# ruanjue/smartdenovo

Hardware: AMD Instinct MI355X
Metric: Gbp of candidate pairs aligned/sec (wtzmo all-vs-all) (higher is better)
Workload: dtype int32/int16

## Files before the change

include/wtzmo_hip.h:

```cpp
#ifndef WTZMO_HIP_H
#define WTZMO_HIP_H

#include <stdint.h>

#ifdef __cplusplus
extern "C" {
#endif

#define WTZ_OK        0
#define WTZ_E_ARG    -1
#define WTZ_E_HIP    -2
#define WTZ_E_POOL   -3
#define WTZ_E_STATE  -4

typedef struct {
	uint32_t ksize, zsize, hk, hz, ksave, kovl, ncand, nbest;
	uint32_t kwin, kstep, ztot, zovl, max_kmer_freq, max_zmer_freq, max_kmer_var;
	float    win_rep_norm, win_rep_cutoff;
	int32_t  w, ew, W, M, X, O, E, T;
	int32_t  min_score; float min_id;
	int32_t  dot_matrix, xvar, yvar, min_block_len, max_overhang;
	float    deviation_penalty, gap_penalty;
	int32_t  refine;
	int32_t  aux_strand;
// ... 21 lines not shown
typedef struct { int32_t beg[2], end[2]; } wtz_winbox_t;

typedef struct {
	int32_t  score, tb, te, qb, qe, aln, mat, mis, ins, del;
	uint32_t n_regs;
	uint32_t cigar_len;
	uint64_t cigar_off;
	uint32_t text_len;
	uint32_t pad;
	uint64_t text_off;
} wtz_aln_result_t;

typedef struct {
	double   ms_index, ms_zindex, ms_candidates, ms_pairs, ms_winalign, ms_stitch;
	uint64_t n_candidates_q, n_pairs, n_winalign, n_stitch;
	uint64_t cells_shift, cells_fixed, cells_global;
	uint64_t bytes_seed_algo;
	uint64_t pool_peak;
	double   ms_ext;
	uint64_t n_extjobs;
	double   ms_gap;
	uint64_t bytes_zmer_algo;
	double   ms_ingest;
	uint64_t bytes_ingest_algo;
	double   ms_local;
	uint64_t n_local, cells_local;
	double   ms_kext;
	uint64_t n_kext, cells_kext;
	double   ms_kglob;
	uint64_t n_kglob, cells_kglob;
	uint64_t ticks_kglob_dp, ticks_kglob_tb;
	double   ms_pwtext;
	uint64_t n_pwtext, bytes_pwtext;
} wtz_counters_t;

const char *wtz_last_error(void);
int  wtz_device_count(void);
int  wtz_device_memory(int device, uint64_t *free_bytes, uint64_t *total_bytes);

int  wtz_ctx_create(int device, const wtz_params_c *params, uint64_t pool_bytes, wtz_ctx_t **out);
void wtz_ctx_destroy(wtz_ctx_t *ctx);
int  wtz_ctx_clone(wtz_ctx_t *parent, uint64_t pool_bytes, wtz_ctx_t **out);

int  wtz_upload_reads(wtz_ctx_t *ctx, const uint64_t *bits, uint64_t n_words, const uint64_t *rdoff, const uint32_t *rdlen, uint32_t n_reads);

int  wtz_upload_reads_ascii(wtz_ctx_t *ctx, const char *seq, uint64_t n_bases, const uint64_t *rdoff, const uint32_t *rdlen, uint32_t n_reads, uint64_t rand_calls_before, uint64_t *n_random);
int  wtz_append_revcomp_views(wtz_ctx_t *ctx);
int  wtz_fetch_read_bits(wtz_ctx_t *ctx, uint64_t *bits, uint64_t n_words);

int  wtz_index_build(wtz_ctx_t *ctx, uint32_t id_beg, uint32_t id_end, uint32_t *max_kmer_freq, wtz_index_stats_t *stats);

int  wtz_index_count(wtz_ctx_t *ctx, uint32_t id_beg, uint32_t id_end, uint64_t *n_distinct, uint64_t *n_occ);
int  wtz_index_counts_fetch(wtz_ctx_t *ctx, uint64_t *kmers, uint32_t *cnts);
int  wtz_index_finish(wtz_ctx_t *ctx, const uint32_t *total_cnt, uint32_t K, uint64_t *n_kept);
int  wtz_candidate_groups_begin(wtz_ctx_t *ctx, const uint32_t *qids, uint32_t nq);
int  wtz_candidate_groups_end(wtz_ctx_t *ctx, uint32_t *ngroups);
int  wtz_candidate_groups_fetch(wtz_ctx_t *ctx, uint64_t *groups, uint64_t total);
void wtz_cand_tail_host(const uint64_t *groups, uint32_t ng, uint32_t kovl, uint32_t ncand, uint64_t *heap, uint32_t *hn);

int  wtz_zindex_build(wtz_ctx_t *ctx);
int  wtz_zindex_build_subset(wtz_ctx_t *ctx, const uint32_t *ids, uint32_t n);
int  wtz_zindex_build_queries(wtz_ctx_t *ctx, const uint32_t *ids, uint32_t n);

int  wtz_candidates(wtz_ctx_t *ctx, const uint32_t *qids, uint32_t nq, uint64_t *cand, uint32_t *ncand_io);
int  wtz_candidates_begin(wtz_ctx_t *ctx, const uint32_t *qids, uint32_t nq, const uint64_t *cand, const uint32_t *ncand_in);
int  wtz_candidates_end(wtz_ctx_t *ctx, uint64_t *cand, uint32_t *ncand_out);
// ... 74 lines not shown
```

smartdenovo_amd/csrc/host/wtzmo_main.c:

```c
#define _GNU_SOURCE
#include <getopt.h>
#include <unistd.h>
#include <time.h>
#include <pthread.h>
#include <sys/uio.h>
#include <errno.h>
#include <sys/stat.h>
#include <fcntl.h>
#include "wtz_host.h"
#include "wtz_ovlb.h"
static int usage(void){
	printf(
	"WTZMO (MI355X): overlapper of long reads using homopolymer compressed k-mer seeding\n"
	"Drop-in for SMARTdenovo wtzmo 1.0 -- identical options and file formats; hot path on the GPU\n"
	"Usage: wtzmo [options]\n"
	" -t <int>    accepted for compatibility (the GPU path is deterministic and equals `wtzmo -t 1`)\n"
	" -P <int> -p <int>  total parallel jobs / index of this job\n"
	" -i <string> long reads (+) *   -I <string> query-only reads (+)   -b <string> clip regions (+)\n"
	" -J <int>    min read length    -o <string> output *  -f overwrite   -9 <string> tested pairs out\n"
	" -L <string> tested pairs in (+)  -F <string> reads to mask (+)  -C no .contained file  -N seeds only\n"
	" -H <int> -k <int> -K <int> -S <int> -d <int> -G <int>      k-mer seeding [3,16,0,4,300,1]\n"
	" -z <int> -Z <int> -l <int> -y <int> -R <int> -r <int> -q <int>  z-mer windows [10,64,2,800,200,300,100]\n"
	" -U <float>x5 | -U -1   dot-matrix engine    -A <int> -B <int> candidates / best [500,100]\n"
	" -w -e -W -M -X -O -E -T  alignment [50,800,3200,2,-5,-3,-1,-50]   -s <int> -m <float> [200,0.5]\n"
// ... 311 lines not shown
		ixjobs_join(E, ixth, ixj);
		const double ti = now_s();
		shard_index_build(E, n_rd, &K);
		t_index += now_s() - ti;
		build_zindex(E, zmod);
	}
	for(uint32_t i_idx = 0; i_idx < E->n_idx && !E->shard; i_idx++){
		pbbeg = pbend; pbend = pbbeg + (n_rd + E->n_idx - 1) / E->n_idx;
		const double ti = now_s();
		rc = wtz_index_build(E->ctx, pbbeg, pbend > n_rd ? n_rd : pbend, &K, &ist); DIE_WTZ(rc, "wtz_index_build");
		t_index += now_s() - ti;
		fprintf(stderr, "[wtzmo-mi355x] index %u/%u: %llu k-mer occurrences, %llu distinct, %llu kept, cutoff %u\n", i_idx + 1, E->n_idx,
			(unsigned long long)ist.n_occ, (unsigned long long)ist.n_distinct, (unsigned long long)ist.n_kept, K);
		if(i_idx + 1 >= E->n_idx){ build_zindex(E, zmod); break; }
		uint32_t n = 0;
		for(uint32_t j = 0; j < n_rd; j++){ if((j % E->n_job) != E->i_job) continue; if(E->masked[j]) continue; ids[n++] = j; }
		for(uint32_t a = 0; a < n; a += 4096){
			uint32_t m = n - a < 4096 ? n - a : 4096;
			uint64_t *tmp_rows = (uint64_t*)hx_realloc(NULL, (size_t)m * E->stride * 8); uint32_t *tmp_n = (uint32_t*)hx_realloc(NULL, (size_t)m * 4);
			for(uint32_t k = 0; k < m; k++){ memcpy(tmp_rows + (size_t)k * E->stride, E->rows + (size_t)ids[a + k] * E->stride, (size_t)E->stride * 8); tmp_n[k] = E->nrow[ids[a + k]]; }
			rc = wtz_candidates(E->ctx, ids + a, m, tmp_rows, tmp_n); DIE_WTZ(rc, "wtz_candidates");
			for(uint32_t k = 0; k < m; k++) g_pass_keep_rows(E, ids[a + k], tmp_rows + (size_t)k * E->stride, tmp_n[k]);
			free(tmp_rows); free(tmp_n);
		}
	}
	if(!E->shard) ixjobs_join(E, ixth, ixj);
	free(ids); return t_index;
}
static void ctx_counters_fold(eng_t *E, wtz_ctx_t *ctx, uint32_t w){
		wtz_counters_t cw; wtz_get_counters(ctx, &cw);
		if(w){ E->step.extra_ms[0] += cw.ms_candidates; E->step.extra_ms[1] += cw.ms_pairs; E->step.extra_ms[2] += cw.ms_winalign; E->step.extra_ms[3] += cw.ms_stitch; E->step.extra_ms[4] += cw.ms_ext; E->step.extra_ms[5] += cw.ms_gap; }
		E->step.extra_u64[0] += cw.cells_shift; E->step.extra_u64[1] += cw.cells_fixed; E->step.extra_u64[2] += cw.cells_global; E->step.extra_u64[3] += cw.bytes_seed_algo; E->step.extra_u64[4] += cw.n_extjobs; E->step.extra_u64[6] += cw.bytes_zmer_algo;
		if(cw.pool_peak > E->step.extra_u64[5]) E->step.extra_u64[5] = cw.pool_peak;
		if(w) wtz_ctx_destroy(ctx); else wtz_reset_counters(ctx);
}
static batch_t *batches_create(eng_t *E, uint32_t nw_run, int nalt, uint64_t pool_bytes){
	const uint32_t nw = nw_run + (uint32_t)nalt; int rc; batch_t *bs = (batch_t*)calloc(nw, sizeof(batch_t));
	const uint32_t nparts = g_dist.world > 1 ? (uint32_t)g_dist.world : (nw_run == 1 ? E->ndev : 1);
	for(uint32_t w = 0; w < nw; w++){
		bs[w].E = E;
		bs[w].nparts = nparts; bs[w].parts = (part_t*)calloc(nparts, sizeof(part_t)); bs[w].spare = (part_t*)calloc(nparts, sizeof(part_t)); bs[w].cparts = bs[w].parts;
		for(uint32_t d = 0; d < nparts; d++){
			part_t *pt = &bs[w].parts[d]; const uint32_t slot = w * nparts + d;
			pt->ext_base = slot < 8 ? (int)slot * 2 : -1;
			if(slot < 8) for(int k = 0; k < 2; k++){ pt->cigs[k] = E->cig_keep[slot * 2 + k]; pt->capcigs[k] = E->cig_keep_cap[slot * 2 + k]; E->cig_keep[slot * 2 + k] = NULL; E->cig_keep_cap[slot * 2 + k] = 0; }
			if(g_dist.world > 1){ pt->remote = (int)d; pt->ctx = d == 0 ? E->ctx : NULL; }
			else if(w == 0 || (nalt && w == 1)) pt->ctx = E->ctxs[d];
			else { rc = wtz_ctx_clone(E->ctx, pool_bytes, &pt->ctx); DIE_WTZ(rc, "wtz_ctx_clone"); }
		}
		bs[w].ctx = bs[w].parts[0].ctx;
	}
	if(nalt){ bs[0].alt = &bs[1]; bs[1].alt = &bs[0]; bs[1].shares_ctx = 1; }
	return bs;
}
static void batches_destroy(eng_t *E, batch_t *bs, uint32_t nw){
	const uint32_t nparts = nw ? bs[0].nparts : 0;
	for(uint32_t w = 0; w < nw; w++){
		for(uint32_t d = 0; d < nparts; d++){
			part_t *pt = &bs[w].parts[d]; const uint32_t slot = w * nparts + d;
			if((w || d) && pt->ctx && !bs[w].shares_ctx) ctx_counters_fold(E, pt->ctx, w);
			free(pt->cq_ids); free(pt->cq_nr); free(pt->cq_rows);
			free(pt->pq); free(pt->pc); free(pt->sum); free(pt->box_off); free(pt->boxes); free(pt->item_of); free(pt->it_pair); free(pt->it_dir); free(pt->aln);
			for(int k = 0; k < 2; k++){ if(slot < 8){ E->cig_keep[slot * 2 + k] = pt->cigs[k]; E->cig_keep_cap[slot * 2 + k] = pt->capcigs[k]; } else wtz_host_free(pt->cigs[k]); }
		}
		for(uint32_t d = 0; d < nparts; d++){ part_t *sp = &bs[w].spare[d]; free(sp->sum); free(sp->box_off); free(sp->boxes); free(sp->item_of); free(sp->it_pair); free(sp->it_dir); free(sp->aln); }
		free(bs[w].spare);
		free(bs[w].parts); free(bs[w].start_job);
		free(bs[w].bq); free(bs[w].want); free(bs[w].ids); free(bs[w].rows); free(bs[w].nrow); free(bs[w].rowpair); free(bs[w].pf_ids); free(bs[w].pf_rows); free(bs[w].pf_nr);
	}
	free(bs);
}
static void run_queries(eng_t *E, uint64_t pool_bytes){
	const uint32_t n_rd = E->st.n_rd;
	const uint32_t qbeg = E->st.n_qr ? n_rd : 0;
	E->step.qend = E->st.n_qr ? n_rd + E->st.n_qr : n_rd;
	E->step.cursor = qbeg; E->step.B = E->max_batch < E->first_batch ? E->max_batch : E->first_batch;
	if(!E->first_batch_set && E->n_workers == 1){
		uint32_t nq = 0; for(uint32_t j = qbeg; j < E->step.qend; j++) if((j % E->n_job) == E->i_job) nq++;
		if(nq <= E->max_batch) E->step.B = E->max_batch;
	}
	uint32_t nw = E->step.rows_all ? 1 : E->n_workers;
	const int nalt = (nw == 1 && g_dist.world == 1 && !E->step.rows_all && !(getenv("WTZ_BATCH_OVERLAP") && !atoi(getenv("WTZ_BATCH_OVERLAP"))) && !(getenv("WTZ_RANGE_OVERLAP") && !atoi(getenv("WTZ_RANGE_OVERLAP")))) ? 1 : 0;
	batch_t *bs = batches_create(E, nw, nalt, pool_bytes); pthread_t th[8];
	if(g_dist.rank > 0){
		part_t *me = &bs[0].parts[0]; me->ctx = E->ctx; me->remote = 0; me->ext_base = -1;
		remote_loop(E, me);
	} else {
		for(uint32_t w = 1; w < nw; w++) pthread_create(&th[w], NULL, worker_main, &bs[w]);
		worker_main(&bs[0]); for(uint32_t w = 1; w < nw; w++) pthread_join(th[w], NULL);
		if(g_dist.world > 1){ wtz_dist_hdr_t h; memset(&h, 0, sizeof h); h.cmd = WTZ_CMD_DONE; g_dist.bcast(&h, sizeof h); }
	}
	batches_destroy(E, bs, nw + (uint32_t)nalt);
}
static void step_report(eng_t *E, const opts_t *o, double t_step, double t_index){
	const char *statsf = o->statsf;
	wtz_counters_t cn; wtz_get_counters(E->ctx, &cn);
	cn.ms_candidates += E->step.extra_ms[0]; cn.ms_pairs += E->step.extra_ms[1]; cn.ms_winalign += E->step.extra_ms[2]; cn.ms_stitch += E->step.extra_ms[3]; cn.ms_ext += E->step.extra_ms[4]; cn.ms_gap += E->step.extra_ms[5];
	cn.cells_shift += E->step.extra_u64[0]; cn.cells_fixed += E->step.extra_u64[1]; cn.cells_global += E->step.extra_u64[2]; cn.bytes_seed_algo += E->step.extra_u64[3]; cn.n_extjobs += E->step.extra_u64[4]; cn.bytes_zmer_algo += E->step.extra_u64[6];
	if(E->step.extra_u64[5] > cn.pool_peak) cn.pool_peak = E->step.extra_u64[5];
	memset(E->step.extra_ms, 0, sizeof E->step.extra_ms); memset(E->step.extra_u64, 0, sizeof E->step.extra_u64);
	fprintf(stderr, "[wtzmo-mi355x] %llu records, %llu pairs aligned, %llu pair-bp, %.3f s (index %.3f s)\n", (unsigned long long)E->step.nrec, (unsigned long long)E->step.n_pairs, (unsigned long long)E->step.pair_bp, t_step, t_index);
	fprintf(stderr, "[wtzmo-mi355x] host seconds: in GPU-stage calls %.3f, commit %.3f, per-batch z-index %.3f; writer thread: formatting %.3f, write %.3f; waiting for it: %.3f before buffer reuse, %.3f at the end\n", E->step.t_gpu, E->step.t_commit, E->step.t_zbatch, g_ow.t_format, g_ow.t_write, E->step.t_io[0], E->step.t_io[1]);
	fprintf(stderr, "[wtzmo-mi355x] commit sections: candidate rows + closed filter + order %.3f, window depth + seed weights %.3f, hits %.3f; planning the pairs of the ranges %.3f\n", E->step.t_cq[0], E->step.t_cq[1], E->step.t_cq[2], E->step.t_cq[3]);
	fprintf(stderr, "[wtzmo-mi355x] queries prepared ahead of the commit by helper threads: %llu taken, %llu prepared again (their read's closed pairs had moved), %.3f s waited for a helper, %.3f s starting / joining them; merging the queries' results into the global state (flush) %.3f s; the sections below count the committing thread only\n", (unsigned long long)E->step.n_spec_hit, (unsigned long long)E->step.n_spec_miss, E->step.t_spec_wait, E->step.t_spec_ctl, E->step.t_flush);
	fprintf(stderr, "[wtzmo-mi355x] window depth + seed weights in parts: window marks %.3f, running depth %.3f, seed weights %.3f, seed order %.3f\n", E->step.t_cq1[0], E->step.t_cq1[1], E->step.t_cq1[2], E->step.t_cq1[3]);
	fprintf(stderr, "[wtzmo-mi355x] wall seconds per call: candidates %.3f pairs_seed %.3f pairs_windows %.3f pairs_align %.3f cigar_text %.3f\n", E->step.t_call[0], E->step.t_call[1], E->step.t_call[2], E->step.t_call[3], E->step.t_call[4]);
	if(E->step.n_split) fprintf(stderr, "[wtzmo-mi355x] %llu range(s) had to be split after a scratch-pool overflow (planned at %.0f KB per pair)\n", (unsigned long long)E->step.n_split, E->step.bytes_per_pair / 1024.0);
	fprintf(stderr, "[wtzmo-mi355x] %llu batches in %llu ranges on %u worker context(s); speculation: queries %llu/%llu pairs %llu/%llu alignments %llu/%llu (used/planned)\n",
			(unsigned long long)E->step.n_batches, (unsigned long long)E->step.n_ranges, E->step.rows_all ? 1u : E->n_workers, (unsigned long long)E->step.used_queries, (unsigned long long)E->step.spec_queries, (unsigned long long)E->step.used_pairs, (unsigned long long)E->step.spec_pairs, (unsigned long long)E->step.used_items, (unsigned long long)E->step.spec_items);
	fprintf(stderr, "[wtzmo-mi355x] kernel ms: index %.1f zindex %.1f candidates %.1f pairs %.1f winalign %.1f stitch %.1f (K-sw3 wave %.1f, K-sw2 gaps %.1f); cells shift %llu fixed %llu global %llu; pool peak %.2f GB\n",
		cn.ms_index, cn.ms_zindex, cn.ms_candidates, cn.ms_pairs, cn.ms_winalign, cn.ms_stitch, cn.ms_ext, cn.ms_gap, (unsigned long long)cn.cells_shift, (unsigned long long)cn.cells_fixed, (unsigned long long)cn.cells_global, cn.pool_peak / 1073741824.0);
	if(statsf){ FILE *sf = fopen(statsf, "a"); if(sf){ fprintf(sf, "%llu\t%llu\t%.6f\t%.6f\t%.3f\t%.3f\t%.3f\t%.3f\t%.3f\t%.3f\t%llu\t%llu\t%llu\t%llu\t%llu\t%.3f\t%llu\t%llu\t%llu\t%.3f\t%llu\t%llu\t%llu\t%.4f\t%llu\t%.4f\t%.4f\t%.4f\t%.4f\t%.4f\t%.4f\t%llu\t%llu\n", (unsigned long long)E->step.n_pairs, (unsigned long long)E->step.pair_bp, t_step, t_index,
			cn.ms_index, cn.ms_zindex, cn.ms_candidates, cn.ms_pairs, cn.ms_winalign, cn.ms_stitch, (unsigned long long)cn.cells_shift, (unsigned long long)cn.cells_fixed, (unsigned long long)cn.cells_global, (unsigned long long)cn.bytes_seed_algo, (unsigned long long)E->step.nrec,
			cn.ms_ext, (unsigned long long)cn.n_extjobs, (unsigned long long)E->step.used_queries, (unsigned long long)cn.pool_peak, cn.ms_gap, (unsigned long long)E->step.n_ranges, (unsigned long long)E->step.n_split, (unsigned long long)cn.bytes_zmer_algo, E->ing_ms, (unsigned long long)E->ing_bytes,
			E->step.t_gpu, E->step.t_commit, E->step.t_cq[0], E->step.t_cq[1], E->step.t_cq[2], E->step.t_cq[3], (unsigned long long)E->step.n_batches, (unsigned long long)E->step.spec_queries); fclose(sf); } }
}
static void write_side_files(eng_t *E, const opts_t *o){
	const char *output = o->output, *pairoutf = o->pairoutf; const uint32_t n_rd = E->st.n_rd;
	if(o->write_contained && strcmp(output, "-")){
		char *maskf = (char*)hx_realloc(NULL, strlen(output) + 16); sprintf(maskf, "%s.contained", output);
		FILE *mf = fopen(maskf, "w");
		for(uint32_t i = 0; i < n_rd; i++) if(E->masked[i]) fprintf(mf, "%s\n", E->st.reads[i].name);
		fclose(mf); free(maskf);
	}
	if(pairoutf){
		FILE *pf = fopen(pairoutf, "w");
		hx_refslots_t T; hx_refslots_init(&T, 1023);
		for(size_t i = 0; i < E->n_order; i++){ if(E->closed_order[i] & 1u) hx_refslots_touch(&T); else hx_refslots_put(&T, E->closed_order[i]); }
		for(uint64_t k = 0; k < T.size; k++) if(T.full[k]) fprintf(pf, "%s\t%s\n", E->st.reads[(uint32_t)(T.slot[k] >> 33)].name, E->st.reads[(uint32_t)((T.slot[k] & 0xFFFFFFFFu) >> 1)].name);
		fclose(pf); free(T.slot); free(T.full);
	}
}
#ifdef WTZ_AS_LIB
int wtzmo_main(int argc, char **argv){
	optind = 1;
#else
int main(int argc, char **argv){
#endif
	eng_t *E = (eng_t*)calloc(1, sizeof(eng_t));
	E->st.keep_text = 1;
	E->bpp_decay = getenv("WTZ_BPP_DECAY") ? atof(getenv("WTZ_BPP_DECAY")) : 0.0;
	wtz_params_c *P = &E->P;
	opts_t o; memset(&o, 0, sizeof o); pthread_mutex_init(&E->mu, NULL); pthread_cond_init(&E->cv, NULL);
	{ const int r = parse_options(argc, argv, E, &o); if(r >= 0) return r; }
// ... 73 lines not shown
```

smartdenovo_amd/csrc/host/wtzmo_types.h:

```cpp
static double now_s(void){ struct timespec t; clock_gettime(CLOCK_MONOTONIC, &t); return (double)t.tv_sec + 1e-9 * (double)t.tv_nsec; }
static inline void cpu_relax(void){
#if defined(__x86_64__) || defined(__i386__)
	__builtin_ia32_pause();
#elif defined(__aarch64__) || defined(__arm__)
	__asm__ __volatile__("yield");
#else
	sched_yield();
#endif
}
#define SWAP(T, a, b) do { T t_ = (a); (a) = (b); (b) = t_; } while(0)
typedef struct { uint64_t e; uint32_t pidx; uint32_t pad; } cand_t;
#define GT_CAND(a, b) ((uint32_t)(b)->e > (uint32_t)(a)->e)
HX_DEFINE_SORT_EXACT(sort_cands_exact, cand_t, GT_CAND)
static int gt_read(const void *a, const void *b, void *ctx){ (void)ctx; return ((const hx_read_t*)b)->len > ((const hx_read_t*)a)->len; }

typedef struct { uint32_t pb2, dir, ovl, closed, pidx; } seed_t;
#define GT_SEED(a, b) ((b)->ovl > (a)->ovl)
HX_DEFINE_SORT_EXACT(sort_seeds_exact, seed_t, GT_SEED)
typedef struct {
	cand_t *cand; size_t capcand; seed_t *seeds; size_t capseeds; uint16_t *dep; size_t capdep;
	uint32_t nc, nseed, ngate; double t[5];
} cq_work_t;

typedef struct { uint32_t pb1, pb2, dir2; int qb, qe, tb, te, score, mat, mis, ins, del, aln; char *cigar; } hit_t;
// ... 10 lines not shown
	wtz_params_c P; int do_align; uint32_t n_idx, n_job, i_job;
	hx_store_t st; uint8_t *masked; uint32_t *rdcovs; hx_set_t closed;
	uint32_t *rdlen; uint32_t avg_rdlen;
	uint64_t *closed_order; size_t n_order, cap_order; int keep_order;
	wtz_ctx_t *ctx; FILE *out;
	double ing_ms; uint64_t ing_bytes;
	int zbatch;
	int binary_out;
	int zsplit;
	int shard;
	uint32_t ndev; int devs[8]; wtz_ctx_t *ctxs[8];
	uint64_t *rows; uint32_t *nrow; uint32_t stride;
	uint32_t max_batch, first_batch, n_workers; int first_batch_set;
	pthread_mutex_t mu; pthread_cond_t cv;
	double bpp_decay; uint64_t main_cap;
	pending_t pend;
	cq_work_t cq;
	struct cq_spec_s *spec;
	uint32_t *closed_touch;
	char *cig_keep[16]; uint64_t cig_keep_cap[16];
	uint64_t cand_main_cap; uint32_t cand_cap0;
	uint8_t *masked0; uint64_t *closed0; size_t nclosed0, n_order0;
	struct {
		int rows_all; uint32_t cursor, qend, B; uint64_t next_seq, commit_seq; double bytes_per_pair; uint64_t n_split, n_ranges;
		uint64_t pair_bp, n_pairs, nrec, n_spec_hit, n_spec_miss; double t_spec_wait, t_spec_ctl, t_flush;
		double t_cq1[4];
		double t_cq[4];
		double t_gpu, t_commit, t_zbatch, t_call[6], t_io[2];
		uint64_t spec_pairs, used_pairs, spec_items, used_items, spec_queries, used_queries, n_batches;
		double pair_row_ratio;
		uint64_t n_masked;
		double cand_bpq;
		double last_mask_rate;
		double extra_ms[6]; uint64_t extra_u64[7];
	} step;
} eng_t;
typedef void (*wtz_dist_bcast_fn)(void *buf, uint64_t nbytes);
typedef void (*wtz_dist_send_fn)(const void *buf, uint64_t nbytes, int dst);
typedef void (*wtz_dist_recv_fn)(void *buf, uint64_t nbytes, int src);
typedef void (*wtz_dist_send_dev_fn)(const void *dev_buf, uint64_t nbytes, int dst);
static struct { int rank, world; wtz_dist_bcast_fn bcast; wtz_dist_send_fn send; wtz_dist_recv_fn recv; wtz_dist_send_dev_fn send_dev; } g_dist = { 0, 1, NULL, NULL, NULL, NULL };
void wtzmo_set_dist(int rank, int world, wtz_dist_bcast_fn b, wtz_dist_send_fn sd, wtz_dist_recv_fn rv){
	g_dist.rank = rank; g_dist.world = world < 1 ? 1 : world; g_dist.bcast = b; g_dist.send = sd; g_dist.recv = rv; g_dist.send_dev = NULL;
}
void wtzmo_set_dist_dev(wtz_dist_send_dev_fn f){ g_dist.send_dev = f; }
#define WTZ_DIST_MAX 16
enum { WTZ_CMD_DONE = 1, WTZ_CMD_PAIRS = 2, WTZ_CMD_CAND_BEGIN = 3, WTZ_CMD_CAND_END = 4, WTZ_CMD_GRP_BEGIN = 5, WTZ_CMD_GRP_END = 6,
       WTZ_CMD_ZIDX = 7,
       WTZ_CMD_ABORT = 8 };
typedef struct { uint64_t cmd, arg[2], count[WTZ_DIST_MAX]; } wtz_dist_hdr_t;
enum { WTZ_ST_OK = 0, WTZ_ST_AGAIN = 1, WTZ_ST_FAILED = 2 };

typedef struct {
	wtz_ctx_t *ctx; int remote;
	uint8_t *xbuf; uint64_t xcap;
	uint32_t *pq, *pc; uint32_t npair, cappair;
	wtz_pair_summary_t *sum; uint64_t *box_off; wtz_winbox_t *boxes; uint64_t nbox, capbox;
	uint32_t *item_of; uint32_t *it_pair; uint8_t *it_dir; uint32_t nitem; wtz_aln_result_t *aln; char *cig; uint64_t ncig;
	void *cig_dev;
	int text_pending;
	char *cigs[2]; uint64_t capcigs[2]; int cig_sel, cig_ext, ext_base;
	double t_call[6], t_io0;
	struct eng_s *E; int again;
	uint32_t *cq_ids, *cq_nr; uint64_t *cq_rows; uint32_t cq_n, cq_cap;
} part_t;
#define PIDX(part, local) (((uint32_t)(local) << 4) | (uint32_t)(part))
#define PART_OF(b, g) (&(b)->parts[(g) & 15u])
// ... 29 lines not shown
```

smartdenovo_amd/csrc/wtz_ctx.h:

```cpp
struct wtz_switches {
	uint32_t xcd_group = 256;
	int zread = 1;
	int ext_fused = 1;
	int ext_pk = 1;
	int heavy_first = -1;
	int gap_lane = 1;
	int lane = 1;
	bool trace = false;
	bool fail_once = false;
	unsigned fail_at = 0, tfail_at = 0;
	int dm_first_big = 1;
	int sw_mode = 0;
	int gap_side = 0;
	bool profile = false;
};
static int env_int(const char *name, int dflt){ const char *e = getenv(name); return e ? atoi(e) : dflt; }
static void wtz_switches_read(wtz_switches *s){
	s->xcd_group = (uint32_t)env_int("WTZ_XCD_GROUP", (int)s->xcd_group);
	s->zread = env_int("WTZ_ZREAD", s->zread);
	s->ext_fused = env_int("WTZ_EXT_FUSED", s->ext_fused);
	s->ext_pk = env_int("WTZ_EXT_PK", s->ext_pk);
	s->heavy_first = env_int("WTZ_PAIR_HEAVY_FIRST", s->heavy_first);
	s->gap_lane = env_int("WTZ_GAP_LANE", s->gap_lane);
	s->lane = env_int("WTZ_WINALIGN_LANE", s->lane);
// ... 4 lines not shown
#ifndef WTZ_EMUL
	s->dm_first_big = env_int("WTZ_DM_FIRST_BIG", s->dm_first_big);
	s->sw_mode = env_int("WTZ_SW_CHECK", 0) ? 2 : env_int("WTZ_SW_SCALAR", 0) ? 1 : 0;
	s->gap_side = env_int("WTZ_GAP_SIDESTREAM", 0) ? 1 : 0;
	s->profile = getenv("WTZ_PROFILE_PAIR") != NULL;
#endif
}

struct wtz_ctx {
	int device = 0;
	wtz_switches sw;
	struct zslot_t {
		std::vector<std::pair<void*, size_t> > parked, live;
		uint64_t *zoff = NULL; uint64_t n_z = 0; wtz_zindex_t Z; bool have = false; bool sub = false; uint64_t sub_cap = 0;
		zslot_t(){ memset(&Z, 0, sizeof Z); }
	} zs[2];
#ifndef WTZ_EMUL
	hipStream_t stream = 0;
	hipStream_t stream_side = 0; hipEvent_t ev_side_fork = 0, ev_side_join = 0;
	hipStream_t stream_gap = 0; hipEvent_t ev_gap_fork = 0, ev_gap_join = 0;
#endif
	bool shares_indexes = false;
	void *kpark_p[2] = {NULL, NULL}; size_t kpark_b[2] = {0, 0}, klive_b[2] = {0, 0};
	wtz_arena arena;
	uint32_t cap_pairs = 0, cap_items = 0;
	wtz_params_t P = wtz_params_t(); wtz_params_t *dP = NULL;
	uint64_t *bits = NULL; uint64_t n_words = 0; uint64_t *rdoff = NULL; uint32_t *rdlen = NULL; uint32_t n_reads = 0;
	std::vector<uint32_t> h_rdlen;
	wtz_kslot_t *ktab = NULL; uint64_t kmask = 0; uint32_t *kseeds = NULL; uint64_t n_kocc = 0;
	uint64_t *pend_keys = NULL; uint32_t *pend_vals = NULL; uint64_t pend_tot = 0; uint64_t *pend_dk = NULL, *pend_dstart = NULL; uint32_t *pend_dc = NULL; uint64_t pend_nd = 0; uint32_t pend_beg = 0, pend_end = 0;
	uint64_t *cq_gptr = NULL; uint32_t cq_gcap = 0; bool cq_groups = false; std::vector<uint32_t> cq_ng;
	uint32_t idx_beg = 0, idx_end = 0; bool idx_len_sorted = false;
	wtz_pool_t *dpool = NULL; uint8_t *pool_base = NULL; uint64_t pool_bytes = 0, main_bytes = 0;
	uint32_t *d_qid = NULL, *d_cid = NULL; wtz_pairres_t *d_pairres = NULL; uint32_t n_pairs = 0; std::vector<wtz_pairres_t> h_pairres;
	wtz_alnres_dev_t *d_alnres = NULL; uint32_t n_items = 0; std::vector<wtz_alnres_dev_t> h_alnres;
	char *d_text = NULL; size_t cap_text = 0;
#ifndef WTZ_EMUL
	hipStream_t stream_copy = 0; hipEvent_t ev_text_ready = 0, ev_text_done[2] = {0, 0}; std::atomic<uint64_t> text_begun{0}, text_known_done{0}, text_ended{0};
#endif
	bool have_pairs = false, have_items = false;
	uint32_t *cq_thr = NULL;
	uint32_t *cq_q = NULL, *cq_nc = NULL; uint64_t *cq_cand = NULL; unsigned long long *cq_bytes = NULL; uint32_t cq_cap = 0, cq_n = 0; bool cq_pending = false; wtz_timer cq_tm;
	wtz_counters_t cnt = wtz_counters_t();
	uint64_t tpool_peak_call = 0, main_used_call = 0;
	int last_pool_fail = 0;
	double ext_use_ratio = 0.4; uint64_t tpool_last_used = 0;
	bool fused_ran = false;
	unsigned long long ext_fr_total = 0;
	unsigned long long ext_open_total = 0;
};

#ifndef WTZ_EMUL
#define CTX_ENTER(c) (void)hipSetDevice((c)->device); g_stream = (c)->stream; wtz_arena_scope arena_scope_(&(c)->arena)
#else
#define CTX_ENTER(c) wtz_arena_scope arena_scope_(&(c)->arena)
#endif

#define STAGE(c, name) do { if((c)->sw.trace){ (void)dev_sync(); fprintf(stderr, "[stage] %s\n", name); fflush(stderr); } } while(0)

static wtz_reads_t ctx_reads(const wtz_ctx *c){ wtz_reads_t R; R.bits = c->bits; R.rdoff = c->rdoff; R.rdlen = c->rdlen; R.n_reads = c->n_reads; return R; }
static wtz_env_t ctx_env(const wtz_ctx *c){ wtz_env_t V; V.R = ctx_reads(c); V.Z = c->zs[0].Z; V.ZQ = c->zs[1].have ? c->zs[1].Z : c->zs[0].Z; V.P = c->dP; V.pool = c->dpool; V.dm_first_big = (uint32_t)c->sw.dm_first_big; return V; }

static int tpool_reset(wtz_ctx *c){
	wtz_pool_t p; wtz_pool_init(&p, c->pool_base + c->main_bytes, c->pool_bytes - c->main_bytes, c->sw.tfail_at);
	return dev_h2d(c->dpool + 1, &p, sizeof p);
}
static int pool_reset(wtz_ctx *c){
	wtz_pool_t p; wtz_pool_init(&p, c->pool_base, c->main_bytes, c->sw.fail_at);
	CHK(dev_h2d(c->dpool, &p, sizeof p));
	c->tpool_peak_call = 0;
	return tpool_reset(c);
}
static int tpool_check(wtz_ctx *c, const char *stage){
	wtz_pool_t p; CHK(dev_d2h(&p, c->dpool + 1, sizeof p));
	const uint64_t u = p.used > p.cap ? p.cap : p.used;
	c->tpool_last_used = u;
	if(u > c->tpool_peak_call) c->tpool_peak_call = u;
	if(p.overflow && c->sw.fail_once) c->sw.tfail_at = 0;
	if(p.overflow) c->last_pool_fail = 2;
	if(p.overflow) return wtz_fail(WTZ_E_POOL, "%s: transient trace pool exhausted (%llu of %llu bytes requested); use a larger pool",
		stage, (unsigned long long)p.used, (unsigned long long)p.cap);
	return WTZ_OK;
}
static int pool_check(wtz_ctx *c, const char *stage){
	wtz_pool_t p; CHK(dev_d2h(&p, c->dpool, sizeof p));
	const uint64_t u = (p.used > p.cap ? p.cap : p.used);
	c->main_used_call = u;
	if(u + c->tpool_peak_call > c->cnt.pool_peak) c->cnt.pool_peak = u + c->tpool_peak_call;
	if(p.overflow && c->sw.fail_once) c->sw.fail_at = 0;
	if(p.overflow) c->last_pool_fail = 1;
	if(p.overflow) return wtz_fail(WTZ_E_POOL, "%s: device scratch pool exhausted (%llu of %llu bytes requested); use fewer items per call or a larger pool",
		stage, (unsigned long long)p.used, (unsigned long long)p.cap);
	return WTZ_OK;
}
extern "C" int wtz_device_count(void){
#ifndef WTZ_EMUL
	int n = 0; if(hipGetDeviceCount(&n) != hipSuccess) return 0; return n;
#else
	return 1;
#endif
}

extern "C" int wtz_device_memory(int device, uint64_t *free_bytes, uint64_t *total_bytes){
	if(!free_bytes || !total_bytes) return wtz_fail(WTZ_E_ARG, "null argument");
#ifndef WTZ_EMUL
	int prev = 0; HIPCHK(hipGetDevice(&prev)); HIPCHK(hipSetDevice(device));
	size_t fr = 0, tot = 0; const hipError_t e = hipMemGetInfo(&fr, &tot); (void)hipSetDevice(prev);
	if(e != hipSuccess) return wtz_fail(WTZ_E_HIP, "hipMemGetInfo: %s", hipGetErrorString(e));
	*free_bytes = fr; *total_bytes = tot;
#else
	(void)device; *free_bytes = *total_bytes = 16ull << 30;
#endif
	return WTZ_OK;
}

extern "C" int wtz_ctx_create(int device, const wtz_params_c *params, uint64_t pool_bytes, wtz_ctx_t **out){
	if(!params || !out) return wtz_fail(WTZ_E_ARG, "null argument");
	if(params->ksize < 5 || params->ksize > 32 || params->zsize < 5 || params->zsize > 16 || params->ksave < 1) return wtz_fail(WTZ_E_ARG, "k/z/S out of range (wtzmo.c:1658-1660)");
#ifndef WTZ_EMUL
	int ndev = 0;
	if(hipGetDeviceCount(&ndev) != hipSuccess || ndev == 0) return wtz_fail(WTZ_E_HIP, "no HIP device visible: libwtzmo_hip needs an MI355X (gfx950); there is no CPU fallback");
	if(device < 0 || device >= ndev) return wtz_fail(WTZ_E_ARG, "device %d out of range (%d visible)", device, ndev);
	HIPCHK(hipSetDevice(device));
#endif
	wtz_ctx *c = new wtz_ctx();
	c->device = device; c->P = *params; wtz_switches_read(&c->sw);
	c->pool_bytes = pool_bytes ? pool_bytes : (4ull << 30);
#ifndef WTZ_EMUL
	if(!pool_bytes){
		size_t fr = 0, tot = 0;
		if(hipMemGetInfo(&fr, &tot) == hipSuccess && fr / 20 * 9 > c->pool_bytes) c->pool_bytes = (uint64_t)(fr / 20 * 9);
		if(c->pool_bytes > (128ull << 30)) c->pool_bytes = 128ull << 30;
		if(const char *e = getenv("WTZ_DEFAULT_POOL_MB")){ const long long mb = atoll(e); if(mb >= 64 && ((uint64_t)mb << 20) < c->pool_bytes) c->pool_bytes = (uint64_t)mb << 20; }
	}
#endif
	c->pool_bytes &= ~(uint64_t)4095; c->main_bytes = (c->pool_bytes / 2) & ~(uint64_t)4095;
#ifndef WTZ_EMUL
	{ void *ab = NULL; const size_t acap = (size_t)3 << 29;
	  if(hipMalloc(&ab, acap) == hipSuccess){ c->arena.base = (uint8_t*)ab; c->arena.cap = acap; } }
	if(hipStreamCreateWithFlags(&c->stream, hipStreamNonBlocking) != hipSuccess
			|| hipStreamCreateWithFlags(&c->stream_side, hipStreamNonBlocking) != hipSuccess || hipEventCreateWithFlags(&c->ev_side_fork, hipEventDisableTiming) != hipSuccess
			|| hipEventCreateWithFlags(&c->ev_side_join, hipEventDisableTiming) != hipSuccess
			|| hipStreamCreateWithFlags(&c->stream_gap, hipStreamNonBlocking) != hipSuccess || hipEventCreateWithFlags(&c->ev_gap_fork, hipEventDisableTiming) != hipSuccess
			|| hipEventCreateWithFlags(&c->ev_gap_join, hipEventDisableTiming) != hipSuccess){ wtz_ctx_destroy(c); return wtz_fail(WTZ_E_HIP, "hipStreamCreate / hipEventCreate failed"); }
	g_stream = c->stream;
#endif
	int rc;
	if((rc = dev_alloc_persist((void**)&c->dP, sizeof(wtz_params_t))) || (rc = dev_h2d(c->dP, &c->P, sizeof(wtz_params_t))) ||
	   (rc = dev_alloc_persist((void**)&c->dpool, 2 * sizeof(wtz_pool_t)))){
		wtz_ctx_destroy(c); return rc;
	}
	for(;;){
#ifndef WTZ_EMUL
		if(!pool_bytes && c->pool_bytes > (4ull << 30)){
			if(hipMalloc((void**)&c->pool_base, c->pool_bytes) == hipSuccess){ rc = WTZ_OK; break; }
			(void)hipGetLastError();
			c->pool_base = NULL;
			uint64_t nb = c->pool_bytes / 2; if(nb < (4ull << 30)) nb = 4ull << 30;
			c->pool_bytes = nb & ~(uint64_t)4095; c->main_bytes = (c->pool_bytes / 2) & ~(uint64_t)4095;
			continue;
		}
#endif
		rc = dev_alloc_persist((void**)&c->pool_base, c->pool_bytes);
		break;
	}
	if(rc || (rc = pool_reset(c))){
		wtz_ctx_destroy(c); return rc;
	}
	*out = c;
	return WTZ_OK;
}

static void free_pending_index(wtz_ctx *c);
static void kpark(wtz_ctx *c, int w, void *p, size_t bytes){ if(!p) return; if(c->kpark_p[w]) dev_free_persist(c->kpark_p[w]); c->kpark_p[w] = p; c->kpark_b[w] = bytes; }
static void kflush(wtz_ctx *c){ for(int w = 0; w < 2; w++){ if(c->kpark_p[w]) dev_free_persist(c->kpark_p[w]); c->kpark_p[w] = NULL; c->kpark_b[w] = 0; } }
static int kalloc(wtz_ctx *c, int w, void **p, size_t n){
	if(c->kpark_p[w] && c->kpark_b[w] >= n && c->kpark_b[w] <= n + n / 8 + ((size_t)1 << 20)){ *p = c->kpark_p[w]; c->klive_b[w] = c->kpark_b[w]; c->kpark_p[w] = NULL; c->kpark_b[w] = 0; return WTZ_OK; }
	if(c->kpark_p[w]){ dev_free_persist(c->kpark_p[w]); c->kpark_p[w] = NULL; c->kpark_b[w] = 0; }
	int rc = dev_alloc_persist(p, n); if(rc == WTZ_OK) c->klive_b[w] = n; return rc;
}
static void free_kindex(wtz_ctx *c){
	if(!c->shares_indexes){
		if(c->klive_b[0]) kpark(c, 0, c->ktab, c->klive_b[0]); else dev_free_persist(c->ktab);
		if(c->klive_b[1]) kpark(c, 1, c->kseeds, c->klive_b[1]); else dev_free_persist(c->kseeds);
		c->klive_b[0] = c->klive_b[1] = 0;
	}
	c->ktab = NULL; c->kseeds = NULL; c->kmask = 0;
}
static int zalloc(wtz_ctx::zslot_t *z, void **p, size_t n){
	if(n == 0) n = 16;
	for(size_t i = 0; i < z->parked.size(); i++){
		if(z->parked[i].second >= n && z->parked[i].second <= n + n / 8 + 4096){
			*p = z->parked[i].first; z->live.push_back(z->parked[i]); z->parked.erase(z->parked.begin() + (long)i); return WTZ_OK;
		}
	}
	int rc = dev_alloc_persist(p, n); if(rc) return rc;
	z->live.push_back(std::make_pair(*p, n)); return WTZ_OK;
}
static void zpark_all(wtz_ctx::zslot_t *z){ for(size_t i = 0; i < z->live.size(); i++) z->parked.push_back(z->live[i]); z->live.clear(); }
static void zflush_parked(wtz_ctx::zslot_t *z){ for(size_t i = 0; i < z->parked.size(); i++) dev_free_persist(z->parked[i].first); z->parked.clear(); }
static void free_zindex(wtz_ctx *c){
	for(int k = 0; k < 2; k++){
		wtz_ctx::zslot_t *z = &c->zs[k];
		if(!c->shares_indexes){ zpark_all(z); zflush_parked(z); }
		z->zoff = NULL; memset(&z->Z, 0, sizeof z->Z); z->have = false; z->sub = false; z->sub_cap = 0; z->n_z = 0;
	}
}
static void free_batch(wtz_ctx *c){ c->n_pairs = 0; c->n_items = 0; c->have_pairs = false; c->have_items = false; }
static void free_batch_storage(wtz_ctx *c){
	dev_free_persist(c->d_qid); dev_free_persist(c->d_cid); dev_free_persist(c->d_pairres); dev_free_persist(c->d_alnres);
	c->d_qid = c->d_cid = NULL; c->d_pairres = NULL; c->d_alnres = NULL; c->cap_pairs = c->cap_items = 0; free_batch(c);
}
static int reserve_pairs(wtz_ctx *c, uint32_t n){
	if(n <= c->cap_pairs && c->d_pairres) return WTZ_OK;
	uint32_t cap = c->cap_pairs ? c->cap_pairs : 4096; while(cap < n) cap *= 2;
	(void)dev_sync();
	dev_free_persist(c->d_qid); dev_free_persist(c->d_cid); dev_free_persist(c->d_pairres); c->d_qid = c->d_cid = NULL; c->d_pairres = NULL; c->cap_pairs = 0;
	CHK(dev_alloc_persist((void**)&c->d_qid, (size_t)cap * 4)); CHK(dev_alloc_persist((void**)&c->d_cid, (size_t)cap * 4));
	CHK(dev_alloc_persist((void**)&c->d_pairres, (size_t)cap * sizeof(wtz_pairres_t)));
	c->cap_pairs = cap; return WTZ_OK;
}
static int reserve_items(wtz_ctx *c, uint32_t m){
	if(m <= c->cap_items && c->d_alnres) return WTZ_OK;
	uint32_t cap = c->cap_items ? c->cap_items : 4096; while(cap < m) cap *= 2;
	(void)dev_sync();
	dev_free_persist(c->d_alnres); c->d_alnres = NULL; c->cap_items = 0;
	CHK(dev_alloc_persist((void**)&c->d_alnres, (size_t)cap * sizeof(wtz_alnres_dev_t)));
	c->cap_items = cap; return WTZ_OK;
}

extern "C" void wtz_ctx_destroy(wtz_ctx_t *c){
	if(!c) return;
	{ CTX_ENTER(c); (void)dev_sync(); }
	free_batch_storage(c); free_kindex(c); if(!c->shares_indexes) kflush(c); free_zindex(c);
	dev_free_persist(c->d_text);
	dev_free_persist(c->cq_q); dev_free_persist(c->cq_nc); dev_free_persist(c->cq_cand); dev_free_persist(c->cq_bytes); dev_free_persist(c->cq_thr); dev_free_persist(c->cq_gptr);
	free_pending_index(c);
#ifndef WTZ_EMUL
	arena_cache_flush(&c->arena);
	if(c->arena.base) (void)hipFree(c->arena.base);
#endif
	if(!c->shares_indexes){ dev_free_persist(c->bits); dev_free_persist(c->rdoff); dev_free_persist(c->rdlen); }
	dev_free_persist(c->dP); dev_free_persist(c->dpool); dev_free_persist(c->pool_base);
#ifndef WTZ_EMUL
	if(c->stream_side) (void)hipStreamDestroy(c->stream_side);
	if(c->stream_gap) (void)hipStreamDestroy(c->stream_gap);
	if(c->stream_copy){ (void)hipStreamSynchronize(c->stream_copy); (void)hipStreamDestroy(c->stream_copy); if(c->ev_text_ready) (void)hipEventDestroy(c->ev_text_ready); for(int k = 0; k < 2; k++) if(c->ev_text_done[k]) (void)hipEventDestroy(c->ev_text_done[k]); }
	{ hipEvent_t evs[4] = { c->ev_side_fork, c->ev_side_join, c->ev_gap_fork, c->ev_gap_join }; for(int k = 0; k < 4; k++) if(evs[k]) (void)hipEventDestroy(evs[k]); }
	if(c->stream) (void)hipStreamDestroy(c->stream);
#endif
	delete c;
}

extern "C" int wtz_ctx_clone(wtz_ctx_t *p, uint64_t pool_bytes, wtz_ctx_t **out){
	if(!p || !out) return wtz_fail(WTZ_E_ARG, "null argument");
	wtz_ctx_t *c = NULL;
	int rc = wtz_ctx_create(p->device, &p->P, pool_bytes ? pool_bytes : p->pool_bytes, &c);
	if(rc) return rc;
	c->shares_indexes = true;
	c->bits = p->bits; c->n_words = p->n_words; c->rdoff = p->rdoff; c->rdlen = p->rdlen; c->n_reads = p->n_reads; c->h_rdlen = p->h_rdlen;
	c->ktab = p->ktab; c->kmask = p->kmask; c->kseeds = p->kseeds; c->n_kocc = p->n_kocc;
	c->idx_beg = p->idx_beg; c->idx_end = p->idx_end; c->idx_len_sorted = p->idx_len_sorted;
	for(int k = 0; k < 2; k++){ c->zs[k].zoff = p->zs[k].zoff; c->zs[k].n_z = p->zs[k].n_z; c->zs[k].Z = p->zs[k].Z; c->zs[k].have = p->zs[k].have; }
	*out = c;
	return WTZ_OK;
}
```

smartdenovo_amd/csrc/wtz_dev.h:

```cpp
static thread_local char g_err[512] = "";
#define CHK(call) do { int rc_ = (call); if(rc_ != WTZ_OK) return rc_; } while(0)
static int wtz_fail(int code, const char *fmt, ...){
	va_list ap; va_start(ap, fmt); vsnprintf(g_err, sizeof g_err, fmt, ap); va_end(ap);
	return code;
}
#include <chrono>
static double wtz_wall(){ return std::chrono::duration<double>(std::chrono::steady_clock::now().time_since_epoch()).count(); }
#ifndef WTZ_EMUL
#include <hip/hip_runtime.h>
#include <rocprim/rocprim.hpp>
#define WTZ_LAMBDA __device__
#ifndef WTZ_OCC_WINALIGN
#define WTZ_OCC_WINALIGN 3
#endif
#ifndef WTZ_OCC_PAIR_DM
#define WTZ_OCC_PAIR_DM 4
#endif
#ifndef WTZ_OCC_PAIR
#define WTZ_OCC_PAIR 5
#endif
#ifndef WTZ_OCC_GAP
#define WTZ_OCC_GAP 3
#endif

static thread_local hipStream_t g_stream = 0;
#define HIPCHK(call) do { hipError_t e_ = (call); if(e_ != hipSuccess) return wtz_fail(WTZ_E_HIP, "%s failed: %s (%s:%d)", #call, hipGetErrorString(e_), __FILE__, __LINE__); } while(0)

#define WTZ_LAUNCH(kernel, blocks, threads, lds_bytes, stream, ...) do { hipLaunchKernelGGL(kernel, dim3(blocks), dim3(threads), lds_bytes, stream, __VA_ARGS__); HIPCHK(hipGetLastError()); } while(0)
struct wtz_stream_scope { hipStream_t prev;
	wtz_stream_scope(hipStream_t st) : prev(g_stream) { g_stream = st; }
	~wtz_stream_scope(){ g_stream = prev; }
	wtz_stream_scope(const wtz_stream_scope&) = delete; wtz_stream_scope &operator=(const wtz_stream_scope&) = delete; };

template<typename TAG, typename F> __global__ void __launch_bounds__(64) wtz_kernel_tasks(uint64_t n, F f){
	uint64_t i = (uint64_t)blockIdx.x * blockDim.x + threadIdx.x;
	WTZ_PROF_BEGIN();
	if(i < n) f(i);
	WTZ_PROF_END();
}
template<typename TAG, typename F> static int wtz_launch(uint64_t n, F f){
	if(n == 0) return WTZ_OK;
	const uint32_t bs = 64;
	uint64_t nb = (n + bs - 1) / bs;
	if(nb > 0x7FFFFFFFull) return wtz_fail(WTZ_E_ARG, "grid too large");
	WTZ_LAUNCH((wtz_kernel_tasks<TAG, F>), (uint32_t)nb, bs, 0, g_stream, n, f);
	return WTZ_OK;
}
template<typename TAG, typename F> __global__ void __launch_bounds__(64) wtz_kernel_wave_tasks(uint64_t n, F f){
	const uint64_t i = blockIdx.x;
	WTZ_PROF_BEGIN();
	if(i < n && threadIdx.x == 0) f(i);
	WTZ_PROF_END();
}
template<typename TAG> struct wtz_occ { static constexpr int waves = 1; };
template<> struct wtz_occ<K_winalign> { static constexpr int waves = WTZ_OCC_WINALIGN; };
template<> struct wtz_occ<K_pair> { static constexpr int waves = WTZ_OCC_PAIR; };
template<> struct wtz_occ<K_pair_dm> { static constexpr int waves = WTZ_OCC_PAIR_DM; };
template<> struct wtz_occ<K_pair_zbig> { static constexpr int waves = 2; };
template<> struct wtz_occ<K_gap> { static constexpr int waves = WTZ_OCC_GAP; };
#ifndef WTZ_OCC_LDP
#define WTZ_OCC_LDP 2
#endif
template<> struct wtz_occ<K_ldp> { static constexpr int waves = WTZ_OCC_LDP; };
template<> struct wtz_occ<K_gdp> { static constexpr int waves = WTZ_OCC_LDP; };
// ... 46 lines not shown
		}
	}
	if(hipMalloc(p, n) != hipSuccess){
		(void)hipGetLastError();
		if(g_arena && !g_arena->cache.empty()){ (void)hipDeviceSynchronize(); arena_cache_flush(g_arena); }
		HIPCHK(hipMalloc(p, n));
	}
	if(g_arena){ g_arena->overflow.push_back(*p); g_arena->overflow_bytes.push_back(n); }
	return WTZ_OK;
}
static void arena_cache_flush(wtz_arena *a){ for(size_t i = 0; i < a->cache.size(); i++) (void)hipFree(a->cache[i].first); a->cache.clear(); a->cache_bytes = 0; }
struct wtz_arena_scope { wtz_arena *a, *prev; size_t mark; size_t nover;
	wtz_arena_scope(wtz_arena *ar) : a(ar), prev(g_arena), mark(ar ? ar->top : 0), nover(ar ? ar->overflow.size() : 0) { g_arena = ar; }
	~wtz_arena_scope(){
		g_arena = prev;
		if(!a) return;
		if(a->overflow.size() > nover){
			(void)hipStreamSynchronize(g_stream);
			while(a->overflow.size() > nover){
				void *q = a->overflow.back(); const size_t qb = a->overflow_bytes.back(); a->overflow.pop_back(); a->overflow_bytes.pop_back();
				if(a->cache_bytes + qb <= WTZ_ARENA_CACHE_BYTES && a->cache.size() < 16){ a->cache.push_back(std::make_pair(q, qb)); a->cache_bytes += qb; }
				else (void)hipFree(q);
			}
		}
		a->top = mark;
	} };
static int dev_alloc_persist(void **p, size_t n){
	if(hipMalloc(p, n ? n : 16) == hipSuccess) return WTZ_OK;
	(void)hipGetLastError();
	if(g_arena && !g_arena->cache.empty()){ (void)hipDeviceSynchronize(); arena_cache_flush(g_arena); }
	HIPCHK(hipMalloc(p, n ? n : 16)); return WTZ_OK;
}
static void dev_free_persist(void *p){ if(p) (void)hipFree(p); }
static int dev_h2d(void *d, const void *h, size_t n){ if(n){ HIPCHK(hipMemcpyAsync(d, h, n, hipMemcpyHostToDevice, g_stream)); HIPCHK(hipStreamSynchronize(g_stream)); } return WTZ_OK; }
static int dev_d2h(void *h, const void *d, size_t n){ if(n){ HIPCHK(hipMemcpyAsync(h, d, n, hipMemcpyDeviceToHost, g_stream)); HIPCHK(hipStreamSynchronize(g_stream)); } return WTZ_OK; }
static int dev_set(void *d, int v, size_t n){ if(n) HIPCHK(hipMemsetAsync(d, v, n, g_stream)); return WTZ_OK; }
static int dev_d2d(void *d, const void *s, size_t n){ if(n) HIPCHK(hipMemcpyAsync(d, s, n, hipMemcpyDeviceToDevice, g_stream)); return WTZ_OK; }
static int dev_sync(){ HIPCHK(hipStreamSynchronize(g_stream)); return WTZ_OK; }

struct wtz_timer { hipEvent_t a, b; bool ok;
	wtz_timer(){ ok = hipEventCreate(&a) == hipSuccess && hipEventCreate(&b) == hipSuccess; }
	~wtz_timer(){ if(ok){ (void)hipEventDestroy(a); (void)hipEventDestroy(b); } }
	void start(){ if(ok) (void)hipEventRecord(a, g_stream); }
	double stop(){ float ms = 0; if(ok){ (void)hipEventRecord(b, g_stream); (void)hipEventSynchronize(b); (void)hipEventElapsedTime(&ms, a, b); } return ms; }
	void lap(){ if(ok) (void)hipEventRecord(b, g_stream); }
	double read(){ float ms = 0; if(ok){ (void)hipEventSynchronize(b); (void)hipEventElapsedTime(&ms, a, b); } return ms; } };

static int dev_sort_pairs_u64_u32(uint64_t *keys, uint32_t *vals, uint64_t n, unsigned end_bit){
	if(n < 2) return WTZ_OK;
	uint64_t *k2 = NULL; uint32_t *v2 = NULL; void *tmp = NULL; size_t tmp_bytes = 0; int rc;
	if((rc = dev_alloc((void**)&k2, n * 8))) return rc;
	if((rc = dev_alloc((void**)&v2, n * 4))) return rc;
	rocprim::double_buffer<uint64_t> kb(keys, k2); rocprim::double_buffer<uint32_t> vb(vals, v2);
	hipError_t e = rocprim::radix_sort_pairs(tmp, tmp_bytes, kb, vb, (size_t)n, 0u, end_bit, g_stream);
	if(e == hipSuccess && (rc = dev_alloc(&tmp, tmp_bytes)) == WTZ_OK){
		e = rocprim::radix_sort_pairs(tmp, tmp_bytes, kb, vb, (size_t)n, 0u, end_bit, g_stream);
		if(e == hipSuccess) e = hipStreamSynchronize(g_stream);
		if(e == hipSuccess && kb.current() != keys){ e = hipMemcpyAsync(keys, kb.current(), n * 8, hipMemcpyDeviceToDevice, g_stream); if(e == hipSuccess) e = hipMemcpyAsync(vals, vb.current(), n * 4, hipMemcpyDeviceToDevice, g_stream); if(e == hipSuccess) e = hipStreamSynchronize(g_stream); }
	}
	if(e != hipSuccess) return wtz_fail(WTZ_E_HIP, "radix_sort_pairs failed: %s", hipGetErrorString(e));
	return rc;
}
static int dev_exclusive_scan_u32(const uint32_t *in, uint32_t *out, uint64_t n){
	if(n == 0) return WTZ_OK;
	void *tmp = NULL; size_t tmp_bytes = 0;
	hipError_t e = rocprim::exclusive_scan(tmp, tmp_bytes, in, out, 0u, (size_t)n, rocprim::plus<uint32_t>(), g_stream);
	if(e != hipSuccess) return wtz_fail(WTZ_E_HIP, "exclusive_scan failed: %s", hipGetErrorString(e));
	CHK(dev_alloc(&tmp, tmp_bytes));
	e = rocprim::exclusive_scan(tmp, tmp_bytes, in, out, 0u, (size_t)n, rocprim::plus<uint32_t>(), g_stream);
	if(e == hipSuccess) e = hipStreamSynchronize(g_stream);
	if(e != hipSuccess) return wtz_fail(WTZ_E_HIP, "exclusive_scan failed: %s", hipGetErrorString(e));
	return WTZ_OK;
}
#else
#define WTZ_LAMBDA
template<typename TAG, typename F> static int wtz_launch(uint64_t n, F f){ for(uint64_t i = 0; i < n; i++) f(i); return WTZ_OK; }
template<typename TAG, typename F> static int wtz_launch_wave(uint64_t n, F f){ return wtz_launch<TAG>(n, f); }
template<typename TAG, typename F> static int wtz_launch_coop(uint64_t n, F f, uint32_t = 0){ return wtz_launch<TAG>(n, f); }
template<typename TAG, typename F> static int wtz_launch_wg(uint64_t n, F f, uint32_t, uint32_t){ for(uint64_t i = 0; i < n; i++) f(i); return WTZ_OK; }
struct wtz_arena { std::vector<void*> blocks; };
static thread_local wtz_arena *g_arena = NULL;
static int dev_alloc_persist(void **p, size_t n){ *p = malloc(n ? n : 16); return *p ? WTZ_OK : wtz_fail(WTZ_E_HIP, "malloc(%zu) failed", n); }
static void dev_free_persist(void *p){ free(p); }
static int dev_alloc(void **p, size_t n){
	if(!g_arena){ *p = NULL; return wtz_fail(WTZ_E_STATE, "dev_alloc(%zu) outside the arena scope of an API call", n); }
	CHK(dev_alloc_persist(p, n)); g_arena->blocks.push_back(*p); return WTZ_OK;
}
struct wtz_arena_scope { wtz_arena *a, *prev; size_t mark;
	wtz_arena_scope(wtz_arena *ar) : a(ar), prev(g_arena), mark(ar ? ar->blocks.size() : 0) { g_arena = ar; }
	~wtz_arena_scope(){ g_arena = prev; if(!a) return; while(a->blocks.size() > mark){ free(a->blocks.back()); a->blocks.pop_back(); } } };
static int dev_h2d(void *d, const void *h, size_t n){ if(n) memcpy(d, h, n); return WTZ_OK; }
static int dev_d2h(void *h, const void *d, size_t n){ if(n) memcpy(h, d, n); return WTZ_OK; }
static int dev_set(void *d, int v, size_t n){ if(n) memset(d, v, n); return WTZ_OK; }
static int dev_d2d(void *d, const void *s, size_t n){ if(n) memcpy(d, s, n); return WTZ_OK; }
static int dev_sync(){ return WTZ_OK; }
#include <time.h>
struct wtz_timer { struct timespec t0; void start(){ clock_gettime(CLOCK_MONOTONIC, &t0); }
	double stop(){ struct timespec t1; clock_gettime(CLOCK_MONOTONIC, &t1); return 1e3 * (double)(t1.tv_sec - t0.tv_sec) + 1e-6 * (double)(t1.tv_nsec - t0.tv_nsec); }
	double lapv = 0; void lap(){ lapv = stop(); } double read(){ return lapv; } };
static int dev_exclusive_scan_u32(const uint32_t *in, uint32_t *out, uint64_t n){ uint32_t a = 0; for(uint64_t i = 0; i < n; i++){ uint32_t v = in[i]; out[i] = a; a += v; } return WTZ_OK; }
static int dev_sort_pairs_u64_u32(uint64_t *keys, uint32_t *vals, uint64_t n, unsigned){
	std::vector<std::pair<uint64_t, uint32_t> > v((size_t)n);
	for(uint64_t i = 0; i < n; i++) v[(size_t)i] = std::make_pair(keys[i], vals[i]);
	std::stable_sort(v.begin(), v.end(), [](const std::pair<uint64_t, uint32_t> &a, const std::pair<uint64_t, uint32_t> &b){ return a.first < b.first; });
	for(uint64_t i = 0; i < n; i++){ keys[i] = v[(size_t)i].first; vals[i] = v[(size_t)i].second; }
	return WTZ_OK;
}
#endif

#ifndef WTZ_EMUL
static void *dev_host_alloc(size_t n){ void *p = NULL; if(hipHostMalloc(&p, n, hipHostMallocDefault) != hipSuccess){ (void)hipGetLastError(); return NULL; } return p; }
static void dev_host_free(void *p){ (void)hipHostFree(p); }
#else
static void *dev_host_alloc(size_t n){ return malloc(n); }
static void dev_host_free(void *p){ free(p); }
#endif
```

smartdenovo_amd/csrc/wtz_lib.cpp:

```cpp
#include <stdio.h>
#include <stdlib.h>
#include <stdarg.h>
#include <vector>
#include <atomic>
#include <algorithm>

#include "wtz_tasks.h"
#include "wtz_sw_frame.h"
#include "wtz_stitch_fused.h"
#include "wtz_sw_local.h"
#include "wtz_sw_kext.h"
#include "wtz_sw_kglob.h"
#include "wtz_pwtext.h"

struct K_candidates_wg;
struct K_extjob_scalar;
struct K_cigar_text;
struct K_misc;
struct K_gap;
struct K_gap_wide;
struct K_kcount;
struct K_lcount;
struct K_lplan;
struct K_ldp;
struct K_ltb;
struct K_lfold;
struct K_gplan;
struct K_gdp;
struct K_gtb;
struct K_glist;
struct K_poolalloc;
struct K_kfill;
struct K_kinsert;
struct K_khead;
struct K_kdistinct;
struct K_kinsert_total;
struct K_pack_groups;
struct K_kstats;
struct K_pack_cigars;
struct K_pack_windows;
struct K_pair;
struct K_pair_dm;
struct K_pair_zbig;
struct K_pair_big;
struct K_refine;
struct K_pack_ascii;
struct K_pack_fix;
struct K_revcomp_views;
struct K_stitch_fin;
struct K_stitch_left;
struct K_stitch_mid;
struct K_winalign;
struct K_winalign_big;
struct K_zfill; struct K_zread;
struct K_zrun;
struct K_zdistinct;
struct K_zdn;
struct K_zcount;
struct K_extcopy;
struct K_globcopy;
struct K_glob_ring;
struct K_glob_scalar;

#include "wtz_dev.h"
#include "wtz_ctx.h"
#include "wtz_lib_index.h"
#include "wtz_lib_pairs.h"
#include "wtz_lib_align.h"
#include "wtz_lib_fetch.h"
#include "wtz_lib_batch.h"

extern "C" const char *wtz_last_error(void){ return g_err; }
extern "C" void *wtz_host_alloc(uint64_t n_bytes){ return dev_host_alloc((size_t)(n_bytes ? n_bytes : 1)); }
extern "C" void wtz_host_free(void *p){ if(p) dev_host_free(p); }

extern "C" int wtz_pool_failure_kind(wtz_ctx_t *c){ return c ? c->last_pool_fail : 0; }

extern "C" int wtz_pool_info(wtz_ctx_t *c, wtz_pool_info_t *out){
	if(!c || !out) return wtz_fail(WTZ_E_ARG, "null argument");
	out->main_cap = c->main_bytes; out->main_used = c->main_used_call; out->transient_cap = c->pool_bytes - c->main_bytes; out->transient_peak = c->tpool_peak_call;
	return WTZ_OK;
}

extern "C" int wtz_get_counters(wtz_ctx_t *c, wtz_counters_t *out){
	if(!c || !out) return wtz_fail(WTZ_E_ARG, "null argument");
	*out = c->cnt;
#if !defined(WTZ_EMUL) && defined(WTZ_PROFILE)
	if(c->sw.profile){
		unsigned long long h[64], z[64]; memset(z, 0, sizeof z);
		if(hipMemcpyFromSymbol(h, HIP_SYMBOL(wtz_prof), sizeof h) == hipSuccess){
			fprintf(stderr, "[phase-profile] Mticks:");
			for(int k = 0; k < 64; k++) fprintf(stderr, " %d:%.1f", k, (double)h[k] / 1e6);
			fprintf(stderr, "\n");
			(void)hipMemcpyToSymbol(HIP_SYMBOL(wtz_prof), z, sizeof z);
		}
	}
#endif
// ... 15 lines not shown
```

smartdenovo_amd/csrc/wtz_lib_align.h:

```cpp
#ifndef WTZ_EMUL
WTZ_HD uint64_t wtz_ext_trace_need(int32_t qlen, int32_t tlen, int32_t init, int32_t W, int32_t M, int32_t O, int32_t E, int32_t T, int32_t *ql_out, int32_t *ncol_out){
	if(ql_out) *ql_out = 0;
	if(ncol_out) *ncol_out = 0;
	if(qlen <= 0 || tlen <= 0) return 0;
	if(init < 0) init = 0;
	int32_t ql, tl, n_col;
	wtz_ext_geometry(qlen, tlen, init, W, M, O, O, E, T, ql, tl, n_col);
	if(ql_out) *ql_out = ql;
	if(ncol_out) *ncol_out = n_col;
	const uint64_t c_reg = ((uint64_t)(n_col + 63) / 64 + 3) / 4, c_mw = ((uint64_t)(n_col + 255) / 256 + 3) / 4 * 4, c_gen = ((((uint64_t)(n_col + 63) / 64) | 1) + 3) / 4;
	uint64_t zrow = (c_reg > c_gen ? c_reg : c_gen) * 256; if(c_mw * 256 > zrow) zrow = c_mw * 256;
	uint64_t nb = ((uint64_t)(ql + 63) / 64) * 64 * zrow + (uint64_t)WTZ_TRACE_MAXCHUNK * 8 + (uint64_t)(ql + 2) * 4 + 256;
	if((n_col + 63) / 64 > 32 || (tl + 63) / 32 + 1 > 1032){
		uint64_t z = 1024; while(z < (uint64_t)ql * (uint64_t)n_col) z <<= 1;
		uint64_t r = 64; while(r < (uint64_t)tl + 3) r <<= 1;
		uint64_t zb = 64; while(zb < (uint64_t)ql + 2) zb <<= 1;
		nb = z + 8 * r + 4 * zb + 256;
	}
	return nb;
}
static uint64_t ext_trace_need(const wtz_ctx *c, int32_t qlen, int32_t tlen, int32_t init, int32_t W, int32_t *ql_out, int32_t *ncol_out){
	return wtz_ext_trace_need(qlen, tlen, init, W, c->P.M, c->P.O, c->P.E, c->P.T, ql_out, ncol_out);
}

// ... 8 lines not shown
		const int32_t pM = c->P.M, pO = c->P.O, pE = c->P.E, pT = c->P.T, pW = -c->P.ew;
		const bool use_pk = c->sw.ext_pk != 0; const wtz_params_t *dP = V.P;
		CHK(wtz_launch<K_misc>(m, [=] WTZ_LAMBDA (uint64_t t){
			const wtz_extjob_t &j = d_jl[t];
			int32_t qa = 0, qb = 0;
			unsigned long long nb = wtz_ext_trace_need(j.valid ? j.qlen : -1, j.tlen, 0, pW, pM, pO, pE, pT, &qa, (int32_t*)NULL);
			nb += wtz_ext_trace_need(d_rgeo[2 * t], d_rgeo[2 * t + 1], 0, pW, pM, pO, pE, pT, &qb, (int32_t*)NULL);
			const uint32_t rows = (uint32_t)qa + (uint32_t)qb;
			uint32_t to_fr = 0;
			if(use_pk){
				if(j.valid && j.qlen > 0 && j.tlen > 0){
					int32_t W = pW, ql = 0, tl = 0, nc = 0, bias, ng, sh; const int32_t in0 = j.init_score < 0 ? 0 : j.init_score;
					wtz_ext_geometry(j.qlen, j.tlen, in0, W, pM, pO, pO, pE, pT, ql, tl, nc);
					if(!wtz_pk_window(dP, in0, ql, tl, &bias, &ng, &sh)) to_fr = 1;
				}
				if(d_rgeo[2 * t] > 0 && d_rgeo[2 * t + 1] > 0){
					const wtz_stitch_state_t &st = d_st[t]; const wtz_alnitem_t &it = d_items[t];
					long long i_lo = st.x.score, gain = 0;
					if(j.valid && j.qlen > 0 && j.tlen > 0) gain = (long long)pM * (j.qlen < j.tlen ? j.qlen : j.tlen);
					const wtz_gapres_t *gp = d_gaps + (it.regs - d_items[0].regs);
					for(uint32_t k = st.first + 1; k < it.nwin; k++) if(it.regs[k].pass == 1) i_lo += (long long)gp[k].score + it.regs[k].x.score;
					int32_t W = pW, ql = 0, tl = 0, nc = 0;
					wtz_ext_geometry(d_rgeo[2 * t], d_rgeo[2 * t + 1], 0, W, pM, pO, pO, pE, pT, ql, tl, nc);
					if(!wtz_pk_window_range(dP, ql, tl, i_lo, i_lo + gain)) to_fr = 1;
				}
			}
			d_k[t] = ((uint64_t)to_fr << 32) | (uint64_t)(0xFFFFFFFFu - rows); d_order[t] = (uint32_t)t;
			if(to_fr) WTZ_ATOMIC_ADD64(&d_acc[2], 1ull);
			if(nb) WTZ_ATOMIC_ADD64(&d_acc[0], nb);
			if(rows) WTZ_ATOMIC_ADD64(&d_acc[1], (unsigned long long)rows);
		}));
	}
	CHK(dev_sort_pairs_u64_u32(d_k, d_order, m, 33));
	unsigned long long h_acc[3] = {0, 0, 0}; CHK(dev_d2h(h_acc, d_acc, 24));
	const uint64_t acc = h_acc[0]; const unsigned long long ext_sum = h_acc[1];
	const uint64_t budget = (c->pool_bytes - c->main_bytes) / 16 * 15;
	uint32_t ng = 1; while(ng < 4 && (double)acc * c->ext_use_ratio / ng > (double)budget) ng++;
	if((double)acc * c->ext_use_ratio / ng > (double)budget){ if(c->sw.profile) fprintf(stderr, "[ext-profile] fused launch declined: %u items, trace bounds %.1f GB x %.2f against %.1f GB\n", m, acc / 1e9, c->ext_use_ratio, budget / 1e9); return WTZ_OK; }
	double ms_l = 0; uint64_t used_sum = 0;
	for(uint32_t g = 0; g < ng; g++){
		const uint32_t mg = (m - g + ng - 1) / ng;
		if(mg == 0) continue;
		CHK(tpool_reset(c));
		wtz_timer te; te.start();
		if(c->sw.ext_pk){
			uint32_t n_fr = ng == 1 ? (uint32_t)h_acc[2] : 0u;
			if(n_fr > mg) n_fr = mg;
			CHK(dev_set(d_open, 0, 4));
			if(n_fr){
				HIPCHK(hipEventRecord(c->ev_side_fork, g_stream)); HIPCHK(hipStreamWaitEvent(c->stream_side, c->ev_side_fork, 0));
				WTZ_LAUNCH((wtz_kernel_stitch_ext_fr<1032>), n_fr, 64, WTZ_WAVE_LDS_BYTES, c->stream_side, V, d_items, d_st, d_jl, d_jr, d_gaps, (const uint32_t*)d_order + (mg - n_fr), n_fr, 1u, 0u);
				HIPCHK(hipEventRecord(c->ev_side_join, c->stream_side));
			}
			const uint32_t n_pk = mg - n_fr;
			if(n_pk){
				WTZ_LAUNCH((wtz_kernel_stitch_ext_pk<1032>), n_pk, 64, WTZ_PK_LDS_BYTES(1032), g_stream, V, d_items, d_st, d_jl, d_jr, d_gaps, (const uint32_t*)d_order, n_pk, ng, g, d_open);
			}
			if(n_fr) HIPCHK(hipStreamWaitEvent(g_stream, c->ev_side_join, 0));
			uint32_t n_open = 0; CHK(dev_d2h(&n_open, d_open, 4));
			c->ext_open_total += n_open; c->ext_fr_total += n_fr;
			if(n_open){ WTZ_LAUNCH((wtz_kernel_stitch_ext_fr<1032>), n_open, 64, WTZ_WAVE_LDS_BYTES, g_stream, V, d_items, d_st, d_jl, d_jr, d_gaps, (const uint32_t*)d_open + 1, n_open, 1u, 0u); }
		} else WTZ_LAUNCH((wtz_kernel_stitch_ext_fr<1032>), mg, 64, WTZ_WAVE_LDS_BYTES, g_stream, V, d_items, d_st, d_jl, d_jr, d_gaps, (const uint32_t*)d_order, mg, ng, g);
		ms_l += te.stop();
		{
			const int rc_t = tpool_check(c, "K-sw3 extension jobs (both ends on one wavefront)");
			if(rc_t != WTZ_OK){
				c->ext_use_ratio = c->ext_use_ratio * 2.0 > 1.0 ? 1.0 : c->ext_use_ratio * 2.0;
				return rc_t;
			}
		}
		used_sum += c->tpool_last_used;
	}
	c->cnt.ms_ext += ms_l; c->cnt.n_extjobs += 2ull * m;
	c->fused_ran = true;
	if(c->sw.profile) fprintf(stderr, "[ext-profile] fused launch: %u items in %u group(s), rows (upper bound) sum %llu, %.2f ms; items of the 32-bit form so far: dealt %llu, declined by the packed form %llu\n", m, ng, ext_sum, ms_l, c->ext_fr_total, c->ext_open_total);
	c->tpool_last_used = used_sum;
	if(acc){ const double seen = 1.3 * (double)c->tpool_last_used / (double)acc, keep = c->ext_use_ratio * 0.9; c->ext_use_ratio = seen > keep ? seen : keep; if(c->ext_use_ratio < 0.2) c->ext_use_ratio = 0.2; if(c->ext_use_ratio > 1.0) c->ext_use_ratio = 1.0; }
	return WTZ_OK;
}
#endif

static int run_extjobs(wtz_ctx *c, const wtz_env_t &V, wtz_extjob_t *d_jobs, uint32_t m, bool leftover = false){
	if(m == 0) return WTZ_OK;
#ifdef WTZ_EMUL
	(void)c; (void)leftover;
	return wtz_launch_wave<K_extjob_scalar>(m, [=] WTZ_LAMBDA (uint64_t t){ wtz_task_extjob_scalar((uint32_t)t, V, d_jobs); });
#else
	if(leftover){
		if(!c->fused_ran) leftover = false;
		else {
			wtz_timer te; te.start();
			WTZ_LAUNCH((wtz_kernel_extjobs<2048, 1032>), m, 64, 0, g_stream, d_jobs, (const uint32_t*)NULL, m, V.P, V.pool, V.pool + 1);
			c->cnt.ms_ext += te.stop();
			return tpool_check(c, "K-sw3 extension jobs");
		}
	}
	const int mode = c->sw.sw_mode;
	if(mode == 1) return wtz_launch_wave<K_extjob_scalar>(m, [=] WTZ_LAMBDA (uint64_t t){ wtz_task_extjob_scalar((uint32_t)t, V, d_jobs); });
// ... 59 lines not shown
			{ std::vector<wtz_extjob_t> jj(m); CHK(dev_d2h(jj.data(), d_jobs, (size_t)m * sizeof(wtz_extjob_t))); uint32_t nd[4] = {0, 0, 0, 0}; for(uint32_t i = 0; i < m; i++){ key[i] = jj[i].valid ? jj[i].x.qe : -1; if(jj[i].valid) nd[jj[i].done & 3]++; }
			  if(const char *dp = getenv("WTZ_EXT_DUMP")){
				if(FILE *df = fopen(dp, "ab")){ for(uint32_t i = 0; i < m; i++) if(jj[i].valid){ const int32_t r[8] = {jj[i].qlen, jj[i].tlen, jj[i].init_score, jj[i].W, jj[i].x.qe, jj[i].x.te, (int32_t)(jj[i].cells > 0x7FFFFFFFull ? 0x7FFFFFFF : jj[i].cells), (int32_t)jj[i].done}; fwrite(r, 4, 8, df); } fclose(df); } }
			  fprintf(stderr, "[ext-profile] %u launch group(s); valid jobs finished by: nobody %u, 32-bit frame form %u, packed form or general kernel %u\n", n_groups, nd[0], nd[1], nd[3]); }
			for(uint32_t i = 0; i < m; i++){ if(key[i] < 0) continue; nv++; if(key[i] >= 256) n256++; if(key[i] >= 512){ n512++; s512 += key[i]; } if(key[i] >= 1024) n1k++; if(key[i] >= 2048) n2k++; if(key[i] >= 4096) n4k++; }
			fprintf(stderr, "[ext-profile] %u jobs (%u valid), rows (upper bound) sum %llu max %d, %.2f ms; qe>=256 %u >=512 %u (sum %llu) >=1k %u >=2k %u >=4k %u; transient pool peak %.2f GB\n", m, nv, ext_sum, ext_max, ms_l, n256, n512, s512, n1k, n2k, n4k, c->tpool_peak_call / 1073741824.0);
		}
	}
	if(mode == 2){
		CHK(dev_sync());
		std::vector<wtz_extjob_t> got(m); CHK(dev_d2h(got.data(), d_jobs, (size_t)m * sizeof(wtz_extjob_t)));
		for(uint32_t i = 0; i < m; i++){
			if(!got[i].valid) continue;
			if(memcmp(&got[i].x, &ref[i].x, sizeof(wtz_aln_t)) || got[i].cigar_len != ref[i].cigar_len || got[i].cells != ref[i].cells)
				return wtz_fail(WTZ_E_STATE, "K-sw3 wave kernel differs from the scalar body on job %u: qlen %d tlen %d init %d W %d; score %d/%d qe %d/%d te %d/%d aln %d/%d cigar %u/%u cells %llu/%llu",
					i, got[i].qlen, got[i].tlen, got[i].init_score, got[i].W, got[i].x.score, ref[i].x.score, got[i].x.qe, ref[i].x.qe, got[i].x.te, ref[i].x.te,
					got[i].x.aln, ref[i].x.aln, got[i].cigar_len, ref[i].cigar_len, (unsigned long long)got[i].cells, (unsigned long long)ref[i].cells);
			if(got[i].cigar_len){
				std::vector<uint32_t> a(got[i].cigar_len), b(got[i].cigar_len);
				CHK(dev_d2h(a.data(), got[i].cigar, a.size() * 4)); CHK(dev_d2h(b.data(), ref[i].cigar, b.size() * 4));
				if(a != b) return wtz_fail(WTZ_E_STATE, "K-sw3 wave kernel: CIGAR differs on job %u", i);
			}
		}
	}
	return WTZ_OK;
#endif
}

#ifdef WTZ_EMUL
#define WTZ_HOST_WAVE 1u
#else
#define WTZ_HOST_WAVE 64u
#endif
static int pool_alloc_host(wtz_ctx *c, int which, size_t bytes, void **out){
	unsigned long long *d_p = NULL; CHK(dev_alloc((void**)&d_p, 8));
	wtz_pool_t *pool = c->dpool + which;
	CHK(wtz_launch<K_poolalloc>(1, [=] WTZ_LAMBDA (uint64_t){ *d_p = (unsigned long long)(uintptr_t)wtz_pool_alloc(pool, bytes); }));
	unsigned long long h = 0; CHK(dev_d2h(&h, d_p, 8));
	if(h == 0) return wtz_fail(WTZ_E_POOL, "device scratch pool exhausted (%zu bytes for the K-sw1 problem lists)", bytes);
	*out = (void*)(uintptr_t)h; return WTZ_OK;
}
static uint32_t lane_classes(const uint32_t ccnt[4], wtz_lclass_t *L){
	uint32_t lo = 0, wv = 0;
	for(int k = 0; k < 4; k++){ const uint32_t n = ccnt[3 - k]; L->lo[k] = lo; L->hi[k] = lo + n; wv += (n + WTZ_HOST_WAVE - 1) / WTZ_HOST_WAVE; L->wend[k] = wv; lo += n; }
	return wv;
}
static size_t carve_bytes(size_t n, size_t elem){ return (n * elem + 255) & ~(size_t)255; }
template<typename T> static void carve(uint8_t *&blk, T *&out, size_t n){ out = (T*)blk; blk += carve_bytes(n, sizeof(T)); }
template<typename KEYS> static int sort_leftovers(uint32_t *d_list, uint32_t nl, KEYS launch_keys){
	if(nl <= 64) return WTZ_OK;
	uint64_t *d_k2 = NULL; CHK(dev_alloc((void**)&d_k2, (size_t)nl * 8));
	CHK(launch_keys(d_k2));
	return dev_sort_pairs_u64_u32(d_k2, d_list + 1, nl, 32);
}
static int run_winalign_lane(wtz_ctx *c, const wtz_env_t &V, const wtz_wintask_t *d_wt, uint64_t nwt, const wtz_alnitem_t *d_items, uint32_t *d_fb, uint32_t *n_fb){
	*n_fb = 0;
	if(nwt == 0) return WTZ_OK;
	const bool prof = c->sw.profile; double tp[8] = {0, 0, 0, 0, 0, 0, 0, 0}, tp0 = 0;
	if(prof){ (void)dev_sync(); tp0 = wtz_wall(); }
	auto lap = [&](int k){ if(prof){ (void)dev_sync(); const double t = wtz_wall(); tp[k] += t - tp0; tp0 = t; } };
	uint32_t *d_na = NULL, *d_woff = NULL;
	CHK(dev_alloc((void**)&d_na, (nwt + 1) * 4)); CHK(dev_alloc((void**)&d_woff, (nwt + 1) * 4));
	CHK(dev_set(d_na, 0, (nwt + 1) * 4));
	CHK(wtz_launch<K_lcount>(nwt, [=] WTZ_LAMBDA (uint64_t t){ wtz_task_lcount((uint32_t)t, d_wt, d_items, d_na); }));
	CHK(dev_exclusive_scan_u32(d_na, d_woff, nwt + 1));
	uint32_t NS = 0; CHK(dev_d2h(&NS, d_woff + nwt, 4));
	lap(0);
	wtz_lprob_t *d_prob = NULL; uint32_t *d_cap = NULL, *d_roff = NULL, *d_val = NULL, *d_ccnt = NULL, *d_uidx = NULL, *d_nu = NULL; uint64_t *d_key = NULL; uint8_t *d_flag = NULL; wtz_lres_t *d_res = NULL;
	{
		const size_t nsp = (size_t)NS + 64;
		uint8_t *blk = NULL; CHK(pool_alloc_host(c, 0, carve_bytes(nsp, sizeof(wtz_lprob_t)) + carve_bytes(nsp, sizeof(wtz_lres_t)) + 4 * carve_bytes(nsp, 4) + carve_bytes(nsp, 8), (void**)&blk));
		carve(blk, d_prob, nsp); carve(blk, d_res, nsp); carve(blk, d_cap, nsp); carve(blk, d_roff, nsp); carve(blk, d_val, nsp); carve(blk, d_uidx, nsp); carve(blk, d_key, nsp);
	}
	CHK(dev_alloc((void**)&d_flag, nwt + 16)); CHK(dev_alloc((void**)&d_nu, (nwt + 1) * 4)); CHK(dev_alloc((void**)&d_ccnt, 32)); CHK(dev_set(d_ccnt, 0, 32));
	CHK(dev_set(d_cap, 0, ((size_t)NS + 1) * 4));
	CHK(dev_set(d_res, 0, ((size_t)NS + 1) * sizeof(wtz_lres_t)));
	CHK(wtz_launch<K_lplan>(nwt, [=] WTZ_LAMBDA (uint64_t t){ wtz_task_lplan((uint32_t)t, V, d_wt, d_items, d_woff, d_prob, d_cap, d_key, d_val, d_flag, d_ccnt, d_uidx, d_nu); }));
	lap(1);
	CHK(dev_exclusive_scan_u32(d_cap, d_roff, (uint64_t)NS + 1));
	uint32_t NR = 0, ccnt[4] = {0, 0, 0, 0};
	CHK(dev_d2h(&NR, d_roff + NS, 4)); CHK(dev_d2h(ccnt, d_ccnt, 16));
	uint32_t *d_runs = NULL; CHK(pool_alloc_host(c, 0, ((size_t)NR + 16) * 4, (void**)&d_runs));
	lap(2);
	CHK(dev_sort_pairs_u64_u32(d_key, d_val, NS, 16));
	lap(3);
	CHK(dev_set(d_fb, 0, 4));
	{
		const uint32_t *d_ord = d_val; const wtz_lprob_t *pp = d_prob; const uint32_t *ro = d_roff; uint32_t *rn = d_runs; wtz_lres_t *rs = d_res;
		wtz_lclass_t L; const uint32_t wv = lane_classes(ccnt, &L);
		uint64_t *d_wtr = NULL; uint32_t *d_wrm = NULL;
		CHK(dev_alloc((void**)&d_wtr, ((size_t)wv + 1) * 8)); CHK(dev_alloc((void**)&d_wrm, ((size_t)wv + 1) * 4)); CHK(dev_set(d_wtr, 0, ((size_t)wv + 1) * 8));
		if(wv) CHK(wtz_launch_coop<K_ldp>(wv, [=] WTZ_LAMBDA (uint64_t t){ wtz_task_ldp_all((uint32_t)t, L, V, d_wt, d_items, d_ord, pp, rs, d_wtr, d_wrm); }, 0));
		lap(4);
		if(wv) CHK(wtz_launch_coop<K_ltb>(wv, [=] WTZ_LAMBDA (uint64_t t){ wtz_task_ltb_all((uint32_t)t, L, V, d_wt, d_items, d_ord, pp, ro, rn, rs, d_wtr, d_wrm); }, 0));
		lap(6);
		CHK(wtz_launch<K_lfold>(nwt, [=] WTZ_LAMBDA (uint64_t t){ wtz_task_lfold((uint32_t)t, V, d_wt, d_items, d_woff, pp, ro, rn, rs, d_flag, d_fb, d_uidx, d_nu); }));
	}
	CHK(dev_d2h(n_fb, d_fb, 4));
	{
		const uint32_t nl = *n_fb; const uint32_t *lst = d_fb + 1;
		CHK(sort_leftovers(d_fb, nl, [&](uint64_t *d_k2){ return wtz_launch<K_misc>(nl, [=] WTZ_LAMBDA (uint64_t i){
			const wtz_wintask_t tk = d_wt[lst[i]];
			const wtz_win_t &w = d_items[tk.item].win[tk.widx];
			d_k2[i] = 0xFFFFFFFFull - (unsigned long long)(w.anchors[1] - w.anchors[0]);
		}); }));
	}
	lap(5);
	if(c->sw.profile) fprintf(stderr, "[lane-profile] %llu windows, %u anchor slots, K-sw1 problems by band class <=16 / <=32 / <=64 / <=104: %u / %u / %u / %u, %u run entries, %u windows left to the chained kernel; ms: count+scan %.2f plan %.2f scan+alloc %.2f sort %.2f dp %.2f traceback %.2f fold %.2f\n",
		(unsigned long long)nwt, NS, ccnt[0], ccnt[1], ccnt[2], ccnt[3], NR, *n_fb, tp[0] * 1e3, tp[1] * 1e3, tp[2] * 1e3, tp[3] * 1e3, tp[4] * 1e3, tp[6] * 1e3, tp[5] * 1e3);
	return WTZ_OK;
}

static int run_gap_lane(wtz_ctx *c, const wtz_env_t &V, const wtz_wintask_t *d_wt, uint64_t nwt, const wtz_alnitem_t *d_items, wtz_gapres_t *d_gaps, uint32_t *d_list, uint32_t *n_list){
	*n_list = 0;
	if(nwt == 0) return WTZ_OK;
	wtz_lgap_t *d_gp = NULL; uint32_t *d_cap = NULL, *d_roff = NULL, *d_val = NULL, *d_ccnt = NULL; uint64_t *d_key = NULL; uint8_t *d_done = NULL;
	{
		const size_t nsp = (size_t)nwt + 64;
		uint8_t *blk = NULL; CHK(pool_alloc_host(c, 0, carve_bytes(nsp, sizeof(wtz_lgap_t)) + 3 * carve_bytes(nsp, 4) + carve_bytes(nsp, 8) + carve_bytes(nsp, 1), (void**)&blk));
		carve(blk, d_gp, nsp); carve(blk, d_cap, nsp); carve(blk, d_roff, nsp); carve(blk, d_val, nsp); carve(blk, d_key, nsp); carve(blk, d_done, nsp);
	}
	CHK(dev_alloc((void**)&d_ccnt, 32)); CHK(dev_set(d_ccnt, 0, 32));
	CHK(dev_set(d_cap, 0, ((size_t)nwt + 1) * 4));
	CHK(wtz_launch<K_gplan>(nwt, [=] WTZ_LAMBDA (uint64_t t){ wtz_task_gplan((uint32_t)t, V, d_wt, d_items, d_gaps, d_gp, d_cap, d_key, d_val, d_done, d_ccnt); }));
	CHK(dev_exclusive_scan_u32(d_cap, d_roff, nwt + 1));
	uint32_t NR = 0, ccnt[4] = {0, 0, 0, 0};
	CHK(dev_d2h(&NR, d_roff + nwt, 4)); CHK(dev_d2h(ccnt, d_ccnt, 16));
	uint32_t *d_runs = NULL; CHK(pool_alloc_host(c, 0, ((size_t)NR + 16) * 4, (void**)&d_runs));
	CHK(dev_sort_pairs_u64_u32(d_key, d_val, nwt, 18));
	CHK(dev_set(d_list, 0, 4));
	{
		const uint32_t *d_ord = d_val; const wtz_lgap_t *gp = d_gp; const uint32_t *ro = d_roff; uint32_t *rn = d_runs; uint8_t *dn = d_done;
		wtz_lclass_t L; const uint32_t wv = lane_classes(ccnt, &L);
		uint64_t *d_wtr = NULL; uint32_t *d_wrm = NULL; wtz_lres_t *d_res = NULL;
		CHK(dev_alloc((void**)&d_wtr, ((size_t)wv + 1) * 8)); CHK(dev_alloc((void**)&d_wrm, ((size_t)wv + 1) * 4)); CHK(dev_set(d_wtr, 0, ((size_t)wv + 1) * 8));
		CHK(pool_alloc_host(c, 0, ((size_t)nwt + 1) * sizeof(wtz_lres_t), (void**)&d_res)); CHK(dev_set(d_res, 0, ((size_t)nwt + 1) * sizeof(wtz_lres_t)));
		if(wv) CHK(wtz_launch_coop<K_gdp>(wv, [=] WTZ_LAMBDA (uint64_t t){ wtz_task_gdp_all((uint32_t)t, L, V, d_wt, d_items, d_ord, gp, d_res, d_wtr, d_wrm); }, 0));
		if(wv) CHK(wtz_launch_coop<K_gtb>(wv, [=] WTZ_LAMBDA (uint64_t t){ wtz_task_gtb_all((uint32_t)t, L, V, d_wt, d_items, d_ord, gp, ro, rn, d_res, d_gaps, dn, d_wtr, d_wrm); }, 0));
		CHK(wtz_launch<K_glist>(nwt, [=] WTZ_LAMBDA (uint64_t t){ wtz_task_glist((uint32_t)t, dn, d_list); }));
	}
	CHK(dev_d2h(n_list, d_list, 4));
	{
		const uint32_t nl = *n_list; const wtz_lgap_t *gp = d_gp; const uint32_t *lst = d_list + 1;
		CHK(sort_leftovers(d_list, nl, [&](uint64_t *d_k2){ return wtz_launch<K_misc>(nl, [=] WTZ_LAMBDA (uint64_t i){
			const wtz_lgap_t G = gp[lst[i]];
			const int32_t nc = G.dq < 2 * G.w + 1 ? G.dq : 2 * G.w + 1;
			unsigned long long wgt = (unsigned long long)(G.dt > 0 ? G.dt : 0) * (unsigned long long)((nc > 0 ? nc : 0) / 64 + 1);
			if(wgt > 0xFFFFFFFEull) wgt = 0xFFFFFFFEull;
			d_k2[i] = 0xFFFFFFFFull - wgt;
		}); }));
	}
	if(c->sw.profile) fprintf(stderr, "[lane-profile] %llu window slots, K-sw2 gaps by band class <=16 / <=32 / <=64 / <=104: %u / %u / %u / %u, %u left to the wavefront kernel\n",
		(unsigned long long)nwt, ccnt[0], ccnt[1], ccnt[2], ccnt[3], *n_list);
	return WTZ_OK;
}

static int run_winalign_chained(wtz_ctx *c, const wtz_env_t &V, const wtz_wintask_t *d_wt, const wtz_alnitem_t *d_items, uint32_t *d_list, uint64_t n, uint32_t *n_redone = NULL){
	if(n_redone) *n_redone = 0;
	if(n == 0) return WTZ_OK;
#ifdef WTZ_EMUL
	if(d_list) return wtz_launch_coop<K_winalign>(n, [=] WTZ_LAMBDA (uint64_t t){ wtz_task_winalign((uint32_t)t, V, d_wt, d_items, (uint32_t*)NULL, d_list); }, WTZ_WINALIGN_LDS_BYTES + WTZ_WINALIGN_QW_BYTES);
	return wtz_launch_coop<K_winalign>(n, [=] WTZ_LAMBDA (uint64_t t){ wtz_task_winalign((uint32_t)t, V, d_wt, d_items); }, WTZ_WINALIGN_LDS_BYTES + WTZ_WINALIGN_QW_BYTES);
#else
	uint32_t *d_defer = NULL, n_def = 0; CHK(dev_alloc((void**)&d_defer, ((size_t)n + 1) * 4)); CHK(dev_set(d_defer, 0, 4));
	if(d_list) CHK(wtz_launch_coop<K_winalign>(n, [=] WTZ_LAMBDA (uint64_t t){ wtz_task_winalign<false>((uint32_t)t, V, d_wt, d_items, d_defer, d_list); }, WTZ_WINALIGN_LDS_BYTES + WTZ_WINALIGN_QW_BYTES));
	else CHK(wtz_launch_coop<K_winalign>(n, [=] WTZ_LAMBDA (uint64_t t){ wtz_task_winalign<false>((uint32_t)t, V, d_wt, d_items, d_defer, NULL); }, WTZ_WINALIGN_LDS_BYTES + WTZ_WINALIGN_QW_BYTES));
	CHK(dev_d2h(&n_def, d_defer, 4));
	if(n_def) CHK(wtz_launch_coop<K_winalign_big>(n_def, [=] WTZ_LAMBDA (uint64_t t){ wtz_task_winalign<true>((uint32_t)t, V, d_wt, d_items, NULL, d_defer); }, WTZ_WINALIGN_LDS_BYTES + WTZ_WINALIGN_QW_BYTES));
	if(n_redone) *n_redone = n_def;
	return WTZ_OK;
#endif
}

static int compare_lane_with_chained(const wtz_reg_t *ra, const wtz_reg_t *rb, uint64_t nreg){
	unsigned int *d_bad = NULL; CHK(dev_alloc((void**)&d_bad, 16)); CHK(dev_set(d_bad, 0, 16));
	CHK(wtz_launch<K_misc>(nreg, [=] WTZ_LAMBDA (uint64_t i){
		const wtz_reg_t &a = ra[i], &b = rb[i];
		bool same = a.pass == 2 || b.pass == 2 || (a.x.score == b.x.score && a.x.tb == b.x.tb && a.x.te == b.x.te && a.x.qb == b.x.qb && a.x.qe == b.x.qe && a.x.aln == b.x.aln && a.x.mat == b.x.mat && a.x.mis == b.x.mis && a.x.ins == b.x.ins && a.x.del == b.x.del && a.pass == b.pass && a.cigar_len == b.cigar_len && (a.cells == b.cells || a.cells == 0 || b.cells == 0));
		if(same && a.pass != 2 && b.pass != 2) for(uint32_t k = 0; k < a.cigar_len; k++) if(a.cigar[k] != b.cigar[k]){ same = false; break; }
		if(!same){ const unsigned int z = WTZ_ATOMIC_INC32(&d_bad[0]); if(z == 0) d_bad[1] = (unsigned int)i; }
	}));
	unsigned int hb[4]; CHK(dev_d2h(hb, d_bad, 16));
	if(hb[0]){
		wtz_reg_t a, b; CHK(dev_d2h(&a, ra + hb[1], sizeof a)); CHK(dev_d2h(&b, rb + hb[1], sizeof b));
		return wtz_fail(WTZ_E_STATE, "K-sw1 lane pipeline differs from the chained kernel on %u of %llu windows; first: window slot %u chained/lane score %d/%d tb %d/%d te %d/%d qb %d/%d qe %d/%d aln %d/%d mat %d/%d mis %d/%d ins %d/%d del %d/%d cigar %u/%u pass %u/%u cells %llu/%llu",
			hb[0], (unsigned long long)nreg, hb[1], a.x.score, b.x.score, a.x.tb, b.x.tb, a.x.te, b.x.te, a.x.qb, b.x.qb, a.x.qe, b.x.qe, a.x.aln, b.x.aln, a.x.mat, b.x.mat, a.x.mis, b.x.mis, a.x.ins, b.x.ins, a.x.del, b.x.del, a.cigar_len, b.cigar_len, a.pass, b.pass, a.cells, b.cells);
	}
	return WTZ_OK;
}

static int run_gap_wave(wtz_ctx *c, const wtz_env_t &V, const wtz_wintask_t *d_wt, const wtz_alnitem_t *d_items, wtz_gapres_t *d_gaps, const uint32_t *d_glist, uint32_t n_glist, uint64_t nwt){
#ifdef WTZ_EMUL
	(void)c; (void)nwt;
	return wtz_launch_coop<K_gap>(n_glist, [=] WTZ_LAMBDA (uint64_t t){ wtz_task_gap((uint32_t)t, V, d_wt, d_items, d_gaps, (uint32_t*)NULL, (const uint32_t*)d_glist); }, WTZ_GAP_LDS_BYTES);
#else
	uint32_t *d_defer = NULL, n_def = 0; CHK(dev_alloc((void**)&d_defer, (size_t)(nwt + 1) * 4)); CHK(dev_set(d_defer, 0, 4));
	STAGE(c, "K_gap");
	CHK(wtz_launch_coop<K_gap>(n_glist, [=] WTZ_LAMBDA (uint64_t t){ wtz_task_gap((uint32_t)t, V, d_wt, d_items, d_gaps, d_defer, (const uint32_t*)d_glist, 0u); }, WTZ_GAP_LDS_BYTES));
	CHK(dev_d2h(&n_def, d_defer, 4));
	if(n_def) CHK(wtz_launch_coop<K_gap_wide>(n_def, [=] WTZ_LAMBDA (uint64_t t){ wtz_task_gap((uint32_t)t, V, d_wt, d_items, d_gaps, NULL, d_defer, (uint32_t)WTZ_GAP_WIDE_LDS_BYTES); }, WTZ_GAP_WIDE_LDS_BYTES));
	if(c->sw.profile){ CHK(dev_sync()); fprintf(stderr, "[gap-profile] %llu window slots, %u wide gaps redone with 72 KB of LDS\n", (unsigned long long)nwt, n_def); }
	return WTZ_OK;
#endif
}

#ifdef WTZ_EMUL
static int check_right_geometry(const int32_t *d_rgeo, const wtz_extjob_t *d_jr, const wtz_stitch_state_t *d_st, uint32_t m){
	for(uint32_t t = 0; t < m; t++){
		const wtz_extjob_t &jr = d_jr[t];
		const int32_t pq = d_rgeo[2 * (size_t)t], pt = d_rgeo[2 * (size_t)t + 1];
		if(jr.valid ? (pq != jr.qlen || pt != jr.tlen) : (pq >= 0 && !d_st[t].bad))
			return wtz_fail(WTZ_E_STATE, "stitch: predicted right extension of item %u (%d x %d) differs from the one K_stitch_mid asks for (valid %u: %d x %d)", t, pq, pt, jr.valid, jr.qlen, jr.tlen);
	}
	return WTZ_OK;
}
#endif

extern "C" int wtz_pairs_align(wtz_ctx_t *c, const uint32_t *pair_idx, const uint8_t *dir, uint32_t m, wtz_aln_result_t *out){
	if(!c || !c->have_pairs) return wtz_fail(WTZ_E_STATE, "wtz_pairs_align before wtz_pairs_seed");
	if(m == 0) return WTZ_OK;
	CTX_ENTER(c);
	if(!pair_idx || !dir || !out) return wtz_fail(WTZ_E_ARG, "null argument");
	c->n_items = 0; c->have_items = false;
	const bool prof_wall = c->sw.profile; double tw[6] = {0, 0, 0, 0, 0, 0}; double tw0 = prof_wall ? wtz_wall() : 0;
	auto lapw = [&](int k){ if(prof_wall){ const double t = wtz_wall(); tw[k] += t - tw0; tw0 = t; } };
	CHK(reserve_items(c, m));
	std::vector<wtz_alnitem_t> items(m); uint64_t nreg = 0;
	std::vector<uint32_t> h_q(c->n_pairs), h_c(c->n_pairs);
	CHK(dev_d2h(h_q.data(), c->d_qid, (size_t)c->n_pairs * 4)); CHK(dev_d2h(h_c.data(), c->d_cid, (size_t)c->n_pairs * 4));
	for(uint32_t i = 0; i < m; i++){
		if(pair_idx[i] >= c->n_pairs || dir[i] > 1) return wtz_fail(WTZ_E_ARG, "align item %u out of range", i);
		const wtz_pairres_t &r = c->h_pairres[pair_idx[i]];
		wtz_alnitem_t it; it.q = h_q[pair_idx[i]]; it.c = h_c[pair_idx[i]]; it.dir = dir[i];
		it.win = r.win[dir[i]]; it.anchors = r.anchors[dir[i]]; it.nwin = r.nwin[dir[i]]; it.regs = (wtz_reg_t*)(uintptr_t)nreg;
		nreg += it.nwin; items[i] = it;
	}
	const uint64_t nwt = (size_t)nreg;
	wtz_reg_t *d_regs = NULL; wtz_alnitem_t *d_items = NULL; wtz_wintask_t *d_wt = NULL;
	CHK(dev_alloc((void**)&d_regs, (size_t)(nreg + 1) * sizeof(wtz_reg_t)));
	for(uint32_t i = 0; i < m; i++) items[i].regs = d_regs + (uintptr_t)items[i].regs;
	CHK(dev_alloc((void**)&d_items, (size_t)m * sizeof(wtz_alnitem_t))); CHK(dev_h2d(d_items, items.data(), (size_t)m * sizeof(wtz_alnitem_t)));
	CHK(dev_alloc((void**)&d_wt, (size_t)(nreg + 1) * sizeof(wtz_wintask_t)));
	{ const wtz_alnitem_t *di = d_items; wtz_wintask_t *dw = d_wt; const wtz_reg_t *r0 = d_regs;
	  CHK(wtz_launch<K_misc>(m, [=] WTZ_LAMBDA (uint64_t i){ const wtz_alnitem_t &it = di[i]; wtz_wintask_t *w = dw + (it.regs - r0); for(uint32_t k = 0; k < it.nwin; k++){ w[k].item = (uint32_t)i; w[k].widx = k; } })); }
	const wtz_env_t V = ctx_env(c); wtz_alnres_dev_t *d_res = c->d_alnres;
	lapw(0);
	wtz_timer tm; tm.start();
	wtz_reg_t *d_regs_chk = NULL;
	if(c->sw.lane){
		uint32_t *d_fb = NULL, n_fb = 0;
		CHK(dev_alloc((void**)&d_fb, (nwt + 1) * 4));
		STAGE(c, "K-sw1 lane pipeline");
		CHK(run_winalign_lane(c, V, d_wt, nwt, d_items, d_fb, &n_fb));
		CHK(run_winalign_chained(c, V, d_wt, d_items, d_fb, n_fb));
		if(c->sw.lane == 2){ CHK(dev_sync()); CHK(dev_alloc((void**)&d_regs_chk, (size_t)(nreg + 1) * sizeof(wtz_reg_t))); CHK(dev_d2d(d_regs_chk, d_regs, (size_t)nreg * sizeof(wtz_reg_t))); }
	}
	if(c->sw.lane == 0 || c->sw.lane == 2){
		uint32_t n_redone = 0;
		STAGE(c, "K_winalign");
		CHK(run_winalign_chained(c, V, d_wt, d_items, NULL, nwt, &n_redone));
		if(c->sw.profile) fprintf(stderr, "[winalign-profile] %zu windows, %u redone by the full task\n", (size_t)nreg, n_redone);
	}
	CHK(dev_sync());
	if(d_regs_chk) CHK(compare_lane_with_chained(d_regs, d_regs_chk, nreg));
	c->cnt.ms_winalign += tm.stop(); c->cnt.n_winalign += (size_t)nreg;
	lapw(1);
	tm.start();
	wtz_stitch_state_t *d_st = NULL; wtz_extjob_t *d_jl = NULL, *d_jr = NULL; wtz_gapres_t *d_gaps = NULL; int32_t *d_rgeo = NULL;
	CHK(dev_alloc((void**)&d_st, (size_t)m * sizeof(wtz_stitch_state_t)));
	CHK(dev_alloc((void**)&d_jl, (size_t)m * sizeof(wtz_extjob_t))); CHK(dev_alloc((void**)&d_jr, (size_t)m * sizeof(wtz_extjob_t)));
	CHK(dev_alloc((void**)&d_gaps, (size_t)(nreg + 1) * sizeof(wtz_gapres_t)));
#ifndef WTZ_EMUL
	const bool fused = c->sw.ext_fused && c->sw.sw_mode == 0, gap_side = c->sw.gap_side != 0;
	if(fused) CHK(dev_alloc((void**)&d_rgeo, (size_t)m * 8));
#else
	const bool fused = false, gap_side = false;
	CHK(dev_alloc((void**)&d_rgeo, (size_t)m * 8));
#endif
	STAGE(c, "K_stitch_left");
	CHK(wtz_launch_wave<K_stitch_left>(m, [=] WTZ_LAMBDA (uint64_t t){ wtz_task_stitch_left((uint32_t)t, V, d_items, d_st, d_jl, d_rgeo); }));
	uint32_t *d_glist = NULL, n_glist = (uint32_t)nwt;
	wtz_timer tgap; tgap.start();
	if(c->sw.gap_lane){
		CHK(dev_alloc((void**)&d_glist, (size_t)(nwt + 1) * 4));
		STAGE(c, "K-sw2 lane pipeline");
		CHK(run_gap_lane(c, V, d_wt, nwt, d_items, d_gaps, d_glist, &n_glist));
	}
#ifndef WTZ_EMUL
	if(gap_side){ HIPCHK(hipEventRecord(c->ev_gap_fork, g_stream)); HIPCHK(hipStreamWaitEvent(c->stream_gap, c->ev_gap_fork, 0)); }
	{ wtz_stream_scope on_gap_stream(gap_side ? c->stream_gap : g_stream); CHK(run_gap_wave(c, V, d_wt, d_items, d_gaps, d_glist, n_glist, nwt)); }
	if(gap_side) HIPCHK(hipEventRecord(c->ev_gap_join, c->stream_gap));
#else
	CHK(run_gap_wave(c, V, d_wt, d_items, d_gaps, d_glist, n_glist, nwt));
#endif
	if(!gap_side) tgap.lap();
#ifndef WTZ_EMUL
	if(fused){
		if(gap_side) HIPCHK(hipStreamWaitEvent(g_stream, c->ev_gap_join, 0));
		STAGE(c, "extjobs left + join + right on one wavefront"); CHK(run_stitch_fused(c, V, d_items, d_st, d_jl, d_jr, d_gaps, d_rgeo, m));
	}
#endif
	STAGE(c, "extjobs left");
	CHK(run_extjobs(c, V, d_jl, m, fused));
#ifndef WTZ_EMUL
	if(gap_side) HIPCHK(hipStreamWaitEvent(g_stream, c->ev_gap_join, 0));
#endif
	if(!gap_side) c->cnt.ms_gap += tgap.read();
	STAGE(c, "K_stitch_mid");
	CHK(wtz_launch_coop<K_stitch_mid>(m, [=] WTZ_LAMBDA (uint64_t t){ wtz_task_stitch_mid((uint32_t)t, V, d_items, d_st, d_jl, d_jr, d_gaps); }));
	STAGE(c, "extjobs right");
#ifdef WTZ_EMUL
	CHK(check_right_geometry(d_rgeo, d_jr, d_st, m));
#endif
	CHK(run_extjobs(c, V, d_jr, m, fused));
	STAGE(c, "K_stitch_fin");
	CHK(wtz_launch_coop<K_stitch_fin>(m, [=] WTZ_LAMBDA (uint64_t t){ wtz_task_stitch_fin((uint32_t)t, V, d_items, d_st, d_jl, d_jr, d_res); }));
	if(c->P.refine) STAGE(c, "K_refine");
	if(c->P.refine) CHK(wtz_launch_coop<K_refine>(m, [=] WTZ_LAMBDA (uint64_t t){ wtz_task_refine((uint32_t)t, V, d_items, d_res); }, WTZ_REFINE_LDS_BYTES));
	CHK(dev_sync());
	c->cnt.ms_stitch += tm.stop(); c->cnt.n_stitch += m;
	lapw(2);
	c->h_alnres.resize(m); c->n_items = m; c->have_items = true;
	CHK(dev_d2h(c->h_alnres.data(), c->d_alnres, (size_t)m * sizeof(wtz_alnres_dev_t)));
	CHK(pool_check(c, "wtz_pairs_align"));
	uint64_t coff = 0, toff = 0;
	for(uint32_t i = 0; i < m; i++){
		const wtz_alnres_dev_t &r = c->h_alnres[i];
		if(r.bad) return wtz_fail(WTZ_E_POOL, "wtz_pairs_align: item %u ran out of scratch", i);
		wtz_aln_result_t o; memset(&o, 0, sizeof o);
		o.score = r.x.score; o.tb = r.x.tb; o.te = r.x.te; o.qb = r.x.qb; o.qe = r.x.qe; o.aln = r.x.aln; o.mat = r.x.mat; o.mis = r.x.mis; o.ins = r.x.ins; o.del = r.x.del;
		o.n_regs = r.n_regs; o.cigar_len = r.cigar_len; o.cigar_off = coff; coff += r.cigar_len; o.text_len = r.text_len; o.text_off = toff; toff += r.text_len;
		c->cnt.cells_shift += r.cells_shift; c->cnt.cells_fixed += r.cells_fixed; c->cnt.cells_global += r.cells_global;
		out[i] = o;
	}
	lapw(3);
	if(prof_wall) fprintf(stderr, "[align-profile] %u items: host wall ms prep %.2f winalign %.2f stitch %.2f results %.2f\n", m, tw[0] * 1e3, tw[1] * 1e3, tw[2] * 1e3, tw[3] * 1e3);
	return WTZ_OK;
}
```

smartdenovo_amd/csrc/wtz_lib_fetch.h:

```cpp
extern "C" int wtz_fetch_cigars(wtz_ctx_t *c, uint32_t *dst, uint64_t n_ops){
	if(!c || !c->have_items) return wtz_fail(WTZ_E_STATE, "wtz_fetch_cigars before wtz_pairs_align");
	CTX_ENTER(c);
	uint64_t tot = 0; for(uint32_t i = 0; i < c->n_items; i++) tot += c->h_alnres[i].cigar_len;
	if(tot != n_ops) return wtz_fail(WTZ_E_ARG, "wtz_fetch_cigars: expected room for %llu ops, got %llu", (unsigned long long)tot, (unsigned long long)n_ops);
	if(tot == 0) return WTZ_OK;
	if(!dst) return wtz_fail(WTZ_E_ARG, "null output");
	std::vector<uint64_t> off((size_t)c->n_items + 1);
	uint64_t o = 0; for(uint32_t i = 0; i < c->n_items; i++){ off[i] = o; o += c->h_alnres[i].cigar_len; } off[c->n_items] = o;
	uint64_t *d_off = NULL; uint32_t *d_c = NULL;
	CHK(dev_alloc((void**)&d_off, off.size() * 8)); CHK(dev_h2d(d_off, off.data(), off.size() * 8));
	CHK(dev_alloc((void**)&d_c, (size_t)tot * 4));
	const wtz_alnres_dev_t *dr = c->d_alnres;
	CHK(wtz_launch<K_pack_cigars>(c->n_items, [=] WTZ_LAMBDA (uint64_t t){ const wtz_alnres_dev_t &r = dr[t]; for(uint32_t k = 0; k < r.cigar_len; k++) d_c[d_off[t] + k] = r.cigar[k]; }));
	CHK(dev_sync());
	CHK(dev_d2h(dst, d_c, (size_t)tot * 4));
	return WTZ_OK;
}

static int render_cigar_text(wtz_ctx_t *c, uint64_t n_bytes, char **d_text_out, bool wait = true){
	uint64_t tot = 0; for(uint32_t i = 0; i < c->n_items; i++) tot += c->h_alnres[i].text_len;
	if(tot != n_bytes) return wtz_fail(WTZ_E_ARG, "CIGAR text: expected room for %llu bytes, got %llu", (unsigned long long)tot, (unsigned long long)n_bytes);
	*d_text_out = NULL;
	if(tot == 0) return WTZ_OK;
#ifndef WTZ_EMUL
	{
		const uint64_t b = c->text_begun.load();
		if(b > c->text_known_done.load()){ HIPCHK(hipEventSynchronize(c->ev_text_done[(b - 1) & 1])); c->text_known_done.store(b); }
	}
#endif
	if(tot + 16 > c->cap_text){
		(void)dev_sync(); dev_free_persist(c->d_text); c->d_text = NULL; c->cap_text = 0;
		const size_t cap = (size_t)(tot + tot / 4 + 4096);
		CHK(dev_alloc_persist((void**)&c->d_text, cap)); c->cap_text = cap;
	}
	std::vector<uint64_t> off((size_t)c->n_items + 1);
	uint64_t o = 0; for(uint32_t i = 0; i < c->n_items; i++){ off[i] = o; o += c->h_alnres[i].text_len; } off[c->n_items] = o;
	uint64_t *d_off = NULL; char *d_t = c->d_text;
	CHK(dev_alloc((void**)&d_off, off.size() * 8)); CHK(dev_h2d(d_off, off.data(), off.size() * 8));
	const wtz_alnres_dev_t *dr = c->d_alnres;
	STAGE(c, "K_cigar_text");
	CHK(wtz_launch_coop<K_cigar_text>(c->n_items, [=] WTZ_LAMBDA (uint64_t t){ const wtz_alnres_dev_t &r = dr[t]; if(r.text_len) wtz_cigar_text_write_coop(r.cigar, r.cigar_len, d_t + d_off[t]); }));
	if(wait) CHK(dev_sync());
	*d_text_out = d_t;
	return WTZ_OK;
}
extern "C" int wtz_fetch_cigar_text(wtz_ctx_t *c, char *dst, uint64_t n_bytes){
	if(!c || !c->have_items) return wtz_fail(WTZ_E_STATE, "wtz_fetch_cigar_text before wtz_pairs_align");
	CTX_ENTER(c);
	char *d_t = NULL;
	CHK(render_cigar_text(c, n_bytes, &d_t));
	if(n_bytes == 0) return WTZ_OK;
	if(!dst) return wtz_fail(WTZ_E_ARG, "null output");
	CHK(dev_d2h(dst, d_t, (size_t)n_bytes));
	return WTZ_OK;
}
extern "C" int wtz_fetch_cigar_text_begin(wtz_ctx_t *c, char *dst, uint64_t n_bytes){
	if(!c || !c->have_items) return wtz_fail(WTZ_E_STATE, "wtz_fetch_cigar_text_begin before wtz_pairs_align");
	CTX_ENTER(c);
#ifdef WTZ_EMUL
	char *d_t = NULL; CHK(render_cigar_text(c, n_bytes, &d_t));
	if(n_bytes && !dst) return wtz_fail(WTZ_E_ARG, "null output");
	if(n_bytes) memcpy(dst, d_t, (size_t)n_bytes);
	return WTZ_OK;
#else
	if(!c->stream_copy){
		if(hipStreamCreateWithFlags(&c->stream_copy, hipStreamNonBlocking) != hipSuccess || hipEventCreateWithFlags(&c->ev_text_ready, hipEventDisableTiming) != hipSuccess
			|| hipEventCreateWithFlags(&c->ev_text_done[0], hipEventDisableTiming) != hipSuccess || hipEventCreateWithFlags(&c->ev_text_done[1], hipEventDisableTiming) != hipSuccess) return wtz_fail(WTZ_E_HIP, "hipStreamCreate / hipEventCreate failed");
	}
	char *d_t = NULL;
	CHK(render_cigar_text(c, n_bytes, &d_t, false));
	if(n_bytes == 0) return WTZ_OK;
// ... 27 lines not shown
```

smartdenovo_amd/csrc/wtz_lib_pairs.h:

```cpp
#ifndef WTZ_PAIR_DM_LDS_TIER2
#define WTZ_PAIR_DM_LDS_TIER2 49152u
#endif
#ifndef WTZ_PAIR_DM_LDS_TIER3
#define WTZ_PAIR_DM_LDS_TIER3 20480u
#endif
#ifndef WTZ_PAIR_DM_LDS_TIER4
#define WTZ_PAIR_DM_LDS_TIER4 36864u
#endif
extern "C" int wtz_batch_begin(wtz_ctx_t *c){
	if(!c) return wtz_fail(WTZ_E_ARG, "null context");
	CTX_ENTER(c);
	free_batch(c);
	return pool_reset(c);
}

#if defined(WTZ_DEBUG_CRUMBS) && !defined(WTZ_EMUL)
#include <signal.h>
#include <unistd.h>
static unsigned int *g_crumbs = NULL; static uint32_t g_crumbs_n = 0; static const uint32_t *g_crumbs_q = NULL, *g_crumbs_c = NULL;
static void wtz_crumbs_dump(int sig){
	unsigned hist[256]; memset(hist, 0, sizeof hist); unsigned shown = 0;
	for(uint32_t i = 0; i < g_crumbs_n; i++) hist[g_crumbs[i] & 0xFF]++;
	fprintf(stderr, "[crumbs] signal %d, %u pairs; tasks per last point:", sig, g_crumbs_n);
	for(int k = 0; k < 256; k++) if(hist[k]) fprintf(stderr, " %d:%u", k, hist[k]);
	fprintf(stderr, "\n");
	for(uint32_t i = 0; i < g_crumbs_n && shown < 16; i++) if((g_crumbs[i] & 0xFF) != 0xFF && (g_crumbs[i] & 0xFF) != 0){ fprintf(stderr, "[crumbs]   pair %u (q %u, c %u): point %u, hits %u\n", i, g_crumbs_q[i], g_crumbs_c[i], g_crumbs[i] & 0xFF, g_crumbs[i] >> 8); shown++; }
	fflush(stderr); _exit(86);
}
#endif

extern "C" int wtz_pairs_seed(wtz_ctx_t *c, const uint32_t *qid, const uint32_t *cid, uint32_t n, wtz_pair_summary_t *out){
	if(!c || !c->zs[0].have || (n && (!qid || !cid || !out))) return wtz_fail(WTZ_E_ARG, "z-index not built / null argument");
	CTX_ENTER(c);
	free_batch(c);
	CHK(pool_reset(c));
	if(n == 0){ c->n_pairs = 0; c->h_pairres.clear(); c->have_pairs = true; return WTZ_OK; }
	for(uint32_t i = 0; i < n; i++) if(qid[i] >= c->n_reads || cid[i] >= c->n_reads) return wtz_fail(WTZ_E_ARG, "pair %u: read id out of range", i);
	CHK(reserve_pairs(c, n));
	CHK(dev_h2d(c->d_qid, qid, (size_t)n * 4)); CHK(dev_h2d(c->d_cid, cid, (size_t)n * 4));
	const wtz_env_t V = ctx_env(c); const uint32_t *dq = c->d_qid, *dc = c->d_cid; wtz_pairres_t *dr = c->d_pairres;
	wtz_timer tm; tm.start();
	wtz_timer t1; t1.start();
	STAGE(c, "K_pair");
#if defined(WTZ_DEBUG_CRUMBS) && !defined(WTZ_EMUL)
	unsigned int *h_crumbs = NULL;
	if(getenv("WTZ_DEBUG_CRUMBS")){
		HIPCHK(hipHostMalloc((void**)&h_crumbs, (size_t)n * 4, hipHostMallocCoherent | hipHostMallocMapped)); memset(h_crumbs, 0, (size_t)n * 4);
		unsigned int *dptr = NULL; HIPCHK(hipHostGetDevicePointer((void**)&dptr, h_crumbs, 0));
		HIPCHK(hipMemcpyToSymbol(HIP_SYMBOL(wtz_crumbs), &dptr, sizeof dptr));
		g_crumbs = h_crumbs; g_crumbs_n = n; g_crumbs_q = qid; g_crumbs_c = cid;
		signal(SIGABRT, wtz_crumbs_dump); signal(SIGPIPE, wtz_crumbs_dump); signal(SIGSEGV, wtz_crumbs_dump); signal(SIGBUS, wtz_crumbs_dump); signal(SIGTERM, wtz_crumbs_dump);
	}
#endif
	const uint32_t xg = c->sw.xcd_group;
	uint32_t nh = 0; const uint32_t *d_ord = NULL;
#ifndef WTZ_EMUL
	if(c->sw.heavy_first >= 0 ? c->sw.heavy_first != 0 : c->P.dot_matrix != 0){
		nh = n / 32u;
		if(nh >= 8u){
			std::vector<uint64_t> key(n); std::vector<uint32_t> ord(n), hv(n);
			for(uint32_t i = 0; i < n; i++){ key[i] = (uint64_t)c->h_rdlen[qid[i]] * c->h_rdlen[cid[i]]; hv[i] = i; }
			std::nth_element(hv.begin(), hv.begin() + nh, hv.end(), [&](uint32_t a, uint32_t b){ return key[a] != key[b] ? key[a] > key[b] : a < b; });
			std::sort(hv.begin(), hv.begin() + nh, [&](uint32_t a, uint32_t b){ return key[a] != key[b] ? key[a] > key[b] : a < b; });
			std::vector<uint8_t> heavy(n, 0);
			for(uint32_t k = 0; k < nh; k++){ ord[k] = hv[k]; heavy[hv[k]] = 1; }
			uint32_t w = nh; for(uint32_t i = 0; i < n; i++) if(!heavy[i]) ord[w++] = i;
			uint32_t *dd = NULL; CHK(dev_alloc((void**)&dd, (size_t)n * 4)); CHK(dev_h2d(dd, ord.data(), (size_t)n * 4)); d_ord = dd;
		} else nh = 0;
	}
#endif
	const uint64_t n64 = n - nh; const uint64_t nh64 = nh;
#ifdef WTZ_EMUL
	CHK(wtz_launch_coop<K_pair>(n, [=] WTZ_LAMBDA (uint64_t b){ (void)xg; (void)n64; (void)nh64; (void)d_ord; wtz_task_pair<-1>((uint32_t)b, V, dq, dc, dr); }, c->P.dot_matrix ? WTZ_PAIR_DM_LDS_BYTES : WTZ_PAIR_LDS_BYTES));
#else
	if(c->P.dot_matrix){
		CHK(wtz_launch_coop<K_pair_dm>(n, [=] WTZ_LAMBDA (uint64_t b){
			uint64_t t = b;
			if(b >= nh64){ const uint64_t b2 = b - nh64; t = b2; if(xg){ const uint64_t per = 8ull * xg, full = n64 / per * per; if(b2 < full){ const uint64_t r = b2 % per; t = b2 - r + (r & 7u) * xg + (r >> 3); } } t += nh64; }
			if(d_ord) t = d_ord[t];
			wtz_task_pair<1>((uint32_t)t, V, dq, dc, dr); }, WTZ_PAIR_DM_LDS_BYTES));
	} else {
		CHK(wtz_launch_coop<K_pair>(n, [=] WTZ_LAMBDA (uint64_t b){
			uint64_t t = b;
			if(b >= nh64){ const uint64_t b2 = b - nh64; t = b2; if(xg){ const uint64_t per = 8ull * xg, full = n64 / per * per; if(b2 < full){ const uint64_t r = b2 % per; t = b2 - r + (r & 7u) * xg + (r >> 3); } } t += nh64; }
			if(d_ord) t = d_ord[t];
#ifdef WTZ_PAIR_TWO_LAUNCH
			wtz_task_pair<0, false>((uint32_t)t, V, dq, dc, dr); }, WTZ_PAIR_LDS_BYTES));
#else
			wtz_task_pair<0, true>((uint32_t)t, V, dq, dc, dr); }, WTZ_PAIR_LDS_BYTES));
#endif
	}
#endif
#if defined(WTZ_DEBUG_CRUMBS) && !defined(WTZ_EMUL)
	if(h_crumbs){
		const double t0 = wtz_wall(); const double limit = atof(getenv("WTZ_DEBUG_CRUMBS")) > 1 ? atof(getenv("WTZ_DEBUG_CRUMBS")) : 20.0;
		while(hipStreamQuery(g_stream) == hipErrorNotReady && wtz_wall() - t0 < limit){ struct timespec ts = {0, 50000000}; nanosleep(&ts, NULL); }
		if(hipStreamQuery(g_stream) == hipErrorNotReady){
			unsigned hist[256]; memset(hist, 0, sizeof hist); unsigned shown = 0;
			for(uint32_t i = 0; i < n; i++) hist[h_crumbs[i] & 0xFF]++;
			fprintf(stderr, "[crumbs] K_pair still running after %.0f s, %u pairs; tasks per last point:", limit, n);
			for(int k = 0; k < 256; k++) if(hist[k]) fprintf(stderr, " %d:%u", k, hist[k]);
			fprintf(stderr, "\n");
			for(uint32_t i = 0; i < n && shown < 12; i++) if((h_crumbs[i] & 0xFF) != 0xFF && (h_crumbs[i] & 0xFF) != 0){ fprintf(stderr, "[crumbs]   pair %u (q %u, c %u): point %u, hits %u\n", i, qid[i], cid[i], h_crumbs[i] & 0xFF, h_crumbs[i] >> 8); shown++; }
			fflush(stderr); _exit(86);
		}
	}
#endif
	CHK(dev_sync());
	{ const double ms1 = t1.stop(); if(c->sw.profile) fprintf(stderr, "[pair-profile] K_pair first launch: %u pairs, %.1f ms\n", n, ms1); }
	c->n_pairs = n; c->h_pairres.resize(n); c->have_pairs = true;
	CHK(dev_d2h(c->h_pairres.data(), c->d_pairres, (size_t)n * sizeof(wtz_pairres_t)));
#ifndef WTZ_EMUL
	if(!c->P.dot_matrix){
		std::vector<uint32_t> list;
		for(uint32_t i = 0; i < n; i++) if(c->h_pairres[i].gate && c->h_pairres[i].dm_dir == WTZ_PAIR_NEEDS_ZBIG && !c->h_pairres[i].bad) list.push_back(i);
		if(!list.empty()){
			uint32_t *d_list = NULL; CHK(dev_alloc((void**)&d_list, list.size() * 4)); CHK(dev_h2d(d_list, list.data(), list.size() * 4));
			wtz_timer tt; tt.start();
			STAGE(c, "K_pair_zbig");
			CHK(wtz_launch_coop<K_pair_zbig>(list.size(), [=] WTZ_LAMBDA (uint64_t t){ wtz_task_pair<0, true>(d_list[t], V, dq, dc, dr); }, WTZ_PAIR_LDS_BYTES));
			CHK(dev_sync());
			const double ms_t = tt.stop();
			CHK(dev_d2h(c->h_pairres.data(), c->d_pairres, (size_t)n * sizeof(wtz_pairres_t)));
			if(c->sw.profile) fprintf(stderr, "[pair-profile] zmo pairs with ranges beyond the LDS slice: %zu of %u, %.1f ms\n", list.size(), n, ms_t);
		}
	}
#endif
	if(c->P.dot_matrix){
		uint32_t tiers[3] = { WTZ_PAIR_DM_LDS_TIER2, WTZ_PAIR_DM_LDS_TIER3, WTZ_PAIR_DM_LDS_TIER4 };
		if(getenv("WTZ_DM_TIER3_KB")) tiers[1] = (uint32_t)atoi(getenv("WTZ_DM_TIER3_KB")) << 10;
		if(getenv("WTZ_DM_TIER4_KB")) tiers[2] = (uint32_t)atoi(getenv("WTZ_DM_TIER4_KB")) << 10;
		for(int tier = c->sw.dm_first_big ? 2 : 0; tier < 3; tier++){
			std::vector<uint32_t> list;
			for(uint32_t i = 0; i < n; i++) if(c->h_pairres[i].gate && c->h_pairres[i].dm_dir == -2 && !c->h_pairres[i].bad) list.push_back(i);
			if(list.empty()) break;
			uint32_t *d_list = NULL; CHK(dev_alloc((void**)&d_list, list.size() * 4)); CHK(dev_h2d(d_list, list.data(), list.size() * 4));
			const uint32_t lb = tiers[tier]; const bool last = (tier == 2), big = (tier >= 1);
			wtz_timer tt; tt.start();
			STAGE(c, "K_pair_big");
			CHK(wtz_launch_coop<K_pair_big>(list.size(), [=] WTZ_LAMBDA (uint64_t t){ wtz_task_pair_dm_big((uint32_t)t, V, d_list, dq, dc, dr, lb, last, big); }, lb));
			CHK(dev_sync());
			const double ms_t = tt.stop();
			CHK(dev_d2h(c->h_pairres.data(), c->d_pairres, (size_t)n * sizeof(wtz_pairres_t)));
			if(c->sw.profile) fprintf(stderr, "[pair-profile] dmo tier %d (%u KB LDS): %zu pairs, %.1f ms\n", tier + 2, lb >> 10, list.size(), ms_t);
		}
	}
	c->cnt.ms_pairs += tm.stop(); c->cnt.n_pairs += n;
	for(uint32_t i = 0; i < n; i++) c->cnt.bytes_zmer_algo += (uint64_t)c->h_rdlen[cid[i]] / 4 + 16ull * c->h_pairres[i].n_hits;
	CHK(pool_check(c, "wtz_pairs_seed"));
	if(c->sw.profile){
		uint64_t sum[4] = {0, 0, 0, 0}; uint32_t mx[4] = {0, 0, 0, 0}, arg = 0;
		for(uint32_t i = 0; i < n; i++){ for(int k = 0; k < 4; k++){ sum[k] += c->h_pairres[i].tick[k]; if(c->h_pairres[i].tick[k] > mx[k]){ mx[k] = c->h_pairres[i].tick[k]; if(k == 3) arg = i; } } }
		fprintf(stderr, "[pair-profile] n=%u kticks sum match/sort/win/total %llu/%llu/%llu/%llu max %u/%u/%u/%u; slowest pair: hits %u (its match/sort/win %u/%u/%u)\n", n,
			(unsigned long long)sum[0], (unsigned long long)sum[1], (unsigned long long)sum[2], (unsigned long long)sum[3], mx[0], mx[1], mx[2], mx[3],
			c->h_pairres[arg].n_hits, c->h_pairres[arg].tick[0], c->h_pairres[arg].tick[1], c->h_pairres[arg].tick[2]);
	}
	for(uint32_t i = 0; i < n; i++){
		const wtz_pairres_t &r = c->h_pairres[i];
		if(r.bad) return wtz_fail(WTZ_E_POOL, "wtz_pairs_seed: pair %u ran out of scratch", i);
		wtz_pair_summary_t s; memset(&s, 0, sizeof s);
		s.n_hits = r.n_hits; s.gate = r.gate; s.ovl[0] = r.ovl[0]; s.ovl[1] = r.ovl[1]; s.nwin[0] = r.nwin[0]; s.nwin[1] = r.nwin[1];
		s.dm_score = r.dm_score; s.dm_qb = r.dm_qb; s.dm_qe = r.dm_qe; s.dm_tb = r.dm_tb; s.dm_te = r.dm_te; s.dm_dir = r.dm_dir;
		out[i] = s;
	}
	return WTZ_OK;
}

extern "C" int wtz_pairs_windows(wtz_ctx_t *c, wtz_winbox_t *wins, uint64_t n_wins){
	if(!c || !c->have_pairs) return wtz_fail(WTZ_E_STATE, "wtz_pairs_windows before wtz_pairs_seed");
	CTX_ENTER(c);
	uint64_t tot = 0; for(uint32_t i = 0; i < c->n_pairs; i++) tot += c->h_pairres[i].nwin[0] + c->h_pairres[i].nwin[1];
	if(tot != n_wins) return wtz_fail(WTZ_E_ARG, "wtz_pairs_windows: expected room for %llu windows, got %llu", (unsigned long long)tot, (unsigned long long)n_wins);
	if(tot == 0) return WTZ_OK;
	if(!wins) return wtz_fail(WTZ_E_ARG, "null output");
	std::vector<uint64_t> off((size_t)c->n_pairs * 2 + 1);
	uint64_t o = 0; for(uint32_t i = 0; i < c->n_pairs; i++) for(int d = 0; d < 2; d++){ off[(size_t)i * 2 + d] = o; o += c->h_pairres[i].nwin[d]; }
	off[(size_t)c->n_pairs * 2] = o;
	uint64_t *d_off = NULL; wtz_winbox_t *d_w = NULL;
	CHK(dev_alloc((void**)&d_off, off.size() * 8)); CHK(dev_h2d(d_off, off.data(), off.size() * 8));
	CHK(dev_alloc((void**)&d_w, (size_t)tot * sizeof(wtz_winbox_t)));
	const wtz_pairres_t *dr = c->d_pairres;
	CHK(wtz_launch<K_pack_windows>((uint64_t)c->n_pairs * 2, [=] WTZ_LAMBDA (uint64_t t){
		const wtz_pairres_t &r = dr[t >> 1]; const uint32_t d = (uint32_t)(t & 1);
		for(uint32_t k = 0; k < r.nwin[d]; k++){ wtz_winbox_t b; b.beg[0] = r.win[d][k].beg[0]; b.beg[1] = r.win[d][k].beg[1]; b.end[0] = r.win[d][k].end[0]; b.end[1] = r.win[d][k].end[1]; d_w[d_off[t] + k] = b; }
	}));
	CHK(dev_sync());
	CHK(dev_d2h(wins, d_w, (size_t)tot * sizeof(wtz_winbox_t)));
	return WTZ_OK;
}
```

smartdenovo_amd/hipabi.py:

```python
from __future__ import annotations

import ctypes as C
import os

import numpy as np

_HERE = os.path.dirname(os.path.abspath(__file__))
LIB_PATH = os.path.join(_HERE, "libwtzmo_hip.so")

SYMBOLS = [
    "wtz_last_error", "wtz_device_count", "wtz_device_memory", "wtz_ctx_create", "wtz_ctx_destroy", "wtz_ctx_clone", "wtz_upload_reads",
    "wtz_index_build", "wtz_zindex_build", "wtz_candidates", "wtz_candidates_begin", "wtz_candidates_end", "wtz_batch_begin", "wtz_pairs_seed",
    "wtz_pairs_windows", "wtz_pairs_align", "wtz_fetch_cigars", "wtz_fetch_cigar_text", "wtz_fetch_cigar_text_begin", "wtz_fetch_cigar_text_end", "wtz_cigar_text_device", "wtz_host_alloc", "wtz_host_free", "wtz_get_counters", "wtz_reset_counters",
    "wtz_test_dp", "wtz_extend_batch", "wtz_local_batch", "wtz_kext_batch", "wtz_align_batch", "wtz_global_batch", "wtz_alignx_batch", "wtz_pwtext_batch", "wtz_pool_info", "wtz_pool_failure_kind",
    "wtz_index_count", "wtz_index_counts_fetch", "wtz_index_finish", "wtz_candidate_groups_begin", "wtz_candidate_groups_end", "wtz_candidate_groups_fetch", "wtz_cand_tail_host", "wtz_zindex_build_subset", "wtz_zindex_build_queries", "wtz_upload_reads_ascii", "wtz_fetch_read_bits", "wtz_append_revcomp_views",
]


class Params(C.Structure):
    _fields_ = [(n, C.c_uint32) for n in ("ksize", "zsize", "hk", "hz", "ksave", "kovl", "ncand", "nbest",
                                          "kwin", "kstep", "ztot", "zovl", "max_kmer_freq", "max_zmer_freq", "max_kmer_var")] + \
               [("win_rep_norm", C.c_float), ("win_rep_cutoff", C.c_float)] + \
               [(n, C.c_int32) for n in ("w", "ew", "W", "M", "X", "O", "E", "T", "min_score")] + [("min_id", C.c_float)] + \
               [(n, C.c_int32) for n in ("dot_matrix", "xvar", "yvar", "min_block_len", "max_overhang")] + \
# ... 25 lines not shown
                       ("text_len", "<u4"), ("pad", "<u4"), ("text_off", "<u8")])


DP_PROBLEM = np.dtype([("q_read", "<u4"), ("t_read", "<u4"), ("q_rev", "<u4"), ("t_rev", "<u4"), ("q_from", "<i4"), ("t_from", "<i4"),
                       ("q_strand", "<i4"), ("t_strand", "<i4"), ("q_len", "<i4"), ("t_len", "<i4"), ("init_score", "<i4"), ("W", "<i4")])
DP_RESULT = np.dtype([("score", "<i4"), ("tb", "<i4"), ("te", "<i4"), ("qb", "<i4"), ("qe", "<i4"), ("aln", "<i4"), ("mat", "<i4"),
                      ("mis", "<i4"), ("ins", "<i4"), ("del", "<i4"), ("cigar_len", "<u4"), ("form_used", "<u4"), ("cigar_off", "<u8"), ("cells", "<u8")])
DP_SHIFT, DP_FIXED, DP_GLOBAL = 0, 1, 2
LOCAL_RESULT = np.dtype([("score", "<i4"), ("te", "<i4"), ("qe", "<i4"), ("tb", "<i4"), ("qb", "<i4"), ("form_used", "<u4"), ("cells", "<u8")])
LOCAL_MAXLEN = 65535
KEXT_RESULT = np.dtype([("score", "<i4"), ("qle", "<i4"), ("tle", "<i4"), ("gtle", "<i4"), ("gscore", "<i4"), ("max_off", "<i4"),
                        ("form_used", "<u4"), ("rows", "<u4"), ("cells", "<u8")])
KEXT_MAXW = 1023
KEXT_MAXLEN = 0xFFFFF
ALIGN_RESULT = np.dtype([(n, "<i4") for n in ("found", "score", "tb", "te", "qb", "qe", "local_score", "local_tb", "local_te", "local_qb", "local_qe")])
GLOBAL_RESULT = np.dtype([(n, "<i4") for n in ("score", "aln", "mat", "mis", "ins", "del")] + [("cigar_len", "<u4"), ("form_used", "<u4"), ("cigar_off", "<u8"), ("cells", "<u8")])
GLOB_MAXSLOTS = 2047
ALIGNX_RESULT = np.dtype([(n, "<i4") for n in ("found", "score", "tb", "te", "qb", "qe", "aln", "mat", "mis", "ins", "del", "band")] +
                         [("form_used", "<u4"), ("cigar_len", "<u4"), ("cigar_off", "<u8")])
PWTEXT_IN = np.dtype([("qb", "<i4"), ("tb", "<i4"), ("cigar_len", "<u4"), ("pad", "<u4"), ("cigar_off", "<u8")])
PWTEXT_RESULT = np.dtype([("text_off", "<u8"), ("cols", "<u4"), ("pad", "<u4")])


class Counters(C.Structure):
    _fields_ = [(n, C.c_double) for n in ("ms_index", "ms_zindex", "ms_candidates", "ms_pairs", "ms_winalign", "ms_stitch")] + \
               [(n, C.c_uint64) for n in ("n_candidates_q", "n_pairs", "n_winalign", "n_stitch", "cells_shift", "cells_fixed",
                                          "cells_global", "bytes_seed_algo", "pool_peak")] + \
               [("ms_ext", C.c_double), ("n_extjobs", C.c_uint64), ("ms_gap", C.c_double), ("bytes_zmer_algo", C.c_uint64),
                ("ms_ingest", C.c_double), ("bytes_ingest_algo", C.c_uint64),
                ("ms_local", C.c_double), ("n_local", C.c_uint64), ("cells_local", C.c_uint64),
                ("ms_kext", C.c_double), ("n_kext", C.c_uint64), ("cells_kext", C.c_uint64),
                ("ms_kglob", C.c_double), ("n_kglob", C.c_uint64), ("cells_kglob", C.c_uint64),
                ("ticks_kglob_dp", C.c_uint64), ("ticks_kglob_tb", C.c_uint64),
                ("ms_pwtext", C.c_double), ("n_pwtext", C.c_uint64), ("bytes_pwtext", C.c_uint64)]


def load(path: str | None = None) -> C.CDLL:
    path = path or LIB_PATH
    if not os.path.exists(path):
        raise RuntimeError("libwtzmo_hip.so not found at %s: build it with `python __graft_entry__.py build` "
                           "(hipcc --offload-arch=gfx950). There is no CPU fallback for the hot path." % path)
    lib = C.CDLL(path)
    lib.wtz_last_error.restype = C.c_char_p
    lib.wtz_ctx_create.argtypes = [C.c_int, C.POINTER(Params), C.c_uint64, C.POINTER(C.c_void_p)]
    lib.wtz_ctx_destroy.argtypes = [C.c_void_p]
    lib.wtz_ctx_destroy.restype = None
    lib.wtz_upload_reads.argtypes = [C.c_void_p, C.c_void_p, C.c_uint64, C.c_void_p, C.c_void_p, C.c_uint32]
    lib.wtz_index_build.argtypes = [C.c_void_p, C.c_uint32, C.c_uint32, C.POINTER(C.c_uint32), C.POINTER(IndexStats)]
    lib.wtz_zindex_build.argtypes = [C.c_void_p]
    lib.wtz_candidates.argtypes = [C.c_void_p, C.c_void_p, C.c_uint32, C.c_void_p, C.c_void_p]
    lib.wtz_batch_begin.argtypes = [C.c_void_p]
    lib.wtz_pairs_seed.argtypes = [C.c_void_p, C.c_void_p, C.c_void_p, C.c_uint32, C.c_void_p]
    lib.wtz_pairs_windows.argtypes = [C.c_void_p, C.c_void_p, C.c_uint64]
    lib.wtz_pairs_align.argtypes = [C.c_void_p, C.c_void_p, C.c_void_p, C.c_uint32, C.c_void_p]
    lib.wtz_fetch_cigars.argtypes = [C.c_void_p, C.c_void_p, C.c_uint64]
    lib.wtz_get_counters.argtypes = [C.c_void_p, C.POINTER(Counters)]
    lib.wtz_reset_counters.argtypes = [C.c_void_p]
    lib.wtz_test_dp.argtypes = [C.c_void_p, C.c_int32, C.c_int32, C.c_void_p, C.c_uint32, C.c_void_p, C.c_void_p, C.c_uint64]
    return lib


def check_symbols(path: str | None = None) -> None:
    lib = C.CDLL(path or LIB_PATH)
    missing = [s for s in SYMBOLS if not hasattr(lib, s)]
    if missing:
        raise RuntimeError("libwtzmo_hip.so does not export: " + ", ".join(missing))

# ... 176 lines not shown
```

Measured before the change: 10.65.

## Cut host-device stream syncs with pinned staging buffers, mailbox, and device-side pool init

Replaces the synchronous host-to-device and device-to-host copies in the pair/window/pool paths with async copies into persistent page-locked staging buffers. The pool-head reads now ride on existing syncs through a pinned mailbox, and pool initialisation moves to a device kernel instead of an upload. Redundant dev_sync calls, such as the one after the radix sort and before packing windows, are removed. Counters for syncs and copies are added for visibility. The goal is to cut per-batch host round-trip latency, at the cost of extra bookkeeping to avoid reusing staging buffers while uploads are still pending.

```diff
diff --git a/include/wtzmo_hip.h b/include/wtzmo_hip.h
--- a/include/wtzmo_hip.h
+++ b/include/wtzmo_hip.h
@@ -77,6 +77,8 @@
 	uint64_t ticks_kglob_dp, ticks_kglob_tb;
 	double   ms_pwtext;
 	uint64_t n_pwtext, bytes_pwtext;
+	uint64_t n_stream_syncs;
+	uint64_t n_copies_h2d, n_copies_d2h, bytes_d2h;
 } wtz_counters_t;
 
 const char *wtz_last_error(void);
diff --git a/smartdenovo_amd/csrc/host/wtzmo_main.c b/smartdenovo_amd/csrc/host/wtzmo_main.c
--- a/smartdenovo_amd/csrc/host/wtzmo_main.c
+++ b/smartdenovo_amd/csrc/host/wtzmo_main.c
@@ -367,6 +367,7 @@
 		if(w){ E->step.extra_ms[0] += cw.ms_candidates; E->step.extra_ms[1] += cw.ms_pairs; E->step.extra_ms[2] += cw.ms_winalign; E->step.extra_ms[3] += cw.ms_stitch; E->step.extra_ms[4] += cw.ms_ext; E->step.extra_ms[5] += cw.ms_gap; }
 		E->step.extra_u64[0] += cw.cells_shift; E->step.extra_u64[1] += cw.cells_fixed; E->step.extra_u64[2] += cw.cells_global; E->step.extra_u64[3] += cw.bytes_seed_algo; E->step.extra_u64[4] += cw.n_extjobs; E->step.extra_u64[6] += cw.bytes_zmer_algo;
 		if(cw.pool_peak > E->step.extra_u64[5]) E->step.extra_u64[5] = cw.pool_peak;
+		E->step.extra_u64[7] += cw.n_stream_syncs; E->step.extra_u64[8] += cw.n_copies_h2d; E->step.extra_u64[9] += cw.n_copies_d2h; E->step.extra_u64[10] += cw.bytes_d2h;
 		if(w) wtz_ctx_destroy(ctx); else wtz_reset_counters(ctx);
 }
 static batch_t *batches_create(eng_t *E, uint32_t nw_run, int nalt, uint64_t pool_bytes){
@@ -433,6 +434,7 @@
 	cn.ms_candidates += E->step.extra_ms[0]; cn.ms_pairs += E->step.extra_ms[1]; cn.ms_winalign += E->step.extra_ms[2]; cn.ms_stitch += E->step.extra_ms[3]; cn.ms_ext += E->step.extra_ms[4]; cn.ms_gap += E->step.extra_ms[5];
 	cn.cells_shift += E->step.extra_u64[0]; cn.cells_fixed += E->step.extra_u64[1]; cn.cells_global += E->step.extra_u64[2]; cn.bytes_seed_algo += E->step.extra_u64[3]; cn.n_extjobs += E->step.extra_u64[4]; cn.bytes_zmer_algo += E->step.extra_u64[6];
 	if(E->step.extra_u64[5] > cn.pool_peak) cn.pool_peak = E->step.extra_u64[5];
+	cn.n_stream_syncs += E->step.extra_u64[7]; cn.n_copies_h2d += E->step.extra_u64[8]; cn.n_copies_d2h += E->step.extra_u64[9]; cn.bytes_d2h += E->step.extra_u64[10];
 	memset(E->step.extra_ms, 0, sizeof E->step.extra_ms); memset(E->step.extra_u64, 0, sizeof E->step.extra_u64);
 	fprintf(stderr, "[wtzmo-mi355x] %llu records, %llu pairs aligned, %llu pair-bp, %.3f s (index %.3f s)\n", (unsigned long long)E->step.nrec, (unsigned long long)E->step.n_pairs, (unsigned long long)E->step.pair_bp, t_step, t_index);
 	fprintf(stderr, "[wtzmo-mi355x] host seconds: in GPU-stage calls %.3f, commit %.3f, per-batch z-index %.3f; writer thread: formatting %.3f, write %.3f; waiting for it: %.3f before buffer reuse, %.3f at the end\n", E->step.t_gpu, E->step.t_commit, E->step.t_zbatch, g_ow.t_format, g_ow.t_write, E->step.t_io[0], E->step.t_io[1]);
@@ -445,6 +447,8 @@
 			(unsigned long long)E->step.n_batches, (unsigned long long)E->step.n_ranges, E->step.rows_all ? 1u : E->n_workers, (unsigned long long)E->step.used_queries, (unsigned long long)E->step.spec_queries, (unsigned long long)E->step.used_pairs, (unsigned long long)E->step.spec_pairs, (unsigned long long)E->step.used_items, (unsigned long long)E->step.spec_items);
 	fprintf(stderr, "[wtzmo-mi355x] kernel ms: index %.1f zindex %.1f candidates %.1f pairs %.1f winalign %.1f stitch %.1f (K-sw3 wave %.1f, K-sw2 gaps %.1f); cells shift %llu fixed %llu global %llu; pool peak %.2f GB\n",
 		cn.ms_index, cn.ms_zindex, cn.ms_candidates, cn.ms_pairs, cn.ms_winalign, cn.ms_stitch, cn.ms_ext, cn.ms_gap, (unsigned long long)cn.cells_shift, (unsigned long long)cn.cells_fixed, (unsigned long long)cn.cells_global, cn.pool_peak / 1073741824.0);
+	fprintf(stderr, "[wtzmo-mi355x] host <-> device: n_stream_syncs %llu n_copies_h2d %llu n_copies_d2h %llu bytes_d2h %llu (index builds included; %llu ranges)\n",
+		(unsigned long long)cn.n_stream_syncs, (unsigned long long)cn.n_copies_h2d, (unsigned long long)cn.n_copies_d2h, (unsigned long long)cn.bytes_d2h, (unsigned long long)E->step.n_ranges);
 	if(statsf){ FILE *sf = fopen(statsf, "a"); if(sf){ fprintf(sf, "%llu\t%llu\t%.6f\t%.6f\t%.3f\t%.3f\t%.3f\t%.3f\t%.3f\t%.3f\t%llu\t%llu\t%llu\t%llu\t%llu\t%.3f\t%llu\t%llu\t%llu\t%.3f\t%llu\t%llu\t%llu\t%.4f\t%llu\t%.4f\t%.4f\t%.4f\t%.4f\t%.4f\t%.4f\t%llu\t%llu\n", (unsigned long long)E->step.n_pairs, (unsigned long long)E->step.pair_bp, t_step, t_index,
 			cn.ms_index, cn.ms_zindex, cn.ms_candidates, cn.ms_pairs, cn.ms_winalign, cn.ms_stitch, (unsigned long long)cn.cells_shift, (unsigned long long)cn.cells_fixed, (unsigned long long)cn.cells_global, (unsigned long long)cn.bytes_seed_algo, (unsigned long long)E->step.nrec,
 			cn.ms_ext, (unsigned long long)cn.n_extjobs, (unsigned long long)E->step.used_queries, (unsigned long long)cn.pool_peak, cn.ms_gap, (unsigned long long)E->step.n_ranges, (unsigned long long)E->step.n_split, (unsigned long long)cn.bytes_zmer_algo, E->ing_ms, (unsigned long long)E->ing_bytes,
diff --git a/smartdenovo_amd/csrc/host/wtzmo_types.h b/smartdenovo_amd/csrc/host/wtzmo_types.h
--- a/smartdenovo_amd/csrc/host/wtzmo_types.h
+++ b/smartdenovo_amd/csrc/host/wtzmo_types.h
@@ -66,7 +66,7 @@
 		uint64_t n_masked;
 		double cand_bpq;
 		double last_mask_rate;
-		double extra_ms[6]; uint64_t extra_u64[7];
+		double extra_ms[6]; uint64_t extra_u64[11];
 	} step;
 } eng_t;
 typedef void (*wtz_dist_bcast_fn)(void *buf, uint64_t nbytes);
diff --git a/smartdenovo_amd/csrc/wtz_ctx.h b/smartdenovo_amd/csrc/wtz_ctx.h
--- a/smartdenovo_amd/csrc/wtz_ctx.h
+++ b/smartdenovo_amd/csrc/wtz_ctx.h
@@ -60,8 +60,10 @@
 	uint64_t *cq_gptr = NULL; uint32_t cq_gcap = 0; bool cq_groups = false; std::vector<uint32_t> cq_ng;
 	uint32_t idx_beg = 0, idx_end = 0; bool idx_len_sorted = false;
 	wtz_pool_t *dpool = NULL; uint8_t *pool_base = NULL; uint64_t pool_bytes = 0, main_bytes = 0;
-	uint32_t *d_qid = NULL, *d_cid = NULL; wtz_pairres_t *d_pairres = NULL; uint32_t n_pairs = 0; std::vector<wtz_pairres_t> h_pairres;
-	wtz_alnres_dev_t *d_alnres = NULL; uint32_t n_items = 0; std::vector<wtz_alnres_dev_t> h_alnres;
+	uint32_t *d_qid = NULL, *d_cid = NULL; wtz_pairres_t *d_pairres = NULL; uint32_t n_pairs = 0;
+	wtz_alnres_dev_t *d_alnres = NULL; uint32_t n_items = 0;
+	wtz_staging stg; wtz_mailbox mb;
+	wtz_pairres_t *h_pairres = NULL; wtz_alnres_dev_t *h_alnres = NULL; const uint32_t *h_qid = NULL, *h_cid = NULL;
 	char *d_text = NULL; size_t cap_text = 0;
 #ifndef WTZ_EMUL
 	hipStream_t stream_copy = 0; hipEvent_t ev_text_ready = 0, ev_text_done[2] = {0, 0}; std::atomic<uint64_t> text_begun{0}, text_known_done{0}, text_ended{0};
@@ -79,9 +81,9 @@
 };
 
 #ifndef WTZ_EMUL
-#define CTX_ENTER(c) (void)hipSetDevice((c)->device); g_stream = (c)->stream; wtz_arena_scope arena_scope_(&(c)->arena)
+#define CTX_ENTER(c) (void)hipSetDevice((c)->device); g_stream = (c)->stream; wtz_arena_scope arena_scope_(&(c)->arena); wtz_cnt_scope cnt_scope_(&(c)->cnt, &(c)->stg.up_pending)
 #else
-#define CTX_ENTER(c) wtz_arena_scope arena_scope_(&(c)->arena)
+#define CTX_ENTER(c) wtz_arena_scope arena_scope_(&(c)->arena); wtz_cnt_scope cnt_scope_(&(c)->cnt, &(c)->stg.up_pending)
 #endif
 
 #define STAGE(c, name) do { if((c)->sw.trace){ (void)dev_sync(); fprintf(stderr, "[stage] %s\n", name); fflush(stderr); } } while(0)
@@ -89,18 +91,26 @@
 static wtz_reads_t ctx_reads(const wtz_ctx *c){ wtz_reads_t R; R.bits = c->bits; R.rdoff = c->rdoff; R.rdlen = c->rdlen; R.n_reads = c->n_reads; return R; }
 static wtz_env_t ctx_env(const wtz_ctx *c){ wtz_env_t V; V.R = ctx_reads(c); V.Z = c->zs[0].Z; V.ZQ = c->zs[1].have ? c->zs[1].Z : c->zs[0].Z; V.P = c->dP; V.pool = c->dpool; V.dm_first_big = (uint32_t)c->sw.dm_first_big; return V; }
 
-static int tpool_reset(wtz_ctx *c){
-	wtz_pool_t p; wtz_pool_init(&p, c->pool_base + c->main_bytes, c->pool_bytes - c->main_bytes, c->sw.tfail_at);
-	return dev_h2d(c->dpool + 1, &p, sizeof p);
-}
+static int pool_init_dev(wtz_pool_t *dp, uint8_t *base, uint64_t cap, unsigned fail_at){
+	wtz_pool_t h; wtz_pool_init(&h, base, cap, fail_at);
+	const unsigned long long slab = h.slab, cap_ = cap;
+	return wtz_launch<K_misc>((uint64_t)WTZ_POOL_NSHARD * 16, [=] WTZ_LAMBDA (uint64_t i){
+		if(i == 0){ dp->base = base; dp->cap = cap_; dp->used = 0; dp->overflow = 0; dp->fail_at = fail_at; dp->nalloc = 0; dp->slab = slab; }
+		dp->shard[i] = (i & 15u) ? 0ull : slab;
+	});
+}
+static int tpool_reset(wtz_ctx *c){ return pool_init_dev(c->dpool + 1, c->pool_base + c->main_bytes, c->pool_bytes - c->main_bytes, c->sw.tfail_at); }
 static int pool_reset(wtz_ctx *c){
-	wtz_pool_t p; wtz_pool_init(&p, c->pool_base, c->main_bytes, c->sw.fail_at);
-	CHK(dev_h2d(c->dpool, &p, sizeof p));
+	CHK(pool_init_dev(c->dpool, c->pool_base, c->main_bytes, c->sw.fail_at));
 	c->tpool_peak_call = 0;
 	return tpool_reset(c);
 }
-static int tpool_check(wtz_ctx *c, const char *stage){
-	wtz_pool_t p; CHK(dev_d2h(&p, c->dpool + 1, sizeof p));
+#define WTZ_POOL_HEAD_BYTES offsetof(wtz_pool_t, shard)
+static int pool_head_post(wtz_ctx *c, int which){ return dev_d2h_async(c->mb.h + WTZ_MBOX_WORDS + 8 * which, c->dpool + which, WTZ_POOL_HEAD_BYTES); }
+static void pool_head(const wtz_ctx *c, int which, wtz_pool_t *p){ memset(p, 0, WTZ_POOL_HEAD_BYTES); memcpy(p, c->mb.h + WTZ_MBOX_WORDS + 8 * which, WTZ_POOL_HEAD_BYTES); }
+static int tpool_check(wtz_ctx *c, const char *stage, bool posted = false){
+	if(!posted){ CHK(pool_head_post(c, 1)); CHK(dev_sync()); }
+	wtz_pool_t p; pool_head(c, 1, &p);
 	const uint64_t u = p.used > p.cap ? p.cap : p.used;
 	c->tpool_last_used = u;
 	if(u > c->tpool_peak_call) c->tpool_peak_call = u;
@@ -110,8 +120,9 @@
 		stage, (unsigned long long)p.used, (unsigned long long)p.cap);
 	return WTZ_OK;
 }
-static int pool_check(wtz_ctx *c, const char *stage){
-	wtz_pool_t p; CHK(dev_d2h(&p, c->dpool, sizeof p));
+static int pool_check(wtz_ctx *c, const char *stage, bool posted = false){
+	if(!posted){ CHK(pool_head_post(c, 0)); CHK(dev_sync()); }
+	wtz_pool_t p; pool_head(c, 0, &p);
 	const uint64_t u = (p.used > p.cap ? p.cap : p.used);
 	c->main_used_call = u;
 	if(u + c->tpool_peak_call > c->cnt.pool_peak) c->cnt.pool_peak = u + c->tpool_peak_call;
@@ -121,6 +132,12 @@
 		stage, (unsigned long long)p.used, (unsigned long long)p.cap);
 	return WTZ_OK;
 }
+static int fetch_small(wtz_ctx *c, const void *d, size_t bytes, const unsigned long long **w){
+	c->mb.h[0] = c->mb.h[1] = c->mb.h[2] = 0;
+	CHK(dev_d2h_async(c->mb.h, d, bytes)); *w = c->mb.h;
+	return dev_sync();
+}
+static int fetch_u32(wtz_ctx *c, const uint32_t *d, uint32_t *out){ const unsigned long long *w = NULL; CHK(fetch_small(c, d, 4, &w)); *out = (uint32_t)w[0]; return WTZ_OK; }
 extern "C" int wtz_device_count(void){
 #ifndef WTZ_EMUL
 	int n = 0; if(hipGetDeviceCount(&n) != hipSuccess) return 0; return n;
@@ -175,7 +192,7 @@
 #endif
 	int rc;
 	if((rc = dev_alloc_persist((void**)&c->dP, sizeof(wtz_params_t))) || (rc = dev_h2d(c->dP, &c->P, sizeof(wtz_params_t))) ||
-	   (rc = dev_alloc_persist((void**)&c->dpool, 2 * sizeof(wtz_pool_t)))){
+	   (rc = dev_alloc_persist((void**)&c->dpool, 2 * sizeof(wtz_pool_t))) || (rc = mbox_create(&c->mb))){
 		wtz_ctx_destroy(c); return rc;
 	}
 	for(;;){
@@ -192,7 +209,7 @@
 		rc = dev_alloc_persist((void**)&c->pool_base, c->pool_bytes);
 		break;
 	}
-	if(rc || (rc = pool_reset(c))){
+	if(rc || (rc = pool_reset(c)) || (rc = dev_sync())){
 		wtz_ctx_destroy(c); return rc;
 	}
 	*out = c;
@@ -234,7 +251,7 @@
 		z->zoff = NULL; memset(&z->Z, 0, sizeof z->Z); z->have = false; z->sub = false; z->sub_cap = 0; z->n_z = 0;
 	}
 }
-static void free_batch(wtz_ctx *c){ c->n_pairs = 0; c->n_items = 0; c->have_pairs = false; c->have_items = false; }
+static void free_batch(wtz_ctx *c){ c->n_pairs = 0; c->n_items = 0; c->have_pairs = false; c->have_items = false; c->h_pairres = NULL; c->h_alnres = NULL; c->h_qid = c->h_cid = NULL; }
 static void free_batch_storage(wtz_ctx *c){
 	dev_free_persist(c->d_qid); dev_free_persist(c->d_cid); dev_free_persist(c->d_pairres); dev_free_persist(c->d_alnres);
 	c->d_qid = c->d_cid = NULL; c->d_pairres = NULL; c->d_alnres = NULL; c->cap_pairs = c->cap_items = 0; free_batch(c);
@@ -262,6 +279,7 @@
 	{ CTX_ENTER(c); (void)dev_sync(); }
 	free_batch_storage(c); free_kindex(c); if(!c->shares_indexes) kflush(c); free_zindex(c);
 	dev_free_persist(c->d_text);
+	stage_free(&c->stg); mbox_free(&c->mb);
 	dev_free_persist(c->cq_q); dev_free_persist(c->cq_nc); dev_free_persist(c->cq_cand); dev_free_persist(c->cq_bytes); dev_free_persist(c->cq_thr); dev_free_persist(c->cq_gptr);
 	free_pending_index(c);
 #ifndef WTZ_EMUL
diff --git a/smartdenovo_amd/csrc/wtz_dev.h b/smartdenovo_amd/csrc/wtz_dev.h
--- a/smartdenovo_amd/csrc/wtz_dev.h
+++ b/smartdenovo_amd/csrc/wtz_dev.h
@@ -6,6 +6,15 @@
 }
 #include <chrono>
 static double wtz_wall(){ return std::chrono::duration<double>(std::chrono::steady_clock::now().time_since_epoch()).count(); }
+static thread_local wtz_counters_t *g_cnt = NULL;
+static thread_local uint32_t *g_up = NULL;
+struct wtz_cnt_scope { wtz_counters_t *prev; uint32_t *prev_up;
+	wtz_cnt_scope(wtz_counters_t *k, uint32_t *up) : prev(g_cnt), prev_up(g_up) { g_cnt = k; g_up = up; }
+	~wtz_cnt_scope(){ g_cnt = prev; g_up = prev_up; }
+	wtz_cnt_scope(const wtz_cnt_scope&) = delete; wtz_cnt_scope &operator=(const wtz_cnt_scope&) = delete; };
+static inline void cnt_sync(){ if(g_cnt) g_cnt->n_stream_syncs++; if(g_up) *g_up = 0; }
+static inline void cnt_h2d(){ if(g_cnt) g_cnt->n_copies_h2d++; }
+static inline void cnt_d2h(size_t n){ if(g_cnt){ g_cnt->n_copies_d2h++; g_cnt->bytes_d2h += n; } }
 #ifndef WTZ_EMUL
 #include <hip/hip_runtime.h>
 #include <rocprim/rocprim.hpp>
@@ -27,9 +36,9 @@
 #define HIPCHK(call) do { hipError_t e_ = (call); if(e_ != hipSuccess) return wtz_fail(WTZ_E_HIP, "%s failed: %s (%s:%d)", #call, hipGetErrorString(e_), __FILE__, __LINE__); } while(0)
 
 #define WTZ_LAUNCH(kernel, blocks, threads, lds_bytes, stream, ...) do { hipLaunchKernelGGL(kernel, dim3(blocks), dim3(threads), lds_bytes, stream, __VA_ARGS__); HIPCHK(hipGetLastError()); } while(0)
-struct wtz_stream_scope { hipStream_t prev;
-	wtz_stream_scope(hipStream_t st) : prev(g_stream) { g_stream = st; }
-	~wtz_stream_scope(){ g_stream = prev; }
+struct wtz_stream_scope { hipStream_t prev; uint32_t *prev_up;
+	wtz_stream_scope(hipStream_t st) : prev(g_stream), prev_up(g_up) { if(st != g_stream) g_up = NULL; g_stream = st; }
+	~wtz_stream_scope(){ g_stream = prev; g_up = prev_up; }
 	wtz_stream_scope(const wtz_stream_scope&) = delete; wtz_stream_scope &operator=(const wtz_stream_scope&) = delete; };
 
 template<typename TAG, typename F> __global__ void __launch_bounds__(64) wtz_kernel_tasks(uint64_t n, F f){
@@ -142,11 +151,13 @@
 	HIPCHK(hipMalloc(p, n ? n : 16)); return WTZ_OK;
 }
 static void dev_free_persist(void *p){ if(p) (void)hipFree(p); }
-static int dev_h2d(void *d, const void *h, size_t n){ if(n){ HIPCHK(hipMemcpyAsync(d, h, n, hipMemcpyHostToDevice, g_stream)); HIPCHK(hipStreamSynchronize(g_stream)); } return WTZ_OK; }
-static int dev_d2h(void *h, const void *d, size_t n){ if(n){ HIPCHK(hipMemcpyAsync(h, d, n, hipMemcpyDeviceToHost, g_stream)); HIPCHK(hipStreamSynchronize(g_stream)); } return WTZ_OK; }
+static int dev_h2d(void *d, const void *h, size_t n){ if(n){ cnt_h2d(); cnt_sync(); HIPCHK(hipMemcpyAsync(d, h, n, hipMemcpyHostToDevice, g_stream)); HIPCHK(hipStreamSynchronize(g_stream)); } return WTZ_OK; }
+static int dev_d2h(void *h, const void *d, size_t n){ if(n){ cnt_d2h(n); cnt_sync(); HIPCHK(hipMemcpyAsync(h, d, n, hipMemcpyDeviceToHost, g_stream)); HIPCHK(hipStreamSynchronize(g_stream)); } return WTZ_OK; }
+static int dev_h2d_async(void *d, const void *h, size_t n){ if(n){ cnt_h2d(); HIPCHK(hipMemcpyAsync(d, h, n, hipMemcpyHostToDevice, g_stream)); } return WTZ_OK; }
+static int dev_d2h_async(void *h, const void *d, size_t n){ if(n){ cnt_d2h(n); HIPCHK(hipMemcpyAsync(h, d, n, hipMemcpyDeviceToHost, g_stream)); } return WTZ_OK; }
 static int dev_set(void *d, int v, size_t n){ if(n) HIPCHK(hipMemsetAsync(d, v, n, g_stream)); return WTZ_OK; }
 static int dev_d2d(void *d, const void *s, size_t n){ if(n) HIPCHK(hipMemcpyAsync(d, s, n, hipMemcpyDeviceToDevice, g_stream)); return WTZ_OK; }
-static int dev_sync(){ HIPCHK(hipStreamSynchronize(g_stream)); return WTZ_OK; }
+static int dev_sync(){ cnt_sync(); HIPCHK(hipStreamSynchronize(g_stream)); return WTZ_OK; }
 
 struct wtz_timer { hipEvent_t a, b; bool ok;
 	wtz_timer(){ ok = hipEventCreate(&a) == hipSuccess && hipEventCreate(&b) == hipSuccess; }
@@ -165,8 +176,7 @@
 	hipError_t e = rocprim::radix_sort_pairs(tmp, tmp_bytes, kb, vb, (size_t)n, 0u, end_bit, g_stream);
 	if(e == hipSuccess && (rc = dev_alloc(&tmp, tmp_bytes)) == WTZ_OK){
 		e = rocprim::radix_sort_pairs(tmp, tmp_bytes, kb, vb, (size_t)n, 0u, end_bit, g_stream);
-		if(e == hipSuccess) e = hipStreamSynchronize(g_stream);
-		if(e == hipSuccess && kb.current() != keys){ e = hipMemcpyAsync(keys, kb.current(), n * 8, hipMemcpyDeviceToDevice, g_stream); if(e == hipSuccess) e = hipMemcpyAsync(vals, vb.current(), n * 4, hipMemcpyDeviceToDevice, g_stream); if(e == hipSuccess) e = hipStreamSynchronize(g_stream); }
+		if(e == hipSuccess && kb.current() != keys){ e = hipMemcpyAsync(keys, kb.current(), n * 8, hipMemcpyDeviceToDevice, g_stream); if(e == hipSuccess) e = hipMemcpyAsync(vals, vb.current(), n * 4, hipMemcpyDeviceToDevice, g_stream); }
 	}
 	if(e != hipSuccess) return wtz_fail(WTZ_E_HIP, "radix_sort_pairs failed: %s", hipGetErrorString(e));
 	return rc;
@@ -178,7 +188,6 @@
 	if(e != hipSuccess) return wtz_fail(WTZ_E_HIP, "exclusive_scan failed: %s", hipGetErrorString(e));
 	CHK(dev_alloc(&tmp, tmp_bytes));
 	e = rocprim::exclusive_scan(tmp, tmp_bytes, in, out, 0u, (size_t)n, rocprim::plus<uint32_t>(), g_stream);
-	if(e == hipSuccess) e = hipStreamSynchronize(g_stream);
 	if(e != hipSuccess) return wtz_fail(WTZ_E_HIP, "exclusive_scan failed: %s", hipGetErrorString(e));
 	return WTZ_OK;
 }
@@ -199,11 +208,13 @@
 struct wtz_arena_scope { wtz_arena *a, *prev; size_t mark;
 	wtz_arena_scope(wtz_arena *ar) : a(ar), prev(g_arena), mark(ar ? ar->blocks.size() : 0) { g_arena = ar; }
 	~wtz_arena_scope(){ g_arena = prev; if(!a) return; while(a->blocks.size() > mark){ free(a->blocks.back()); a->blocks.pop_back(); } } };
-static int dev_h2d(void *d, const void *h, size_t n){ if(n) memcpy(d, h, n); return WTZ_OK; }
-static int dev_d2h(void *h, const void *d, size_t n){ if(n) memcpy(h, d, n); return WTZ_OK; }
+static int dev_h2d(void *d, const void *h, size_t n){ if(n){ cnt_h2d(); cnt_sync(); memcpy(d, h, n); } return WTZ_OK; }
+static int dev_d2h(void *h, const void *d, size_t n){ if(n){ cnt_d2h(n); cnt_sync(); memcpy(h, d, n); } return WTZ_OK; }
+static int dev_h2d_async(void *d, const void *h, size_t n){ if(n){ cnt_h2d(); memcpy(d, h, n); } return WTZ_OK; }
+static int dev_d2h_async(void *h, const void *d, size_t n){ if(n){ cnt_d2h(n); memcpy(h, d, n); } return WTZ_OK; }
 static int dev_set(void *d, int v, size_t n){ if(n) memset(d, v, n); return WTZ_OK; }
 static int dev_d2d(void *d, const void *s, size_t n){ if(n) memcpy(d, s, n); return WTZ_OK; }
-static int dev_sync(){ return WTZ_OK; }
+static int dev_sync(){ cnt_sync(); return WTZ_OK; }
 #include <time.h>
 struct wtz_timer { struct timespec t0; void start(){ clock_gettime(CLOCK_MONOTONIC, &t0); }
 	double stop(){ struct timespec t1; clock_gettime(CLOCK_MONOTONIC, &t1); return 1e3 * (double)(t1.tv_sec - t0.tv_sec) + 1e-6 * (double)(t1.tv_nsec - t0.tv_nsec); }
diff --git a/smartdenovo_amd/csrc/wtz_lib.cpp b/smartdenovo_amd/csrc/wtz_lib.cpp
--- a/smartdenovo_amd/csrc/wtz_lib.cpp
+++ b/smartdenovo_amd/csrc/wtz_lib.cpp
@@ -1,6 +1,7 @@
 #include <stdio.h>
 #include <stdlib.h>
 #include <stdarg.h>
+#include <stddef.h>
 #include <vector>
 #include <atomic>
 #include <algorithm>
@@ -63,6 +64,7 @@
 struct K_glob_scalar;
 
 #include "wtz_dev.h"
+#include "wtz_stage.h"
 #include "wtz_ctx.h"
 #include "wtz_lib_index.h"
 #include "wtz_lib_pairs.h"
diff --git a/smartdenovo_amd/csrc/wtz_lib_align.h b/smartdenovo_amd/csrc/wtz_lib_align.h
--- a/smartdenovo_amd/csrc/wtz_lib_align.h
+++ b/smartdenovo_amd/csrc/wtz_lib_align.h
@@ -64,7 +64,8 @@
 		}));
 	}
 	CHK(dev_sort_pairs_u64_u32(d_k, d_order, m, 33));
-	unsigned long long h_acc[3] = {0, 0, 0}; CHK(dev_d2h(h_acc, d_acc, 24));
+	unsigned long long h_acc[3] = {0, 0, 0};
+	{ const unsigned long long *w = NULL; CHK(fetch_small(c, d_acc, 24, &w)); h_acc[0] = w[0]; h_acc[1] = w[1]; h_acc[2] = w[2]; }
 	const uint64_t acc = h_acc[0]; const unsigned long long ext_sum = h_acc[1];
 	const uint64_t budget = (c->pool_bytes - c->main_bytes) / 16 * 15;
 	uint32_t ng = 1; while(ng < 4 && (double)acc * c->ext_use_ratio / ng > (double)budget) ng++;
@@ -75,6 +76,7 @@
 		if(mg == 0) continue;
 		CHK(tpool_reset(c));
 		wtz_timer te; te.start();
+		bool head_posted = false;
 		if(c->sw.ext_pk){
 			uint32_t n_fr = ng == 1 ? (uint32_t)h_acc[2] : 0u;
 			if(n_fr > mg) n_fr = mg;
@@ -89,13 +91,14 @@
 				WTZ_LAUNCH((wtz_kernel_stitch_ext_pk<1032>), n_pk, 64, WTZ_PK_LDS_BYTES(1032), g_stream, V, d_items, d_st, d_jl, d_jr, d_gaps, (const uint32_t*)d_order, n_pk, ng, g, d_open);
 			}
 			if(n_fr) HIPCHK(hipStreamWaitEvent(g_stream, c->ev_side_join, 0));
-			uint32_t n_open = 0; CHK(dev_d2h(&n_open, d_open, 4));
+			uint32_t n_open = 0;
+			{ const unsigned long long *w = NULL; c->mb.h[0] = 0; CHK(dev_d2h_async(c->mb.h, d_open, 4)); CHK(pool_head_post(c, 1)); CHK(dev_sync()); w = c->mb.h; n_open = (uint32_t)w[0]; head_posted = true; }
 			c->ext_open_total += n_open; c->ext_fr_total += n_fr;
-			if(n_open){ WTZ_LAUNCH((wtz_kernel_stitch_ext_fr<1032>), n_open, 64, WTZ_WAVE_LDS_BYTES, g_stream, V, d_items, d_st, d_jl, d_jr, d_gaps, (const uint32_t*)d_open + 1, n_open, 1u, 0u); }
+			if(n_open){ head_posted = false; WTZ_LAUNCH((wtz_kernel_stitch_ext_fr<1032>), n_open, 64, WTZ_WAVE_LDS_BYTES, g_stream, V, d_items, d_st, d_jl, d_jr, d_gaps, (const uint32_t*)d_open + 1, n_open, 1u, 0u); }
 		} else WTZ_LAUNCH((wtz_kernel_stitch_ext_fr<1032>), mg, 64, WTZ_WAVE_LDS_BYTES, g_stream, V, d_items, d_st, d_jl, d_jr, d_gaps, (const uint32_t*)d_order, mg, ng, g);
 		ms_l += te.stop();
 		{
-			const int rc_t = tpool_check(c, "K-sw3 extension jobs (both ends on one wavefront)");
+			const int rc_t = tpool_check(c, "K-sw3 extension jobs (both ends on one wavefront)", head_posted);
 			if(rc_t != WTZ_OK){
 				c->ext_use_ratio = c->ext_use_ratio * 2.0 > 1.0 ? 1.0 : c->ext_use_ratio * 2.0;
 				return rc_t;
@@ -221,20 +224,24 @@
 #else
 #define WTZ_HOST_WAVE 64u
 #endif
+static int pool_letter(wtz_ctx *c, uint32_t n, uint32_t ptr0, uint32_t n_ptr, const char *what, const unsigned long long **w){
+	CHK(mbox_read(&c->mb, n, w));
+	for(uint32_t k = ptr0; k < ptr0 + n_ptr; k++) if((*w)[k] == 0){ c->last_pool_fail = 1; return wtz_fail(WTZ_E_POOL, "device scratch pool exhausted (%s)", what); }
+	return WTZ_OK;
+}
 static int pool_alloc_host(wtz_ctx *c, int which, size_t bytes, void **out){
-	unsigned long long *d_p = NULL; CHK(dev_alloc((void**)&d_p, 8));
-	wtz_pool_t *pool = c->dpool + which;
-	CHK(wtz_launch<K_poolalloc>(1, [=] WTZ_LAMBDA (uint64_t){ *d_p = (unsigned long long)(uintptr_t)wtz_pool_alloc(pool, bytes); }));
-	unsigned long long h = 0; CHK(dev_d2h(&h, d_p, 8));
-	if(h == 0) return wtz_fail(WTZ_E_POOL, "device scratch pool exhausted (%zu bytes for the K-sw1 problem lists)", bytes);
-	*out = (void*)(uintptr_t)h; return WTZ_OK;
+	unsigned long long *const d_mb = c->mb.d; wtz_pool_t *pool = c->dpool + which; const unsigned long long *w = NULL;
+	CHK(wtz_launch<K_poolalloc>(1, [=] WTZ_LAMBDA (uint64_t){ d_mb[0] = (unsigned long long)(uintptr_t)wtz_pool_alloc(pool, bytes); }));
+	CHK(mbox_read(&c->mb, 1, &w));
+	if(w[0] == 0){ c->last_pool_fail = which + 1; return wtz_fail(WTZ_E_POOL, "device scratch pool exhausted (%zu bytes for a host-side array)", bytes); }
+	*out = (void*)(uintptr_t)w[0]; return WTZ_OK;
 }
 static uint32_t lane_classes(const uint32_t ccnt[4], wtz_lclass_t *L){
 	uint32_t lo = 0, wv = 0;
 	for(int k = 0; k < 4; k++){ const uint32_t n = ccnt[3 - k]; L->lo[k] = lo; L->hi[k] = lo + n; wv += (n + WTZ_HOST_WAVE - 1) / WTZ_HOST_WAVE; L->wend[k] = wv; lo += n; }
 	return wv;
 }
-static size_t carve_bytes(size_t n, size_t elem){ return (n * elem + 255) & ~(size_t)255; }
+WTZ_HD size_t carve_bytes(size_t n, size_t elem){ return (n * elem + 255) & ~(size_t)255; }
 template<typename T> static void carve(uint8_t *&blk, T *&out, size_t n){ out = (T*)blk; blk += carve_bytes(n, sizeof(T)); }
 template<typename KEYS> static int sort_leftovers(uint32_t *d_list, uint32_t nl, KEYS launch_keys){
 	if(nl <= 64) return WTZ_OK;
@@ -253,12 +260,21 @@
 	CHK(dev_set(d_na, 0, (nwt + 1) * 4));
 	CHK(wtz_launch<K_lcount>(nwt, [=] WTZ_LAMBDA (uint64_t t){ wtz_task_lcount((uint32_t)t, d_wt, d_items, d_na); }));
 	CHK(dev_exclusive_scan_u32(d_na, d_woff, nwt + 1));
-	uint32_t NS = 0; CHK(dev_d2h(&NS, d_woff + nwt, 4));
-	lap(0);
+	unsigned long long *const d_mb = c->mb.d; wtz_pool_t *const mpool = c->dpool; const unsigned long long *w = NULL;
 	wtz_lprob_t *d_prob = NULL; uint32_t *d_cap = NULL, *d_roff = NULL, *d_val = NULL, *d_ccnt = NULL, *d_uidx = NULL, *d_nu = NULL; uint64_t *d_key = NULL; uint8_t *d_flag = NULL; wtz_lres_t *d_res = NULL;
-	{
+	uint32_t NS = 0;
+	{
+		const uint32_t *d_ns = d_woff + nwt;
+		CHK(wtz_launch<K_poolalloc>(1, [=] WTZ_LAMBDA (uint64_t){
+			const size_t nsp = (size_t)*d_ns + 64;
+			d_mb[0] = *d_ns;
+			d_mb[1] = (unsigned long long)(uintptr_t)wtz_pool_alloc(mpool, carve_bytes(nsp, sizeof(wtz_lprob_t)) + carve_bytes(nsp, sizeof(wtz_lres_t)) + 4 * carve_bytes(nsp, 4) + carve_bytes(nsp, 8));
+		}));
+		CHK(pool_letter(c, 2, 1, 1, "the K-sw1 problem lists", &w));
+		NS = (uint32_t)w[0];
+		lap(0);
 		const size_t nsp = (size_t)NS + 64;
-		uint8_t *blk = NULL; CHK(pool_alloc_host(c, 0, carve_bytes(nsp, sizeof(wtz_lprob_t)) + carve_bytes(nsp, sizeof(wtz_lres_t)) + 4 * carve_bytes(nsp, 4) + carve_bytes(nsp, 8), (void**)&blk));
+		uint8_t *blk = (uint8_t*)(uintptr_t)w[1];
 		carve(blk, d_prob, nsp); carve(blk, d_res, nsp); carve(blk, d_cap, nsp); carve(blk, d_roff, nsp); carve(blk, d_val, nsp); carve(blk, d_uidx, nsp); carve(blk, d_key, nsp);
 	}
 	CHK(dev_alloc((void**)&d_flag, nwt + 16)); CHK(dev_alloc((void**)&d_nu, (nwt + 1) * 4)); CHK(dev_alloc((void**)&d_ccnt, 32)); CHK(dev_set(d_ccnt, 0, 32));
@@ -267,9 +283,16 @@
 	CHK(wtz_launch<K_lplan>(nwt, [=] WTZ_LAMBDA (uint64_t t){ wtz_task_lplan((uint32_t)t, V, d_wt, d_items, d_woff, d_prob, d_cap, d_key, d_val, d_flag, d_ccnt, d_uidx, d_nu); }));
 	lap(1);
 	CHK(dev_exclusive_scan_u32(d_cap, d_roff, (uint64_t)NS + 1));
-	uint32_t NR = 0, ccnt[4] = {0, 0, 0, 0};
-	CHK(dev_d2h(&NR, d_roff + NS, 4)); CHK(dev_d2h(ccnt, d_ccnt, 16));
-	uint32_t *d_runs = NULL; CHK(pool_alloc_host(c, 0, ((size_t)NR + 16) * 4, (void**)&d_runs));
+	uint32_t NR = 0, ccnt[4] = {0, 0, 0, 0}; uint32_t *d_runs = NULL;
+	{
+		const uint32_t *d_nr = d_roff + NS, *d_cc = d_ccnt;
+		CHK(wtz_launch<K_poolalloc>(1, [=] WTZ_LAMBDA (uint64_t){
+			d_mb[0] = *d_nr; for(int k = 0; k < 4; k++) d_mb[1 + k] = d_cc[k];
+			d_mb[5] = (unsigned long long)(uintptr_t)wtz_pool_alloc(mpool, ((size_t)*d_nr + 16) * 4);
+		}));
+		CHK(pool_letter(c, 6, 5, 1, "the K-sw1 run lists", &w));
+		NR = (uint32_t)w[0]; for(int k = 0; k < 4; k++) ccnt[k] = (uint32_t)w[1 + k]; d_runs = (uint32_t*)(uintptr_t)w[5];
+	}
 	lap(2);
 	CHK(dev_sort_pairs_u64_u32(d_key, d_val, NS, 16));
 	lap(3);
@@ -285,7 +308,7 @@
 		lap(6);
 		CHK(wtz_launch<K_lfold>(nwt, [=] WTZ_LAMBDA (uint64_t t){ wtz_task_lfold((uint32_t)t, V, d_wt, d_items, d_woff, pp, ro, rn, rs, d_flag, d_fb, d_uidx, d_nu); }));
 	}
-	CHK(dev_d2h(n_fb, d_fb, 4));
+	CHK(fetch_u32(c, d_fb, n_fb));
 	{
 		const uint32_t nl = *n_fb; const uint32_t *lst = d_fb + 1;
 		CHK(sort_leftovers(d_fb, nl, [&](uint64_t *d_k2){ return wtz_launch<K_misc>(nl, [=] WTZ_LAMBDA (uint64_t i){
@@ -304,31 +327,46 @@
 	*n_list = 0;
 	if(nwt == 0) return WTZ_OK;
 	wtz_lgap_t *d_gp = NULL; uint32_t *d_cap = NULL, *d_roff = NULL, *d_val = NULL, *d_ccnt = NULL; uint64_t *d_key = NULL; uint8_t *d_done = NULL;
+	unsigned long long *const d_mb = c->mb.d; wtz_pool_t *const mpool = c->dpool; const unsigned long long *w = NULL;
+	wtz_lres_t *d_res = NULL;
 	{
 		const size_t nsp = (size_t)nwt + 64;
-		uint8_t *blk = NULL; CHK(pool_alloc_host(c, 0, carve_bytes(nsp, sizeof(wtz_lgap_t)) + 3 * carve_bytes(nsp, 4) + carve_bytes(nsp, 8) + carve_bytes(nsp, 1), (void**)&blk));
+		const size_t b_slots = carve_bytes(nsp, sizeof(wtz_lgap_t)) + 3 * carve_bytes(nsp, 4) + carve_bytes(nsp, 8) + carve_bytes(nsp, 1), b_res = ((size_t)nwt + 1) * sizeof(wtz_lres_t);
+		CHK(wtz_launch<K_poolalloc>(1, [=] WTZ_LAMBDA (uint64_t){
+			d_mb[0] = (unsigned long long)(uintptr_t)wtz_pool_alloc(mpool, b_slots);
+			d_mb[1] = (unsigned long long)(uintptr_t)wtz_pool_alloc(mpool, b_res);
+		}));
+		CHK(pool_letter(c, 2, 0, 2, "the K-sw2 problem lists", &w));
+		uint8_t *blk = (uint8_t*)(uintptr_t)w[0]; d_res = (wtz_lres_t*)(uintptr_t)w[1];
 		carve(blk, d_gp, nsp); carve(blk, d_cap, nsp); carve(blk, d_roff, nsp); carve(blk, d_val, nsp); carve(blk, d_key, nsp); carve(blk, d_done, nsp);
 	}
 	CHK(dev_alloc((void**)&d_ccnt, 32)); CHK(dev_set(d_ccnt, 0, 32));
 	CHK(dev_set(d_cap, 0, ((size_t)nwt + 1) * 4));
 	CHK(wtz_launch<K_gplan>(nwt, [=] WTZ_LAMBDA (uint64_t t){ wtz_task_gplan((uint32_t)t, V, d_wt, d_items, d_gaps, d_gp, d_cap, d_key, d_val, d_done, d_ccnt); }));
 	CHK(dev_exclusive_scan_u32(d_cap, d_roff, nwt + 1));
-	uint32_t NR = 0, ccnt[4] = {0, 0, 0, 0};
-	CHK(dev_d2h(&NR, d_roff + nwt, 4)); CHK(dev_d2h(ccnt, d_ccnt, 16));
-	uint32_t *d_runs = NULL; CHK(pool_alloc_host(c, 0, ((size_t)NR + 16) * 4, (void**)&d_runs));
+	uint32_t ccnt[4] = {0, 0, 0, 0}; uint32_t *d_runs = NULL;
+	{
+		const uint32_t *d_nr = d_roff + nwt, *d_cc = d_ccnt;
+		CHK(wtz_launch<K_poolalloc>(1, [=] WTZ_LAMBDA (uint64_t){
+			d_mb[0] = *d_nr; for(int k = 0; k < 4; k++) d_mb[1 + k] = d_cc[k];
+			d_mb[5] = (unsigned long long)(uintptr_t)wtz_pool_alloc(mpool, ((size_t)*d_nr + 16) * 4);
+		}));
+		CHK(pool_letter(c, 6, 5, 1, "the K-sw2 run lists", &w));
+		for(int k = 0; k < 4; k++) ccnt[k] = (uint32_t)w[1 + k]; d_runs = (uint32_t*)(uintptr_t)w[5];
+	}
 	CHK(dev_sort_pairs_u64_u32(d_key, d_val, nwt, 18));
 	CHK(dev_set(d_list, 0, 4));
 	{
 		const uint32_t *d_ord = d_val; const wtz_lgap_t *gp = d_gp; const uint32_t *ro = d_roff; uint32_t *rn = d_runs; uint8_t *dn = d_done;
 		wtz_lclass_t L; const uint32_t wv = lane_classes(ccnt, &L);
-		uint64_t *d_wtr = NULL; uint32_t *d_wrm = NULL; wtz_lres_t *d_res = NULL;
+		uint64_t *d_wtr = NULL; uint32_t *d_wrm = NULL;
 		CHK(dev_alloc((void**)&d_wtr, ((size_t)wv + 1) * 8)); CHK(dev_alloc((void**)&d_wrm, ((size_t)wv + 1) * 4)); CHK(dev_set(d_wtr, 0, ((size_t)wv + 1) * 8));
-		CHK(pool_alloc_host(c, 0, ((size_t)nwt + 1) * sizeof(wtz_lres_t), (void**)&d_res)); CHK(dev_set(d_res, 0, ((size_t)nwt + 1) * sizeof(wtz_lres_t)));
+		CHK(dev_set(d_res, 0, ((size_t)nwt + 1) * sizeof(wtz_lres_t)));
 		if(wv) CHK(wtz_launch_coop<K_gdp>(wv, [=] WTZ_LAMBDA (uint64_t t){ wtz_task_gdp_all((uint32_t)t, L, V, d_wt, d_items, d_ord, gp, d_res, d_wtr, d_wrm); }, 0));
 		if(wv) CHK(wtz_launch_coop<K_gtb>(wv, [=] WTZ_LAMBDA (uint64_t t){ wtz_task_gtb_all((uint32_t)t, L, V, d_wt, d_items, d_ord, gp, ro, rn, d_res, d_gaps, dn, d_wtr, d_wrm); }, 0));
 		CHK(wtz_launch<K_glist>(nwt, [=] WTZ_LAMBDA (uint64_t t){ wtz_task_glist((uint32_t)t, dn, d_list); }));
 	}
-	CHK(dev_d2h(n_list, d_list, 4));
+	CHK(fetch_u32(c, d_list, n_list));
 	{
 		const uint32_t nl = *n_list; const wtz_lgap_t *gp = d_gp; const uint32_t *lst = d_list + 1;
 		CHK(sort_leftovers(d_list, nl, [&](uint64_t *d_k2){ return wtz_launch<K_misc>(nl, [=] WTZ_LAMBDA (uint64_t i){
@@ -354,14 +392,14 @@
 	uint32_t *d_defer = NULL, n_def = 0; CHK(dev_alloc((void**)&d_defer, ((size_t)n + 1) * 4)); CHK(dev_set(d_defer, 0, 4));
 	if(d_list) CHK(wtz_launch_coop<K_winalign>(n, [=] WTZ_LAMBDA (uint64_t t){ wtz_task_winalign<false>((uint32_t)t, V, d_wt, d_items, d_defer, d_list); }, WTZ_WINALIGN_LDS_BYTES + WTZ_WINALIGN_QW_BYTES));
 	else CHK(wtz_launch_coop<K_winalign>(n, [=] WTZ_LAMBDA (uint64_t t){ wtz_task_winalign<false>((uint32_t)t, V, d_wt, d_items, d_defer, NULL); }, WTZ_WINALIGN_LDS_BYTES + WTZ_WINALIGN_QW_BYTES));
-	CHK(dev_d2h(&n_def, d_defer, 4));
+	CHK(fetch_u32(c, d_defer, &n_def));
 	if(n_def) CHK(wtz_launch_coop<K_winalign_big>(n_def, [=] WTZ_LAMBDA (uint64_t t){ wtz_task_winalign<true>((uint32_t)t, V, d_wt, d_items, NULL, d_defer); }, WTZ_WINALIGN_LDS_BYTES + WTZ_WINALIGN_QW_BYTES));
 	if(n_redone) *n_redone = n_def;
 	return WTZ_OK;
 #endif
 }
 
-static int compare_lane_with_chained(const wtz_reg_t *ra, const wtz_reg_t *rb, uint64_t nreg){
+static int compare_lane_with_chained(wtz_ctx *c, const wtz_reg_t *ra, const wtz_reg_t *rb, uint64_t nreg){
 	unsigned int *d_bad = NULL; CHK(dev_alloc((void**)&d_bad, 16)); CHK(dev_set(d_bad, 0, 16));
 	CHK(wtz_launch<K_misc>(nreg, [=] WTZ_LAMBDA (uint64_t i){
 		const wtz_reg_t &a = ra[i], &b = rb[i];
@@ -369,7 +407,7 @@
 		if(same && a.pass != 2 && b.pass != 2) for(uint32_t k = 0; k < a.cigar_len; k++) if(a.cigar[k] != b.cigar[k]){ same = false; break; }
 		if(!same){ const unsigned int z = WTZ_ATOMIC_INC32(&d_bad[0]); if(z == 0) d_bad[1] = (unsigned int)i; }
 	}));
-	unsigned int hb[4]; CHK(dev_d2h(hb, d_bad, 16));
+	unsigned int hb[4]; { const unsigned long long *w = NULL; CHK(fetch_small(c, d_bad, 16, &w)); memcpy(hb, w, 16); }
 	if(hb[0]){
 		wtz_reg_t a, b; CHK(dev_d2h(&a, ra + hb[1], sizeof a)); CHK(dev_d2h(&b, rb + hb[1], sizeof b));
 		return wtz_fail(WTZ_E_STATE, "K-sw1 lane pipeline differs from the chained kernel on %u of %llu windows; first: window slot %u chained/lane score %d/%d tb %d/%d te %d/%d qb %d/%d qe %d/%d aln %d/%d mat %d/%d mis %d/%d ins %d/%d del %d/%d cigar %u/%u pass %u/%u cells %llu/%llu",
@@ -386,7 +424,7 @@
 	uint32_t *d_defer = NULL, n_def = 0; CHK(dev_alloc((void**)&d_defer, (size_t)(nwt + 1) * 4)); CHK(dev_set(d_defer, 0, 4));
 	STAGE(c, "K_gap");
 	CHK(wtz_launch_coop<K_gap>(n_glist, [=] WTZ_LAMBDA (uint64_t t){ wtz_task_gap((uint32_t)t, V, d_wt, d_items, d_gaps, d_defer, (const uint32_t*)d_glist, 0u); }, WTZ_GAP_LDS_BYTES));
-	CHK(dev_d2h(&n_def, d_defer, 4));
+	CHK(fetch_u32(c, d_defer, &n_def));
 	if(n_def) CHK(wtz_launch_coop<K_gap_wide>(n_def, [=] WTZ_LAMBDA (uint64_t t){ wtz_task_gap((uint32_t)t, V, d_wt, d_items, d_gaps, NULL, d_defer, (uint32_t)WTZ_GAP_WIDE_LDS_BYTES); }, WTZ_GAP_WIDE_LDS_BYTES));
 	if(c->sw.profile){ CHK(dev_sync()); fprintf(stderr, "[gap-profile] %llu window slots, %u wide gaps redone with 72 KB of LDS\n", (unsigned long long)nwt, n_def); }
 	return WTZ_OK;
@@ -410,13 +448,13 @@
 	if(m == 0) return WTZ_OK;
 	CTX_ENTER(c);
 	if(!pair_idx || !dir || !out) return wtz_fail(WTZ_E_ARG, "null argument");
-	c->n_items = 0; c->have_items = false;
+	c->n_items = 0; c->have_items = false; c->h_alnres = NULL; c->last_pool_fail = 0;
 	const bool prof_wall = c->sw.profile; double tw[6] = {0, 0, 0, 0, 0, 0}; double tw0 = prof_wall ? wtz_wall() : 0;
 	auto lapw = [&](int k){ if(prof_wall){ const double t = wtz_wall(); tw[k] += t - tw0; tw0 = t; } };
 	CHK(reserve_items(c, m));
-	std::vector<wtz_alnitem_t> items(m); uint64_t nreg = 0;
-	std::vector<uint32_t> h_q(c->n_pairs), h_c(c->n_pairs);
-	CHK(dev_d2h(h_q.data(), c->d_qid, (size_t)c->n_pairs * 4)); CHK(dev_d2h(h_c.data(), c->d_cid, (size_t)c->n_pairs * 4));
+	wtz_alnitem_t *items = NULL; wtz_alnres_dev_t *h_res = NULL; uint64_t nreg = 0;
+	CHK(stage_reserve(&c->stg, WTZ_ST_ITEMS, (size_t)m * sizeof(wtz_alnitem_t), (void**)&items)); CHK(stage_reserve(&c->stg, WTZ_ST_ALNRES, (size_t)m * sizeof(wtz_alnres_dev_t), (void**)&h_res));
+	const uint32_t *h_q = c->h_qid, *h_c = c->h_cid;
 	for(uint32_t i = 0; i < m; i++){
 		if(pair_idx[i] >= c->n_pairs || dir[i] > 1) return wtz_fail(WTZ_E_ARG, "align item %u out of range", i);
 		const wtz_pairres_t &r = c->h_pairres[pair_idx[i]];
@@ -428,7 +466,7 @@
 	wtz_reg_t *d_regs = NULL; wtz_alnitem_t *d_items = NULL; wtz_wintask_t *d_wt = NULL;
 	CHK(dev_alloc((void**)&d_regs, (size_t)(nreg + 1) * sizeof(wtz_reg_t)));
 	for(uint32_t i = 0; i < m; i++) items[i].regs = d_regs + (uintptr_t)items[i].regs;
-	CHK(dev_alloc((void**)&d_items, (size_t)m * sizeof(wtz_alnitem_t))); CHK(dev_h2d(d_items, items.data(), (size_t)m * sizeof(wtz_alnitem_t)));
+	CHK(dev_alloc((void**)&d_items, (size_t)m * sizeof(wtz_alnitem_t))); CHK(dev_h2d_async(d_items, items, (size_t)m * sizeof(wtz_alnitem_t))); stage_uploaded(&c->stg, WTZ_ST_ITEMS);
 	CHK(dev_alloc((void**)&d_wt, (size_t)(nreg + 1) * sizeof(wtz_wintask_t)));
 	{ const wtz_alnitem_t *di = d_items; wtz_wintask_t *dw = d_wt; const wtz_reg_t *r0 = d_regs;
 	  CHK(wtz_launch<K_misc>(m, [=] WTZ_LAMBDA (uint64_t i){ const wtz_alnitem_t &it = di[i]; wtz_wintask_t *w = dw + (it.regs - r0); for(uint32_t k = 0; k < it.nwin; k++){ w[k].item = (uint32_t)i; w[k].widx = k; } })); }
@@ -450,11 +488,10 @@
 		CHK(run_winalign_chained(c, V, d_wt, d_items, NULL, nwt, &n_redone));
 		if(c->sw.profile) fprintf(stderr, "[winalign-profile] %zu windows, %u redone by the full task\n", (size_t)nreg, n_redone);
 	}
-	CHK(dev_sync());
-	if(d_regs_chk) CHK(compare_lane_with_chained(d_regs, d_regs_chk, nreg));
-	c->cnt.ms_winalign += tm.stop(); c->cnt.n_winalign += (size_t)nreg;
+	if(d_regs_chk){ CHK(dev_sync()); CHK(compare_lane_with_chained(c, d_regs, d_regs_chk, nreg)); }
+	tm.lap(); c->cnt.n_winalign += (size_t)nreg;
 	lapw(1);
-	tm.start();
+	wtz_timer tm_s; tm_s.start();
 	wtz_stitch_state_t *d_st = NULL; wtz_extjob_t *d_jl = NULL, *d_jr = NULL; wtz_gapres_t *d_gaps = NULL; int32_t *d_rgeo = NULL;
 	CHK(dev_alloc((void**)&d_st, (size_t)m * sizeof(wtz_stitch_state_t)));
 	CHK(dev_alloc((void**)&d_jl, (size_t)m * sizeof(wtz_extjob_t))); CHK(dev_alloc((void**)&d_jr, (size_t)m * sizeof(wtz_extjob_t)));
@@ -506,16 +543,17 @@
 	CHK(wtz_launch_coop<K_stitch_fin>(m, [=] WTZ_LAMBDA (uint64_t t){ wtz_task_stitch_fin((uint32_t)t, V, d_items, d_st, d_jl, d_jr, d_res); }));
 	if(c->P.refine) STAGE(c, "K_refine");
 	if(c->P.refine) CHK(wtz_launch_coop<K_refine>(m, [=] WTZ_LAMBDA (uint64_t t){ wtz_task_refine((uint32_t)t, V, d_items, d_res); }, WTZ_REFINE_LDS_BYTES));
+	tm_s.lap();
+	c->h_alnres = h_res; c->n_items = m; c->have_items = true;
+	CHK(dev_d2h_async(c->h_alnres, c->d_alnres, (size_t)m * sizeof(wtz_alnres_dev_t))); CHK(pool_head_post(c, 0));
 	CHK(dev_sync());
-	c->cnt.ms_stitch += tm.stop(); c->cnt.n_stitch += m;
+	c->cnt.ms_winalign += tm.read(); c->cnt.ms_stitch += tm_s.read(); c->cnt.n_stitch += m;
 	lapw(2);
-	c->h_alnres.resize(m); c->n_items = m; c->have_items = true;
-	CHK(dev_d2h(c->h_alnres.data(), c->d_alnres, (size_t)m * sizeof(wtz_alnres_dev_t)));
-	CHK(pool_check(c, "wtz_pairs_align"));
+	CHK(pool_check(c, "wtz_pairs_align", true));
 	uint64_t coff = 0, toff = 0;
 	for(uint32_t i = 0; i < m; i++){
 		const wtz_alnres_dev_t &r = c->h_alnres[i];
-		if(r.bad) return wtz_fail(WTZ_E_POOL, "wtz_pairs_align: item %u ran out of scratch", i);
+		if(r.bad){ c->last_pool_fail = 1; return wtz_fail(WTZ_E_POOL, "wtz_pairs_align: item %u ran out of scratch", i); }
 		wtz_aln_result_t o; memset(&o, 0, sizeof o);
 		o.score = r.x.score; o.tb = r.x.tb; o.te = r.x.te; o.qb = r.x.qb; o.qe = r.x.qe; o.aln = r.x.aln; o.mat = r.x.mat; o.mis = r.x.mis; o.ins = r.x.ins; o.del = r.x.del;
 		o.n_regs = r.n_regs; o.cigar_len = r.cigar_len; o.cigar_off = coff; coff += r.cigar_len; o.text_len = r.text_len; o.text_off = toff; toff += r.text_len;
diff --git a/smartdenovo_amd/csrc/wtz_lib_fetch.h b/smartdenovo_amd/csrc/wtz_lib_fetch.h
--- a/smartdenovo_amd/csrc/wtz_lib_fetch.h
+++ b/smartdenovo_amd/csrc/wtz_lib_fetch.h
@@ -5,14 +5,14 @@
 	if(tot != n_ops) return wtz_fail(WTZ_E_ARG, "wtz_fetch_cigars: expected room for %llu ops, got %llu", (unsigned long long)tot, (unsigned long long)n_ops);
 	if(tot == 0) return WTZ_OK;
 	if(!dst) return wtz_fail(WTZ_E_ARG, "null output");
-	std::vector<uint64_t> off((size_t)c->n_items + 1);
+	const size_t n_off = (size_t)c->n_items + 1;
+	uint64_t *off = NULL; CHK(stage_reserve(&c->stg, WTZ_ST_OFF, n_off * 8, (void**)&off));
 	uint64_t o = 0; for(uint32_t i = 0; i < c->n_items; i++){ off[i] = o; o += c->h_alnres[i].cigar_len; } off[c->n_items] = o;
 	uint64_t *d_off = NULL; uint32_t *d_c = NULL;
-	CHK(dev_alloc((void**)&d_off, off.size() * 8)); CHK(dev_h2d(d_off, off.data(), off.size() * 8));
+	CHK(dev_alloc((void**)&d_off, n_off * 8)); CHK(dev_h2d_async(d_off, off, n_off * 8)); stage_uploaded(&c->stg, WTZ_ST_OFF);
 	CHK(dev_alloc((void**)&d_c, (size_t)tot * 4));
 	const wtz_alnres_dev_t *dr = c->d_alnres;
 	CHK(wtz_launch<K_pack_cigars>(c->n_items, [=] WTZ_LAMBDA (uint64_t t){ const wtz_alnres_dev_t &r = dr[t]; for(uint32_t k = 0; k < r.cigar_len; k++) d_c[d_off[t] + k] = r.cigar[k]; }));
-	CHK(dev_sync());
 	CHK(dev_d2h(dst, d_c, (size_t)tot * 4));
 	return WTZ_OK;
 }
@@ -33,10 +33,11 @@
 		const size_t cap = (size_t)(tot + tot / 4 + 4096);
 		CHK(dev_alloc_persist((void**)&c->d_text, cap)); c->cap_text = cap;
 	}
-	std::vector<uint64_t> off((size_t)c->n_items + 1);
+	const size_t n_off = (size_t)c->n_items + 1;
+	uint64_t *off = NULL; CHK(stage_reserve(&c->stg, WTZ_ST_OFF, n_off * 8, (void**)&off));
 	uint64_t o = 0; for(uint32_t i = 0; i < c->n_items; i++){ off[i] = o; o += c->h_alnres[i].text_len; } off[c->n_items] = o;
 	uint64_t *d_off = NULL; char *d_t = c->d_text;
-	CHK(dev_alloc((void**)&d_off, off.size() * 8)); CHK(dev_h2d(d_off, off.data(), off.size() * 8));
+	CHK(dev_alloc((void**)&d_off, n_off * 8)); CHK(dev_h2d_async(d_off, off, n_off * 8)); stage_uploaded(&c->stg, WTZ_ST_OFF);
 	const wtz_alnres_dev_t *dr = c->d_alnres;
 	STAGE(c, "K_cigar_text");
 	CHK(wtz_launch_coop<K_cigar_text>(c->n_items, [=] WTZ_LAMBDA (uint64_t t){ const wtz_alnres_dev_t &r = dr[t]; if(r.text_len) wtz_cigar_text_write_coop(r.cigar, r.cigar_len, d_t + d_off[t]); }));
diff --git a/smartdenovo_amd/csrc/wtz_lib_pairs.h b/smartdenovo_amd/csrc/wtz_lib_pairs.h
--- a/smartdenovo_amd/csrc/wtz_lib_pairs.h
+++ b/smartdenovo_amd/csrc/wtz_lib_pairs.h
@@ -33,11 +33,16 @@
 	if(!c || !c->zs[0].have || (n && (!qid || !cid || !out))) return wtz_fail(WTZ_E_ARG, "z-index not built / null argument");
 	CTX_ENTER(c);
 	free_batch(c);
+	c->last_pool_fail = 0;
 	CHK(pool_reset(c));
-	if(n == 0){ c->n_pairs = 0; c->h_pairres.clear(); c->have_pairs = true; return WTZ_OK; }
+	if(n == 0){ c->n_pairs = 0; c->have_pairs = true; return WTZ_OK; }
 	for(uint32_t i = 0; i < n; i++) if(qid[i] >= c->n_reads || cid[i] >= c->n_reads) return wtz_fail(WTZ_E_ARG, "pair %u: read id out of range", i);
 	CHK(reserve_pairs(c, n));
-	CHK(dev_h2d(c->d_qid, qid, (size_t)n * 4)); CHK(dev_h2d(c->d_cid, cid, (size_t)n * 4));
+	uint32_t *h_ids = NULL, *h_ord = NULL; wtz_pairres_t *h_res = NULL;
+	CHK(stage_reserve(&c->stg, WTZ_ST_IDS, (size_t)n * 8, (void**)&h_ids)); CHK(stage_reserve(&c->stg, WTZ_ST_ORD, (size_t)n * 4, (void**)&h_ord));
+	CHK(stage_reserve(&c->stg, WTZ_ST_PAIRRES, (size_t)n * sizeof(wtz_pairres_t), (void**)&h_res));
+	memcpy(h_ids, qid, (size_t)n * 4); memcpy(h_ids + n, cid, (size_t)n * 4);
+	CHK(dev_h2d_async(c->d_qid, h_ids, (size_t)n * 4)); CHK(dev_h2d_async(c->d_cid, h_ids + n, (size_t)n * 4)); stage_uploaded(&c->stg, WTZ_ST_IDS);
 	const wtz_env_t V = ctx_env(c); const uint32_t *dq = c->d_qid, *dc = c->d_cid; wtz_pairres_t *dr = c->d_pairres;
 	wtz_timer tm; tm.start();
 	wtz_timer t1; t1.start();
@@ -58,14 +63,14 @@
 	if(c->sw.heavy_first >= 0 ? c->sw.heavy_first != 0 : c->P.dot_matrix != 0){
 		nh = n / 32u;
 		if(nh >= 8u){
-			std::vector<uint64_t> key(n); std::vector<uint32_t> ord(n), hv(n);
+			std::vector<uint64_t> key(n); std::vector<uint32_t> hv(n); uint32_t *ord = h_ord;
 			for(uint32_t i = 0; i < n; i++){ key[i] = (uint64_t)c->h_rdlen[qid[i]] * c->h_rdlen[cid[i]]; hv[i] = i; }
 			std::nth_element(hv.begin(), hv.begin() + nh, hv.end(), [&](uint32_t a, uint32_t b){ return key[a] != key[b] ? key[a] > key[b] : a < b; });
 			std::sort(hv.begin(), hv.begin() + nh, [&](uint32_t a, uint32_t b){ return key[a] != key[b] ? key[a] > key[b] : a < b; });
 			std::vector<uint8_t> heavy(n, 0);
 			for(uint32_t k = 0; k < nh; k++){ ord[k] = hv[k]; heavy[hv[k]] = 1; }
 			uint32_t w = nh; for(uint32_t i = 0; i < n; i++) if(!heavy[i]) ord[w++] = i;
-			uint32_t *dd = NULL; CHK(dev_alloc((void**)&dd, (size_t)n * 4)); CHK(dev_h2d(dd, ord.data(), (size_t)n * 4)); d_ord = dd;
+			uint32_t *dd = NULL; CHK(dev_alloc((void**)&dd, (size_t)n * 4)); CHK(dev_h2d_async(dd, ord, (size_t)n * 4)); stage_uploaded(&c->stg, WTZ_ST_ORD); d_ord = dd;
 		} else nh = 0;
 	}
 #endif
@@ -106,10 +111,10 @@
 		}
 	}
 #endif
+	if(c->sw.profile){ const double ms1 = t1.stop(); fprintf(stderr, "[pair-profile] K_pair first launch: %u pairs, %.1f ms\n", n, ms1); }
+	c->n_pairs = n; c->h_pairres = h_res; c->h_qid = h_ids; c->h_cid = h_ids + n; c->have_pairs = true;
+	CHK(dev_d2h_async(c->h_pairres, c->d_pairres, (size_t)n * sizeof(wtz_pairres_t))); CHK(pool_head_post(c, 0));
 	CHK(dev_sync());
-	{ const double ms1 = t1.stop(); if(c->sw.profile) fprintf(stderr, "[pair-profile] K_pair first launch: %u pairs, %.1f ms\n", n, ms1); }
-	c->n_pairs = n; c->h_pairres.resize(n); c->have_pairs = true;
-	CHK(dev_d2h(c->h_pairres.data(), c->d_pairres, (size_t)n * sizeof(wtz_pairres_t)));
 #ifndef WTZ_EMUL
 	if(!c->P.dot_matrix){
 		std::vector<uint32_t> list;
@@ -119,9 +124,9 @@
 			wtz_timer tt; tt.start();
 			STAGE(c, "K_pair_zbig");
 			CHK(wtz_launch_coop<K_pair_zbig>(list.size(), [=] WTZ_LAMBDA (uint64_t t){ wtz_task_pair<0, true>(d_list[t], V, dq, dc, dr); }, WTZ_PAIR_LDS_BYTES));
+			const double ms_t = c->sw.profile ? tt.stop() : 0.0;
+			CHK(dev_d2h_async(c->h_pairres, c->d_pairres, (size_t)n * sizeof(wtz_pairres_t))); CHK(pool_head_post(c, 0));
 			CHK(dev_sync());
-			const double ms_t = tt.stop();
-			CHK(dev_d2h(c->h_pairres.data(), c->d_pairres, (size_t)n * sizeof(wtz_pairres_t)));
 			if(c->sw.profile) fprintf(stderr, "[pair-profile] zmo pairs with ranges beyond the LDS slice: %zu of %u, %.1f ms\n", list.size(), n, ms_t);
 		}
 	}
@@ -139,15 +144,15 @@
 			wtz_timer tt; tt.start();
 			STAGE(c, "K_pair_big");
 			CHK(wtz_launch_coop<K_pair_big>(list.size(), [=] WTZ_LAMBDA (uint64_t t){ wtz_task_pair_dm_big((uint32_t)t, V, d_list, dq, dc, dr, lb, last, big); }, lb));
+			const double ms_t = c->sw.profile ? tt.stop() : 0.0;
+			CHK(dev_d2h_async(c->h_pairres, c->d_pairres, (size_t)n * sizeof(wtz_pairres_t))); CHK(pool_head_post(c, 0));
 			CHK(dev_sync());
-			const double ms_t = tt.stop();
-			CHK(dev_d2h(c->h_pairres.data(), c->d_pairres, (size_t)n * sizeof(wtz_pairres_t)));
 			if(c->sw.profile) fprintf(stderr, "[pair-profile] dmo tier %d (%u KB LDS): %zu pairs, %.1f ms\n", tier + 2, lb >> 10, list.size(), ms_t);
 		}
 	}
 	c->cnt.ms_pairs += tm.stop(); c->cnt.n_pairs += n;
 	for(uint32_t i = 0; i < n; i++) c->cnt.bytes_zmer_algo += (uint64_t)c->h_rdlen[cid[i]] / 4 + 16ull * c->h_pairres[i].n_hits;
-	CHK(pool_check(c, "wtz_pairs_seed"));
+	CHK(pool_check(c, "wtz_pairs_seed", true));
 	if(c->sw.profile){
 		uint64_t sum[4] = {0, 0, 0, 0}; uint32_t mx[4] = {0, 0, 0, 0}, arg = 0;
 		for(uint32_t i = 0; i < n; i++){ for(int k = 0; k < 4; k++){ sum[k] += c->h_pairres[i].tick[k]; if(c->h_pairres[i].tick[k] > mx[k]){ mx[k] = c->h_pairres[i].tick[k]; if(k == 3) arg = i; } } }
@@ -157,7 +162,7 @@
 	}
 	for(uint32_t i = 0; i < n; i++){
 		const wtz_pairres_t &r = c->h_pairres[i];
-		if(r.bad) return wtz_fail(WTZ_E_POOL, "wtz_pairs_seed: pair %u ran out of scratch", i);
+		if(r.bad){ c->last_pool_fail = 1; return wtz_fail(WTZ_E_POOL, "wtz_pairs_seed: pair %u ran out of scratch", i); }
 		wtz_pair_summary_t s; memset(&s, 0, sizeof s);
 		s.n_hits = r.n_hits; s.gate = r.gate; s.ovl[0] = r.ovl[0]; s.ovl[1] = r.ovl[1]; s.nwin[0] = r.nwin[0]; s.nwin[1] = r.nwin[1];
 		s.dm_score = r.dm_score; s.dm_qb = r.dm_qb; s.dm_qe = r.dm_qe; s.dm_tb = r.dm_tb; s.dm_te = r.dm_te; s.dm_dir = r.dm_dir;
@@ -173,18 +178,18 @@
 	if(tot != n_wins) return wtz_fail(WTZ_E_ARG, "wtz_pairs_windows: expected room for %llu windows, got %llu", (unsigned long long)tot, (unsigned long long)n_wins);
 	if(tot == 0) return WTZ_OK;
 	if(!wins) return wtz_fail(WTZ_E_ARG, "null output");
-	std::vector<uint64_t> off((size_t)c->n_pairs * 2 + 1);
+	const size_t n_off = (size_t)c->n_pairs * 2 + 1;
+	uint64_t *off = NULL; CHK(stage_reserve(&c->stg, WTZ_ST_OFF, n_off * 8, (void**)&off));
 	uint64_t o = 0; for(uint32_t i = 0; i < c->n_pairs; i++) for(int d = 0; d < 2; d++){ off[(size_t)i * 2 + d] = o; o += c->h_pairres[i].nwin[d]; }
 	off[(size_t)c->n_pairs * 2] = o;
 	uint64_t *d_off = NULL; wtz_winbox_t *d_w = NULL;
-	CHK(dev_alloc((void**)&d_off, off.size() * 8)); CHK(dev_h2d(d_off, off.data(), off.size() * 8));
+	CHK(dev_alloc((void**)&d_off, n_off * 8)); CHK(dev_h2d_async(d_off, off, n_off * 8)); stage_uploaded(&c->stg, WTZ_ST_OFF);
 	CHK(dev_alloc((void**)&d_w, (size_t)tot * sizeof(wtz_winbox_t)));
 	const wtz_pairres_t *dr = c->d_pairres;
 	CHK(wtz_launch<K_pack_windows>((uint64_t)c->n_pairs * 2, [=] WTZ_LAMBDA (uint64_t t){
 		const wtz_pairres_t &r = dr[t >> 1]; const uint32_t d = (uint32_t)(t & 1);
 		for(uint32_t k = 0; k < r.nwin[d]; k++){ wtz_winbox_t b; b.beg[0] = r.win[d][k].beg[0]; b.beg[1] = r.win[d][k].beg[1]; b.end[0] = r.win[d][k].end[0]; b.end[1] = r.win[d][k].end[1]; d_w[d_off[t] + k] = b; }
 	}));
-	CHK(dev_sync());
 	CHK(dev_d2h(wins, d_w, (size_t)tot * sizeof(wtz_winbox_t)));
 	return WTZ_OK;
 }
diff --git a/smartdenovo_amd/csrc/wtz_stage.h b/smartdenovo_amd/csrc/wtz_stage.h
--- /dev/null
+++ b/smartdenovo_amd/csrc/wtz_stage.h
@@ -0,0 +1,49 @@
+enum { WTZ_ST_PAIRRES = 0,
+       WTZ_ST_ALNRES,
+       WTZ_ST_IDS,
+       WTZ_ST_ORD,
+       WTZ_ST_ITEMS,
+       WTZ_ST_OFF,
+       WTZ_ST_N };
+struct wtz_staging {
+	void *p[WTZ_ST_N]; size_t cap[WTZ_ST_N];
+	uint64_t n_grow;
+	uint32_t up_pending;
+	wtz_staging(){ for(int k = 0; k < WTZ_ST_N; k++){ p[k] = NULL; cap[k] = 0; } n_grow = 0; up_pending = 0; }
+};
+static int stage_reserve(wtz_staging *st, int k, size_t n, void **out){
+	*out = NULL;
+	if(k < 0 || k >= WTZ_ST_N) return wtz_fail(WTZ_E_ARG, "staging slot %d out of range", k);
+	if(st->up_pending >> k & 1u){ CHK(dev_sync()); st->up_pending = 0; }
+	if(n > st->cap[k]){
+		size_t cap = st->cap[k] ? st->cap[k] : 4096; while(cap < n) cap += cap / 2 + 4096;
+		CHK(dev_sync());
+		if(st->p[k]) dev_host_free(st->p[k]);
+		st->p[k] = NULL; st->cap[k] = 0;
+		void *q = dev_host_alloc(cap);
+		if(!q) return wtz_fail(WTZ_E_HIP, "cannot allocate %zu bytes of page-locked host memory", cap);
+		st->p[k] = q; st->cap[k] = cap; st->n_grow++;
+	}
+	*out = st->p[k];
+	return WTZ_OK;
+}
+static void stage_free(wtz_staging *st){ for(int k = 0; k < WTZ_ST_N; k++){ if(st->p[k]) dev_host_free(st->p[k]); st->p[k] = NULL; st->cap[k] = 0; } st->up_pending = 0; }
+static void stage_uploaded(wtz_staging *st, int k){ st->up_pending |= 1u << k; }
+
+#define WTZ_MBOX_WORDS 16
+struct wtz_mailbox { unsigned long long *h, *d; uint64_t round; wtz_mailbox() : h(NULL), d(NULL), round(0) {} };
+static int mbox_create(wtz_mailbox *mb){
+	mb->h = (unsigned long long*)dev_host_alloc((WTZ_MBOX_WORDS + 16) * 8);
+	if(!mb->h) return wtz_fail(WTZ_E_HIP, "cannot allocate the page-locked mailbox");
+	memset(mb->h, 0, (WTZ_MBOX_WORDS + 16) * 8);
+	return dev_alloc_persist((void**)&mb->d, WTZ_MBOX_WORDS * 8);
+}
+static void mbox_free(wtz_mailbox *mb){ if(mb->h) dev_host_free(mb->h); dev_free_persist(mb->d); mb->h = NULL; mb->d = NULL; }
+static int mbox_read(wtz_mailbox *mb, uint32_t n, const unsigned long long **out){
+	*out = mb->h;
+	if(n == 0) return WTZ_OK;
+	if(n > WTZ_MBOX_WORDS) return wtz_fail(WTZ_E_ARG, "mailbox: %u words asked for, %d there", n, WTZ_MBOX_WORDS);
+	mb->round++;
+	CHK(dev_d2h_async(mb->h, mb->d, (size_t)n * 8));
+	return dev_sync();
+}
diff --git a/smartdenovo_amd/hipabi.py b/smartdenovo_amd/hipabi.py
--- a/smartdenovo_amd/hipabi.py
+++ b/smartdenovo_amd/hipabi.py
@@ -81,7 +81,8 @@
                 ("ms_kext", C.c_double), ("n_kext", C.c_uint64), ("cells_kext", C.c_uint64),
                 ("ms_kglob", C.c_double), ("n_kglob", C.c_uint64), ("cells_kglob", C.c_uint64),
                 ("ticks_kglob_dp", C.c_uint64), ("ticks_kglob_tb", C.c_uint64),
-                ("ms_pwtext", C.c_double), ("n_pwtext", C.c_uint64), ("bytes_pwtext", C.c_uint64)]
+                ("ms_pwtext", C.c_double), ("n_pwtext", C.c_uint64), ("bytes_pwtext", C.c_uint64),
+                ("n_stream_syncs", C.c_uint64), ("n_copies_h2d", C.c_uint64), ("n_copies_d2h", C.c_uint64), ("bytes_d2h", C.c_uint64)]
 
 
 def load(path: str | None = None) -> C.CDLL:
```

After: 10.79, median of 6. No clear change (+1.3%).
